# simonamtoft/downsampled-diffusion

Measured on AMD Instinct MI355X. Metric: images/sec (T=1000 sampling), 256x256 dDDPM-x3, higher is better.
Workload: dtype f32

## Files before the change

### downsampled-diffusion_amd/csrc/conv_wino.hip

```cpp
#include <atomic>
#include <cstdlib>
#include <type_traits>
#include <utility>

#include "conv_common.h"
#include "pack_elems.h"

namespace ddk {

__device__ __attribute__((aligned(128))) float g_wino_zero[32];

struct WinoParams {
    const float* src0;
    const float* src1;
    const float* wu;
    const float* bias;
    const float* resid;
    float* out;
    int c0, c1, cin;
    int B, H, W, TH, TW;
    int N, tiles;
    int splits, chunks, chunks_per_split;
    long long slab_stride;
    int post_mish;
    FastDivU dTW, dTH;
    float2* gn_part;
    int cpg, groups;
    const float* gn_gamma;
    const float* gn_beta;
    const float* gn_temb;
    const long long* gn_temb_rows;
    int gn_temb_stride;
    float gn_eps;
    float* cl_rec;
    unsigned* cl_cnt;
    unsigned* cl_fail;
    int cl_np;
    float* cl_slab;
    unsigned* cl_pair;
    const float* r1_x;
    const float* r1_w;
    const float* r1_b;
    int r1_cin, r1_ld;
};

constexpr int WBT = 32, WBN = 64;
constexpr int W_V = 4 * WBT * 32, W_U = 4 * WBN * 32;
constexpr int W_STAGE = W_V + W_U, W_NS = 3;
constexpr int W_LDS_FLOATS = W_NS * W_STAGE;
constexpr int W_TP = WBN + 4;
#ifndef DDK_WINO_LP
#define DDK_WINO_LP 4
#endif
constexpr int W_LP = DDK_WINO_LP;
static_assert(4 * 2 * WBT * W_TP <= W_LDS_FLOATS, "epilogue staging fits");

template <bool DGRAD>
__global__ __launch_bounds__(256) void pack_conv_weight_wino_kernel(const float* __restrict__ w, float* __restrict__ dst, int O, int I,
                                                                     int i_pad, long long total, int lo, int wi) {
    for (long long idx = blockIdx.x * 256LL + threadIdx.x; idx < total; idx += (long long)gridDim.x * 256)
        pack_wino_elem<DGRAD>(w, dst, idx, O, I, i_pad, lo, wi);
}

typedef int i32x4 __attribute__((ext_vector_type(4)));
typedef float f32x4 __attribute__((ext_vector_type(4)));

__device__ __forceinline__ i32x4 make_srd(const void* p, unsigned bytes) {
    const unsigned long long a = reinterpret_cast<unsigned long long>(p);
    i32x4 r;
    r.x = __builtin_amdgcn_readfirstlane((int)(unsigned)a);
    r.y = __builtin_amdgcn_readfirstlane((int)(unsigned)((a >> 32) & 0xFFFFu));
    r.z = __builtin_amdgcn_readfirstlane((int)bytes);
    r.w = 0x00020000;
    return r;
}
constexpr unsigned WINO_OOB = 0x80000000u;

__device__ __forceinline__ void buf_load16(f32x4& d, unsigned voff, const i32x4& srd, unsigned soff) {
    asm volatile("buffer_load_dwordx4 %0, %1, %2, %3 offen" : "=v"(d) : "v"(voff), "s"(srd), "s"(soff) : "memory");
}

__device__ __forceinline__ float4 f4add(float4 a, float4 b) { return make_float4(a.x + b.x, a.y + b.y, a.z + b.z, a.w + b.w); }
typedef float wino_f32x4 __attribute__((ext_vector_type(4)));
__device__ __forceinline__ void st_sc1_f4(float* p, float4 v) {
    const wino_f32x4 t = {v.x, v.y, v.z, v.w};
    asm volatile("global_store_dwordx4 %0, %1, off sc1\n\ts_nop 1" ::"v"(p), "v"(t) : "memory");
}
__device__ __forceinline__ void ld_sc1_f4x4(float4& a, float4& b, float4& c, float4& d, const float* pa, const float* pb, const float* pc,
                                            const float* pd) {
    wino_f32x4 x, y, z, w;
    asm volatile("global_load_dwordx4 %0, %4, off sc1\n\tglobal_load_dwordx4 %1, %5, off sc1\n\tglobal_load_dwordx4 %2, %6, off sc1\n\t"
                 "global_load_dwordx4 %3, %7, off sc1\n\ts_waitcnt vmcnt(0)"
                 : "=&v"(x), "=&v"(y), "=&v"(z), "=&v"(w)
                 : "v"(pa), "v"(pb), "v"(pc), "v"(pd)
                 : "memory");
    a = make_float4(x.x, x.y, x.z, x.w); b = make_float4(y.x, y.y, y.z, y.w);
    c = make_float4(z.x, z.y, z.z, z.w); d = make_float4(w.x, w.y, w.z, w.w);
}
__device__ __forceinline__ float4 f4sub(float4 a, float4 b) { return make_float4(a.x - b.x, a.y - b.y, a.z - b.z, a.w - b.w); }

__device__ unsigned long long g_wino_stamps[8 * 1024];

__device__ unsigned g_wino_cl_timeouts;
constexpr unsigned long long CL_TIMEOUT_TICKS = 2000000ull;

template <int DBG, bool CL = false>
__global__ __launch_bounds__(512) void conv3x3_wino_kernel(const WinoParams p) {
    extern __shared__ __attribute__((aligned(16))) float smem[];
    unsigned long long r_entry = 0;
    if (DBG) r_entry = __builtin_amdgcn_s_memrealtime();
    const int tid = threadIdx.x, lane = tid & 63;
    const int wid = __builtin_amdgcn_readfirstlane(tid >> 6);
    int tile_m, tile_n, split;
    {
        const int nwg = gridDim.x * gridDim.y * gridDim.z;
        const int bid = blockIdx.x + gridDim.x * (blockIdx.y + gridDim.y * blockIdx.z);
// ... 366 lines not shown
                    }
                }
            }
            __syncthreads();
            const unsigned long long* r0 = reinterpret_cast<const unsigned long long*>(p.cl_rec) +
                                           ((long long)image * p.cl_np * gridDim.y + tile_n) * 16 + gl;
            const bool poisoned = *gave_up != 0;
            float rm[8], rq[8];
#pragma unroll
            for (int i = 0; i < 8; ++i) {
                rm[i] = 0.f; rq[i] = 0.f;
                if (i < p.cl_np) {
                    const unsigned long long bits = __hip_atomic_load(r0 + (long long)i * gridDim.y * 16, __ATOMIC_RELAXED, __HIP_MEMORY_SCOPE_AGENT);
                    rm[i] = __uint_as_float((unsigned)bits);
                    rq[i] = __uint_as_float((unsigned)(bits >> 32));
                }
            }
            if (tid == 0) {
                const unsigned old = __hip_atomic_fetch_add(cnt + 1, 1u, __ATOMIC_RELAXED, __HIP_MEMORY_SCOPE_AGENT);
                if (old == (unsigned)p.cl_np - 1u) {
                    __hip_atomic_store(cnt, 0u, __ATOMIC_RELAXED, __HIP_MEMORY_SCOPE_AGENT);
                    __hip_atomic_store(cnt + 1, 0u, __ATOMIC_RELAXED, __HIP_MEMORY_SCOPE_AGENT);
                }
            }
            float ms = 0.f;
#pragma unroll
            for (int i = 0; i < 8; ++i) if (i < p.cl_np) ms += rm[i];
            const float gmean = poisoned ? __builtin_nanf("") : ms / (float)p.cl_np;
            float gm2 = 0.f, gd2 = 0.f;
#pragma unroll
            for (int i = 0; i < 8; ++i) if (i < p.cl_np) { gm2 += rq[i]; gd2 += (rm[i] - gmean) * (rm[i] - gmean); }
            const float n_i = 128.0f * (float)p.cpg;
            const float rstd = 1.0f / sqrtf((gm2 + n_i * gd2) / ((float)p.cl_np * n_i) + p.gn_eps);
            auto fin = [&](float4 v) {
                return make_float4(mish_f((v.x - gmean) * rstd * ga.x + be.x) + ts.x, mish_f((v.y - gmean) * rstd * ga.y + be.y) + ts.y,
                                   mish_f((v.z - gmean) * rstd * ga.z + be.z) + ts.z, mish_f((v.w - gmean) * rstd * ga.w + be.w) + ts.w);
            };
#pragma unroll
            for (int it = 0; it < 2; ++it) {
                *reinterpret_cast<float4*>(p.out + oo[it]) = f4add(fin(keep[it][0]), rs[it][0]);
                *reinterpret_cast<float4*>(p.out + oo[it] + p.N) = f4add(fin(keep[it][1]), rs[it][1]);
            }
        }
    }
    if (DBG && tid == 0) {
        asm volatile("s_waitcnt vmcnt(0)" ::: "memory");
        const int wg = (blockIdx.x + gridDim.x * (blockIdx.y + gridDim.y * blockIdx.z)) & 1023;
        g_wino_stamps[wg * 8 + 6] = __builtin_amdgcn_s_memrealtime();
        g_wino_stamps[wg * 8 + 7] = 1;
    }
}

#include "conv_wino2_kernel.inc"
#include "conv_winoT_kernel.inc"

enum { WINO_V_OLD = 0, WINO_V_D = 1, WINO_V_F = 2 };
static int wino_variant(int B, int H, int W, int N) {
#ifdef DDK_TUNING
    if (const char* e = getenv("DDK_WINO_VARIANT")) {
        const int v = atoi(e);
        if (v == WINO_V_OLD || v == WINO_V_D || (v == WINO_V_F && N % 128 == 0)) return v;
    }
#endif
    const long long mt = ceil_div((long long)B * (H / 2) * (W / 2), WBT);
    return (N % 128 == 0 && mt * (N / 128) >= 224) ? WINO_V_F : WINO_V_D;
}
static int wino_nt(int variant) { return variant == WINO_V_F ? 128 : WBN; }
bool conv_wino_ok(int kind, int H, int W, int cin, int N) {
    return kind == DDK_CONV3X3_S1 && H >= 2 && W >= 2 && H % 2 == 0 && W % 2 == 0 && cin > 0 && cin % 32 == 0 && N % 64 == 0;
}

int conv_wino_splits(int B, int H, int W, int cin, int N) {
    const long long tiles = (long long)B * (H / 2) * (W / 2);
    const long long wgs = ceil_div(tiles, WBT) * (N / wino_nt(wino_variant(B, H, W, N)));
    const int chunks = cin / 32;
    int s = 1;
    while (wgs * s < 256 && s * 2 <= chunks) s *= 2;
    const int cps = (int)ceil_div(chunks, s);
    return (int)ceil_div(chunks, cps);
}

static int wino_stats_shape_parts(int B, int H, int W, int cin, int N, int groups) {
    if (!conv_wino_ok(DDK_CONV3X3_S1, H, W, cin, N) || groups <= 0 || N % groups) return 0;
    const int cpg = N / groups, tpi = (H / 2) * (W / 2), nt_w = wino_nt(wino_variant(B, H, W, N));
    if (cpg % 4 || nt_w % cpg || nt_w / cpg > 8 || tpi % WBT || tpi / WBT > 32) return 0;
    return tpi / WBT;
}
int conv_wino_stats_parts(int B, int H, int W, int cin, int N, int groups) {
    if (conv_wino_splits(B, H, W, cin, N) != 1) return 0;
    return wino_stats_shape_parts(B, H, W, cin, N, groups);
}

bool convT_wino_ok(int H, int W, int cin, int N) {
    return H >= 2 && W >= 2 && H % 2 == 0 && W % 2 == 0 && cin > 0 && cin % 32 == 0 && N > 0 && N % WT_NT == 0;
}
int convT_wino_splits(int B, int H, int W, int cin, int N) {
    const long long wgs = ceil_div((long long)B * (H / 2) * (W / 2), WBT) * (N / WT_NT) * 4;
    const int chunks = cin / 32;
    int s = 1;
    while (wgs * s < 256 && s * 2 <= chunks) s *= 2;
    const int cps = (int)ceil_div(chunks, s);
    return (int)ceil_div(chunks, cps);
}
int convT_wino_forward(const ddk_conv_args& a, int splits, hipStream_t st) {
    WinoParams p{};
    p.src0 = a.src0; p.wu = a.weight_wino; p.bias = a.bias; p.out = a.out;
    p.c0 = a.c0; p.c1 = 0; p.cin = a.c0;
    p.B = a.B; p.H = a.H; p.W = a.W; p.TH = a.H / 2; p.TW = a.W / 2;
    p.N = a.N; p.tiles = a.B * p.TH * p.TW;
    p.chunks = p.cin / 32;
    p.chunks_per_split = (int)ceil_div(p.chunks, splits);
    p.splits = (int)ceil_div(p.chunks, p.chunks_per_split);
    p.slab_stride = (long long)a.B * (2 * a.H) * (2 * a.W) * a.N;
    p.dTW = make_fastdiv_u((unsigned)p.TW);
    p.dTH = make_fastdiv_u((unsigned)p.TH);
    if (p.splits > 1) p.out = static_cast<float*>(a.workspace);
    dim3 grid((unsigned)ceil_div(p.tiles, WBT), (unsigned)(a.N / WT_NT), (unsigned)(4 * p.splits));
#ifdef DDK_TUNING
    if (getenv("DDK_WINO_STAMPS")) {
        hipLaunchKernelGGL(convT_wino_kernel<1>, grid, dim3(1024), WT_LDS_FL * sizeof(float), st, p);
        return check_launch("convT_wino_kernel<dbg>");
    }
#endif
    hipLaunchKernelGGL(convT_wino_kernel<0>, grid, dim3(1024), WT_LDS_FL * sizeof(float), st, p);
    return check_launch("convT_wino_kernel");
}

int conv_wino_init_device() {
    DDK_HIP(hipFuncSetAttribute(reinterpret_cast<const void*>(&convT_wino_kernel<0>), hipFuncAttributeMaxDynamicSharedMemorySize,
                                (int)(WT_LDS_FL * sizeof(float))));
#ifdef DDK_TUNING
    DDK_HIP(hipFuncSetAttribute(reinterpret_cast<const void*>(&convT_wino_kernel<1>), hipFuncAttributeMaxDynamicSharedMemorySize,
                                (int)(WT_LDS_FL * sizeof(float))));
#endif
    DDK_HIP(hipFuncSetAttribute(reinterpret_cast<const void*>(&conv3x3_wino_kernel<0>), hipFuncAttributeMaxDynamicSharedMemorySize,
                                (int)(W_LDS_FLOATS * sizeof(float))));
    DDK_HIP(hipFuncSetAttribute(reinterpret_cast<const void*>(&conv3x3_wino_kernel<0, true>), hipFuncAttributeMaxDynamicSharedMemorySize,
                                (int)(W_LDS_FLOATS * sizeof(float))));
    DDK_HIP(hipFuncSetAttribute(reinterpret_cast<const void*>(&conv3x3_wino2_kernel<2, 0, false>), hipFuncAttributeMaxDynamicSharedMemorySize,
                                (int)(W2<2>::LDS_FL * sizeof(float))));
    DDK_HIP(hipFuncSetAttribute(reinterpret_cast<const void*>(&conv3x3_wino2_kernel<2, 0, true>), hipFuncAttributeMaxDynamicSharedMemorySize,
                                (int)(W2<2>::LDS_FL * sizeof(float))));
    DDK_HIP(hipFuncSetAttribute(reinterpret_cast<const void*>(&conv3x3_wino2_kernel<4, 0, false>), hipFuncAttributeMaxDynamicSharedMemorySize,
                                (int)(W2<4>::LDS_FL * sizeof(float))));
    DDK_HIP(hipFuncSetAttribute(reinterpret_cast<const void*>(&conv3x3_wino2_kernel<4, 0, true>), hipFuncAttributeMaxDynamicSharedMemorySize,
                                (int)(W2<4>::LDS_FL * sizeof(float))));
#ifdef DDK_TUNING
#define W2_DBG_ATTR(P_, D_) DDK_HIP(hipFuncSetAttribute(reinterpret_cast<const void*>(&conv3x3_wino2_kernel<P_, D_, false>), \
                                                hipFuncAttributeMaxDynamicSharedMemorySize, (int)(W2<P_>::LDS_FL * sizeof(float))))
    W2_DBG_ATTR(2, 1); W2_DBG_ATTR(2, 7); W2_DBG_ATTR(2, 9); W2_DBG_ATTR(2, 15); W2_DBG_ATTR(2, 17);
    W2_DBG_ATTR(4, 1); W2_DBG_ATTR(4, 7); W2_DBG_ATTR(4, 9); W2_DBG_ATTR(4, 15); W2_DBG_ATTR(4, 17);
#undef W2_DBG_ATTR
    DDK_HIP(hipFuncSetAttribute(reinterpret_cast<const void*>(&conv3x3_wino_kernel<1>), hipFuncAttributeMaxDynamicSharedMemorySize, (int)(W_LDS_FLOATS * sizeof(float))));
    DDK_HIP(hipFuncSetAttribute(reinterpret_cast<const void*>(&conv3x3_wino_kernel<2>), hipFuncAttributeMaxDynamicSharedMemorySize, (int)(W_LDS_FLOATS * sizeof(float))));
    DDK_HIP(hipFuncSetAttribute(reinterpret_cast<const void*>(&conv3x3_wino_kernel<3>), hipFuncAttributeMaxDynamicSharedMemorySize, (int)(W_LDS_FLOATS * sizeof(float))));
    DDK_HIP(hipFuncSetAttribute(reinterpret_cast<const void*>(&conv3x3_wino_kernel<4>), hipFuncAttributeMaxDynamicSharedMemorySize, (int)(W_LDS_FLOATS * sizeof(float))));
#endif
    return DDK_OK;
}

int conv_wino_cluster_np(int B, int H, int W, int cin, int N, int groups) {
    const int np = conv_wino_stats_parts(B, H, W, cin, N, groups);
    if (np <= 0 || np > 8) return 0;
    const int nt_w = wino_nt(wino_variant(B, H, W, N));
    if (N / groups > 32 || nt_w % (N / groups)) return 0;
    if (nt_w / (N / groups) > 8) return 0;
    const long long mt = (long long)B * np, nt = N / nt_w;
    if ((mt * nt) % 8) return 0;
    const long long run = mt * nt / 8;
    const long long per_round = run < 32 ? run : 32;
    if (run % (np * nt) || per_round % (np * nt)) return 0;
    return np;
}
int conv_wino_cluster_split_np(int B, int H, int W, int cin, int N, int groups, int* splits_out) {
    if (!conv_wino_ok(DDK_CONV3X3_S1, H, W, cin, N)) return 0;
    const int splits = conv_wino_splits(B, H, W, cin, N);
    if (splits_out) *splits_out = splits;
    if (splits <= 1 || splits > 4) return 0;
    const int np = wino_stats_shape_parts(B, H, W, cin, N, groups);
    if (np <= 0 || np > 8) return 0;
    const int variant = wino_variant(B, H, W, N);
    if (variant != WINO_V_D) return 0;
    const int nt_w = wino_nt(variant);
    if (N / groups > 32 || nt_w % (N / groups) || nt_w / (N / groups) > 8) return 0;
    const long long mt = (long long)B * np, nt = N / nt_w;
    if (mt * nt * splits > 256) return 0;
    return np;
}
size_t conv_wino_cluster_pair_words(int B, int H, int W, int N) {
    return (size_t)ceil_div((long long)B * (H / 2) * (W / 2), WBT) * (size_t)(N / WBN) * 16;
}
// ... 67 lines not shown
    p.post_mish = a.post_mish;
    p.dTW = make_fastdiv_u((unsigned)p.TW);
    p.dTH = make_fastdiv_u((unsigned)p.TH);
    if (p.splits > 1 && !fuse) p.out = static_cast<float*>(a.workspace);
    const int variant = wino_variant(a.B, a.H, a.W, a.N);
    if (variant != WINO_V_OLD) {
        dim3 grid2((unsigned)ceil_div(p.tiles, WBT), (unsigned)(a.N / wino_nt(variant)), (unsigned)p.splits);
        const bool f = variant == WINO_V_F;
        const size_t lds = (size_t)(f ? W2<2>::LDS_FL : W2<4>::LDS_FL) * sizeof(float);
#ifdef DDK_TUNING
        if (getenv("DDK_WINO_STAMPS")) {
            const int v = getenv("DDK_WINO_DEBUG") ? atoi(getenv("DDK_WINO_DEBUG")) : 1;
#define W2_DBG_LAUNCH(D_)                                                                                              \
    if (v == D_) {                                                                                                     \
        if (f) hipLaunchKernelGGL((conv3x3_wino2_kernel<2, D_, false>), grid2, dim3(768), lds, st, p);                 \
        else hipLaunchKernelGGL((conv3x3_wino2_kernel<4, D_, false>), grid2, dim3(768), lds, st, p);                   \
        return check_launch("conv3x3_wino2_kernel<dbg>");                                                              \
    }
            W2_DBG_LAUNCH(7) W2_DBG_LAUNCH(9) W2_DBG_LAUNCH(15) W2_DBG_LAUNCH(17)
#undef W2_DBG_LAUNCH
            if (f) hipLaunchKernelGGL((conv3x3_wino2_kernel<2, 1, false>), grid2, dim3(768), lds, st, p);
            else hipLaunchKernelGGL((conv3x3_wino2_kernel<4, 1, false>), grid2, dim3(768), lds, st, p);
            return check_launch("conv3x3_wino2_kernel<dbg>");
        }
#endif
        if (fuse) {
            if (f) hipLaunchKernelGGL((conv3x3_wino2_kernel<2, 0, true>), grid2, dim3(768), lds, st, p);
            else hipLaunchKernelGGL((conv3x3_wino2_kernel<4, 0, true>), grid2, dim3(768), lds, st, p);
            return check_launch("conv3x3_wino2_kernel<cluster>");
        }
        if (f) hipLaunchKernelGGL((conv3x3_wino2_kernel<2, 0, false>), grid2, dim3(768), lds, st, p);
        else hipLaunchKernelGGL((conv3x3_wino2_kernel<4, 0, false>), grid2, dim3(768), lds, st, p);
        return check_launch("conv3x3_wino2_kernel");
    }
    dim3 grid((unsigned)ceil_div(p.tiles, WBT), (unsigned)(a.N / WBN), (unsigned)p.splits);
#ifdef DDK_TUNING
    if (getenv("DDK_WINO_STAMPS")) {
        const int v = getenv("DDK_WINO_DEBUG") ? atoi(getenv("DDK_WINO_DEBUG")) : 1;
        if (v == 2) hipLaunchKernelGGL(conv3x3_wino_kernel<2>, grid, dim3(512), W_LDS_FLOATS * sizeof(float), st, p);
        else if (v == 3) hipLaunchKernelGGL(conv3x3_wino_kernel<3>, grid, dim3(512), W_LDS_FLOATS * sizeof(float), st, p);
        else if (v == 4) hipLaunchKernelGGL(conv3x3_wino_kernel<4>, grid, dim3(512), W_LDS_FLOATS * sizeof(float), st, p);
        else hipLaunchKernelGGL(conv3x3_wino_kernel<1>, grid, dim3(512), W_LDS_FLOATS * sizeof(float), st, p);
        return check_launch("conv3x3_wino_kernel<dbg>");
    }
#endif
    if (fuse) {
        hipLaunchKernelGGL((conv3x3_wino_kernel<0, true>), grid, dim3(512), W_LDS_FLOATS * sizeof(float), st, p);
        return check_launch("conv3x3_wino_kernel<cluster>");
    }
    hipLaunchKernelGGL(conv3x3_wino_kernel<0>, grid, dim3(512), W_LDS_FLOATS * sizeof(float), st, p);
    return check_launch("conv3x3_wino_kernel");
}

__global__ __launch_bounds__(256) void occupy_kernel(unsigned long long ticks, unsigned* sink) {
    extern __shared__ float occupy_lds[];
    occupy_lds[threadIdx.x] = (float)threadIdx.x;
    __syncthreads();
    const unsigned long long t_begin = __builtin_amdgcn_s_memrealtime();
    while (__builtin_amdgcn_s_memrealtime() - t_begin < ticks) __builtin_amdgcn_s_sleep(32);
    if (occupy_lds[(threadIdx.x + 1) & 255] < 0.f && sink) *sink = 1;
}

unsigned conv_wino_cluster_timeouts() {
    unsigned v = 0;
    if (hipMemcpyFromSymbol(&v, HIP_SYMBOL(g_wino_cl_timeouts), sizeof(v)) != hipSuccess) return ~0u;
    return v;
}

}

extern "C" int ddk_pack_conv_weight_wino(const float* w_oihw, float* dst, int O, int I, int i_pad, ddk_stream_t s) {
    using namespace ddk;
    DDK_REQUIRE(w_oihw && dst && O > 0 && I > 0 && i_pad >= I && i_pad % 32 == 0, "pack_conv_weight_wino: arguments (i_pad % 32 == 0)");
    const long long total = (long long)O * i_pad;
    DDK_REQUIRE(total < (1LL << 31), "pack_conv_weight_wino: 2^31 (n, c) pairs or more");
    const long long blocks = ceil_div(total, 256);
    hipLaunchKernelGGL(pack_conv_weight_wino_kernel<false>, dim3((unsigned)(blocks < 4096 ? blocks : 4096)), dim3(256), 0, as_stream(s), w_oihw,
                       dst, O, I, i_pad, total, 0, I);
    return check_launch("pack_conv_weight_wino_kernel");
}

extern "C" int ddk_pack_convT_weight_wino(const float* w_iohw, float* dst, int I, int O, int i_pad, ddk_stream_t s) {
    using namespace ddk;
    DDK_REQUIRE(w_iohw && dst && O > 0 && I > 0 && i_pad >= I && i_pad % 32 == 0, "pack_convT_weight_wino: arguments (i_pad % 32 == 0)");
    const long long total = (long long)O * i_pad;
    const long long blocks = ceil_div(total, 256);
    hipLaunchKernelGGL(pack_convT_weight_wino_kernel, dim3((unsigned)(blocks < 4096 ? blocks : 4096)), dim3(256), 0, as_stream(s), w_iohw, dst,
                       I, O, i_pad, total);
    return check_launch("pack_convT_weight_wino_kernel");
}
extern "C" int ddk_convT_wino_splits(int B, int H, int W, int cin, int N) {
    if (!ddk::convT_wino_ok(H, W, cin, N)) return 0;
    return ddk::convT_wino_splits(B, H, W, cin, N);
}

extern "C" int ddk_pack_conv_weight_wino_dgrad(const float* w_oihw, float* dst, int O, int I, int c_lo, int c_hi, int o_pad, ddk_stream_t s) {
    using namespace ddk;
    DDK_REQUIRE(w_oihw && dst && O > 0 && I > 0 && c_lo >= 0 && c_hi > c_lo && c_hi <= I && o_pad >= O && o_pad % 32 == 0,
                "pack_conv_weight_wino_dgrad: arguments (0 <= c_lo < c_hi <= I, o_pad % 32 == 0)");
    const long long total = (long long)(c_hi - c_lo) * o_pad;
    DDK_REQUIRE(total < (1LL << 31), "pack_conv_weight_wino_dgrad: 2^31 (n, c) pairs or more");
    const long long blocks = ceil_div(total, 256);
    hipLaunchKernelGGL(pack_conv_weight_wino_kernel<true>, dim3((unsigned)(blocks < 4096 ? blocks : 4096)), dim3(256), 0, as_stream(s), w_oihw,
                       dst, c_hi - c_lo, O, o_pad, total, c_lo, I);
    return check_launch("pack_conv_weight_wino_kernel<dgrad>");
}

#ifdef DDK_TUNING
extern "C" int ddk_debug_read_wino_timeline(unsigned long long* host_out) {
    if (hipDeviceSynchronize() != hipSuccess) return -2;
    return hipMemcpyFromSymbol(host_out, HIP_SYMBOL(ddk::g_wino_timeline), sizeof(unsigned long long) * 12 * 8 * 2) == hipSuccess ? 0 : -2;
}
extern "C" int ddk_debug_read_wino_stamps(unsigned long long* host_out) {
    if (hipDeviceSynchronize() != hipSuccess) return -2;
    if (hipMemcpyFromSymbol(host_out, HIP_SYMBOL(ddk::g_wino_stamps), sizeof(unsigned long long) * 8 * 1024) != hipSuccess) return -2;
    static unsigned long long zeros[8 * 1024];
    return hipMemcpyToSymbol(HIP_SYMBOL(ddk::g_wino_stamps), zeros, sizeof(zeros)) == hipSuccess ? 0 : -2;
}
#endif

extern "C" int ddk_conv_gn_partials(int B, int H, int W, int cin, int N, int groups) {
    return ddk::conv_wino_stats_parts(B, H, W, cin, N, groups);
}

extern "C" int ddk_conv_wino_splits(int B, int H, int W, int cin, int N) {
    if (!ddk::conv_wino_ok(DDK_CONV3X3_S1, H, W, cin, N)) return 0;
    return ddk::conv_wino_splits(B, H, W, cin, N);
}

extern "C" int ddk_conv3x3_gn_mish_cluster_ok(int B, int H, int W, int cin, int N, int groups) {
    if (!ddk::conv_wino_cluster_device_ok()) return 0;
    const int np = ddk::conv_wino_cluster_np(B, H, W, cin, N, groups);
// ... 70 lines not shown
```

### downsampled-diffusion_amd/csrc/ddk_internal.h

```cpp
#pragma once
#include <hip/hip_runtime.h>

#include <cstdarg>
#include <cstdint>
#include <cstdio>

#include "ddk.h"

#ifdef DDK_HOST_SANITIZE
#include "host_sanitize.h"
#endif

namespace ddk {

void set_error(const char* fmt, ...);

inline int fail_arg(const char* what) {
    set_error("bad argument: %s", what);
    return DDK_ERR_ARG;
}

inline int check_launch(const char* what) {
    hipError_t e = hipGetLastError();
    if (e != hipSuccess) {
// ... 66 lines not shown
    const int lane = threadIdx.x & 63, wid = threadIdx.x >> 6, nw = blockDim.x >> 6;
    __syncthreads();
    if (lane == 0) red[wid] = v;
    __syncthreads();
    float t = (lane < nw) ? red[lane] : 0.0f;
    t = wave_sum(t);
    return t;
}

__device__ __forceinline__ float block_max(float v, float* red) {
    v = wave_max(v);
    const int lane = threadIdx.x & 63, wid = threadIdx.x >> 6, nw = blockDim.x >> 6;
    __syncthreads();
    if (lane == 0) red[wid] = v;
    __syncthreads();
    float t = (lane < nw) ? red[lane] : -INFINITY;
    t = wave_max(t);
    return t;
}

int ensure_device_init();
int conv_init_device();
int wgrad_init_device();

size_t conv_workspace_bytes(int kind, int B, int H, int W, int cin, int N);
struct ConvLnFold {
    const float* c1;
    const float* c2;
    float eps;
};
struct WinoGnFuse {
    const float* gamma;
    const float* beta;
    const float* temb;
    const long long* temb_rows;
    int temb_stride;
    float eps;
    int groups;
    float* records;
    unsigned* counters;
    unsigned* fail;
    unsigned* pairs = nullptr;
    const float* res_x = nullptr;
    const float* res_w = nullptr;
    const float* res_b = nullptr;
    int res_cin = 0, res_ld = 0;
};
bool conv_ln_fold_ok(int B, int H, int W, int cin, int N);
int conv_forward(const ddk_conv_args& a, hipStream_t st, const ConvLnFold* ln = nullptr, const WinoGnFuse* fuse = nullptr);
int conv_splits(int kind, int B, int H, int W, int cin, int N);
bool conv_wino_ok(int kind, int H, int W, int cin, int N);
int conv_wino_splits(int B, int H, int W, int cin, int N);
int conv_wino_forward(const ddk_conv_args& a, int splits, hipStream_t st, const WinoGnFuse* fuse = nullptr);
int conv_wino_cluster_np(int B, int H, int W, int cin, int N, int groups);
int conv_wino_cluster_split_np(int B, int H, int W, int cin, int N, int groups, int* splits_out);
size_t conv_wino_cluster_pair_words(int B, int H, int W, int N);
bool conv_wino_variant_new(int B, int H, int W, int N);
bool conv_wino_cluster_device_ok();
size_t conv_wino_cluster_ws_floats(int B, int H, int W, int N);
unsigned conv_wino_cluster_timeouts();
bool convT_wino_ok(int H, int W, int cin, int N);
int convT_wino_splits(int B, int H, int W, int cin, int N);
int convT_wino_forward(const ddk_conv_args& a, int splits, hipStream_t st);
int conv_wino_init_device();
int conv_wino_stats_parts(int B, int H, int W, int cin, int N, int groups);
bool conv_first_ok(int cin, int N, int H, int W, int groups);
int conv_first(const float* x, const float* wp, const float* bias, float* out, float* gn_partials, int B, int H, int W, int cin, int N,
               int groups, int64_t* counter, int64_t* t_cur, hipStream_t st);
int conv_first_init_device();
bool conv_first_gn_ok(int cin, int N, int H, int W, int groups);
size_t conv_first_gn_ws_floats(int B, int H, int W);
int conv_first_gn(const float* x, const float* wp, const float* bias, const float* gamma, const float* beta, const float* temb,
                  int temb_stride, const long long* temb_rows, float eps, float* out, int B, int H, int W, int cin, int N, int groups,
                  float* records, unsigned* counters, unsigned* fail, int64_t* counter, int64_t* t_cur, hipStream_t st);
bool conv1x1_sm_ok(long long M, int c0, int c1, int N);
int conv1x1_sm(const float* src0, int c0, const float* src1, int c1, const float* w, const float* bias, const float* resid, float* out,
               long long M, int N, const ConvLnFold* ln, hipStream_t st);
int conv1x1_sm_init_device();
bool conv1x1_stream_ok(long long M, int cin, int N);
int conv1x1_stream(const float* x, int cin, const float* w, const float* bias, const float* dmish_src, const float* resid, float* out,
                   float* mish_out, long long M, int N, int pre_mish, int post_mish, hipStream_t st);
bool conv1x1_ws_ok(long long M, int K, int N);
int conv1x1_ws(const float* x, const float* w, const float* bias, const float* resid, float* out, long long M, int N, const ConvLnFold* ln,
               hipStream_t st, int images = 0);
int conv1x1_ws_init_device();
struct AddendSlabs {
    int n = 1;
    long long stride = 0;
    const float* bias = nullptr;
};
bool conv_gn_local_ok(int H, int W, int cin, int c0, int N, int groups);
int conv_gn_local(const float* src0, int c0, const float* src1, int c1, const float* w, const float* bias, const float* gamma,
                  const float* beta, const float* temb, int temb_stride, const long long* temb_rows, const float* addend, float* out,
                  int B, int H, int W, int N, int groups, float eps, hipStream_t st, const AddendSlabs& as = AddendSlabs(),
                  const AddendSlabs& src_slabs = AddendSlabs());
int conv_gn_local_init_device();
bool conv_gn_wlocal_ok(int H, int W, int cin, int c0, int N, int groups);
int conv_gn_wlocal(const float* src0, int c0, const float* src1, int c1, const float* w, const float* bias, const float* gamma,
                   const float* beta, const float* temb, int temb_stride, const long long* temb_rows, const float* addend, float* out,
                   int B, int H, int W, int N, int groups, float eps, hipStream_t st, const AddendSlabs& as = AddendSlabs(),
                   const AddendSlabs& src_slabs = AddendSlabs());
double conv_flops(int kind, int B, int H, int W, int cin, int N);
size_t groupnorm_workspace_bytes(int B, int HW, int C, int groups);
int gn_train_nsplit(int HW, int cpg);
int gn_stats_partials(const float* x, float* part, int B, int HW, int C, int groups, int ns, hipStream_t st);
int groupnorm_mish(const float* x, const float* gamma, const float* beta, const float* temb, int temb_stride,
// ... 53 lines not shown
```

### downsampled-diffusion_amd/csrc/unet_plan.hip

```cpp
#include <mutex>
#include <string>
#include <vector>

#include "ddk_internal.h"
#include "level_chain.h"

namespace ddk {

constexpr int HEADS = 4;
constexpr int HIDDEN = HEADS * 32;
constexpr int GROUPS = 8;
constexpr float GN_EPS = 1e-5f, LN_EPS = 1e-5f;

static inline int pad32(int c) { return (c + 31) / 32 * 32; }

enum PackKind { PK_COPY = 0, PK_CONV = 1, PK_CONVT = 2, PK_LINEAR_T = 3, PK_WINO = 4, PK_LOCAL = 5, PK_WLOCAL = 6, PK_FIRST = 7, PK_CONVT_WINO = 8,
                PK_ROWS = 9 , PK_LOCAL1 = 10 ,
                PK_CONVT_LOCAL = 11  };

struct Slot {
    std::string name;
    long long numel;
    int kind;
    size_t off;
    int O, I, KH, KW, i_pad, ld, col0;
    int split = 0, split_pad = 0;
    int attn = -1;
};

struct ConvW {
    size_t w = 0, b = 0;
    bool has_bias = false;
    int cin = 0, cin_pad = 0, cout = 0;
    size_t wu = 0;
    bool has_wu = false;
    size_t wl = 0;
    bool has_wl = false;
    size_t wwl = 0;
    bool has_wwl = false;
    size_t wf = 0;
    bool has_wf = false;
    size_t wl1 = 0;
    bool has_wl1 = false;
    size_t wtl = 0;
    bool has_wtl = false;
};
struct NormW { size_t g = 0, b = 0; int c_real = 0; };
struct ResW {
    int ci = 0, ci_pad = 0, co = 0, temb_off = 0, ci_real = 0, co_real = 0;
    ConvW c1, c2, res;
    NormW n1, n2;
    bool has_res = false;
};
struct AttnW {
    int c = 0, c_real = 0;
    NormW ln;
    ConvW qkv, out;
    size_t qkv_lnw = 0, ln_c1 = 0, ln_c2 = 0;
    size_t qkv_op = 0;
};

}

using namespace ddk;

struct SamplerGraph {
    const void *packed, *x, *noise, *ws, *c_recip, *c_recipm1, *c1, *c2, *sigma;
    int B, H, W, t_start, device;
    unsigned long long pack_epoch;
    hipGraph_t graph = nullptr;
    hipGraphExec_t exec = nullptr;
    hipGraph_t graph_multi = nullptr;
    hipGraphExec_t exec_multi = nullptr;
    hipEvent_t done = nullptr;
    unsigned long long last_use = 0;
};
constexpr int SAMPLER_MULTI = 16;

struct ddk_unet {
    std::mutex mu;
    std::vector<SamplerGraph> graphs;
    unsigned long long use_clock = 0;
    unsigned long long pack_epoch = 0;
    struct { const void* ws = nullptr; int t_start = -1, B = 0, H = 0, W = 0; unsigned long long pack_epoch = 0; } table;
    ddk_unet_config cfg;
    int cluster_gn = 1;
    int cluster_limit = 1 << 30;
    int cluster_np_max = 8;
    bool cluster_split = true;
    bool attn_kvctx = true;
    bool fold_down_reduce = false;
    bool first_gn = true;
    int level_chain = 9;
    int level_chain_max_batch = 32;
    int attn_fold_min_hw = 256;
    bool attn_fold = true;
    bool generic = false;
    std::vector<int> dimp;
    std::vector<Slot> slots;
    size_t packed_floats = 0;
    int L = 0;
    std::vector<int> dims;
    int time_dim = 0, temb_total = 0;
    size_t freqs = 0, w1t = 0, b1 = 0, w2t = 0, b2 = 0, temb_wt = 0, temb_bias = 0;
    std::vector<ResW> down_res, up_res;
    std::vector<AttnW> down_attn, up_attn;
    std::vector<ConvW> down_conv, up_conv;
    ResW mid1, mid2;
    AttnW mid_attn;
    ConvW final_conv;
    NormW final_norm;
    size_t final_w = 0, final_b = 0;

    size_t alloc(size_t n) {
        const size_t o = packed_floats;
        packed_floats += (n + 3) / 4 * 4;
        return o;
    }
    size_t add_copy(const std::string& name, long long n) {
        const size_t o = alloc((size_t)n);
        slots.push_back(Slot{name, n, PK_COPY, o, 0, 0, 0, 0, 0, 0, 0});
        return o;
    }
    void add_copy_at(const std::string& name, long long n, size_t off) {
        slots.push_back(Slot{name, n, PK_COPY, off, 0, 0, 0, 0, 0, 0, 0});
    }
    ConvW add_conv(const std::string& prefix, int cout, int cin, int k, bool bias, bool gn_follows = false, int split = 0, bool local = false) {
        ConvW c;
        c.cin = cin; c.cin_pad = split > 0 ? pad32(split) + pad32(cin - split) : pad32(cin); c.cout = cout;
        const int cout_rows = pad32(cout);
        c.w = alloc((size_t)cout_rows * k * k * c.cin_pad);
        Slot sl{prefix + "weight", (long long)cout * cin * k * k, PK_CONV, c.w, cout, cin, k, k, c.cin_pad, 0, 0};
        if (split > 0 && c.cin_pad != cin) { sl.split = split; sl.split_pad = pad32(split); }
        slots.push_back(sl);
        c.has_bias = bias;
        if (bias) {
            c.b = alloc((size_t)cout_rows);
            slots.push_back(Slot{prefix + "bias", cout, PK_COPY, c.b, 0, 0, 0, 0, 0, 0, 0});
        }
        if (generic) return c;
        if (k == 1 && bias && cout % 32 == 0 && c.cin_pad == cin && cin % 32 == 0) {
            c.wl1 = alloc((size_t)cout * c.cin_pad);
            c.has_wl1 = true;
            slots.push_back(Slot{prefix + "weight", (long long)cout * cin, PK_LOCAL1, c.wl1, cout, cin, 1, 1, c.cin_pad, 0, 0});
        }
        if (k == 3 && cout % 64 == 0) {
            c.wu = alloc((size_t)16 * cout * c.cin_pad);
            c.has_wu = true;
            slots.push_back(Slot{prefix + "weight", (long long)cout * cin * k * k, PK_WINO, c.wu, cout, cin, k, k, c.cin_pad, 0, 0});
        }
        if (k == 3 && (gn_follows || local) && cout % 32 == 0) {
            c.wl = alloc((size_t)9 * cout * c.cin_pad);
            c.has_wl = true;
            slots.push_back(Slot{prefix + "weight", (long long)cout * cin * k * k, PK_LOCAL, c.wl, cout, cin, k, k, c.cin_pad, 0, 0});
            if (gn_follows && (c.cin_pad <= 320 || c.cin_pad == 512)) {
                c.wwl = alloc((size_t)16 * cout * c.cin_pad);
                c.has_wwl = true;
                slots.push_back(Slot{prefix + "weight", (long long)cout * cin * k * k, PK_WLOCAL, c.wwl, cout, cin, k, k, c.cin_pad, 0, 0});
            }
        }
        return c;
    }
    ConvW add_convT(const std::string& prefix, int ch, bool local = false) {
        ConvW c;
        c.cin = ch; c.cin_pad = pad32(ch); c.cout = ch;
        c.w = alloc((size_t)16 * pad32(ch) * pad32(ch));
        slots.push_back(Slot{prefix + "weight", (long long)16 * ch * ch, PK_CONVT, c.w, ch, ch, 4, 4, pad32(ch), 0, 0});
        c.has_bias = true;
        c.b = alloc((size_t)pad32(ch));
        slots.push_back(Slot{prefix + "bias", ch, PK_COPY, c.b, 0, 0, 0, 0, 0, 0, 0});
        if (local && ch % 32 == 0 && !generic) {
            c.wtl = alloc((size_t)16 * ch * ch);
            c.has_wtl = true;
            slots.push_back(Slot{prefix + "weight", (long long)16 * ch * ch, PK_CONVT_LOCAL, c.wtl, ch, ch, 4, 4, ch, 0, 0});
        }
        if (ch % 128 == 0) {
            c.wu = alloc((size_t)36 * ch * ch);
            c.has_wu = true;
            slots.push_back(Slot{prefix + "weight", (long long)16 * ch * ch, PK_CONVT_WINO, c.wu, ch, ch, 4, 4, ch, 0, 0});
        }
        return c;
    }
    NormW add_norm(const std::string& wname, const std::string& bname, int c) {
        NormW n;
        n.c_real = c;
        n.g = alloc((size_t)pad32(c));
        slots.push_back(Slot{wname, c, PK_COPY, n.g, 0, 0, 0, 0, 0, 0, 0});
        n.b = alloc((size_t)pad32(c));
        slots.push_back(Slot{bname, c, PK_COPY, n.b, 0, 0, 0, 0, 0, 0, 0});
        return n;
    }
    ResW add_res(const std::string& p, int ci, int co, int& temb_cursor, int split = 0) {
        ResW r;
        r.ci_real = ci; r.co_real = co;
        r.ci = ci; r.ci_pad = split > 0 ? pad32(split) + pad32(ci - split) : pad32(ci); r.co = pad32(co);
        if (!generic) r.co = co;
        r.temb_off = temb_cursor;
        temb_cursor += co;
        slots.push_back(Slot{p + "mlp.1.weight", (long long)co * time_dim, PK_LINEAR_T, temb_wt, co, time_dim, 0, 0, 0, temb_total, r.temb_off});
        add_copy_at(p + "mlp.1.bias", co, temb_bias + r.temb_off);
        r.c1 = add_conv(p + "block1.block.0.", co, ci, 3, true, true, split);
        r.n1 = add_norm(p + "block1.block.1.weight", p + "block1.block.1.bias", co);
// ... 7 lines not shown
    std::vector<AttnW> attn_all;
    AttnW add_attn(const std::string& p, int c) {
        AttnW a;
        a.c = generic ? pad32(c) : c;
        a.c_real = c;
        const size_t s0 = slots.size();
        a.qkv = add_conv(p + "fn.fn.to_qkv.", 3 * HIDDEN, c, 1, false);
        const size_t s1 = slots.size();
        a.out = add_conv(p + "fn.fn.to_out.", c, HIDDEN, 1, true);
        const size_t s2 = slots.size();
        a.ln = add_norm(p + "fn.norm.g", p + "fn.norm.b", c);
        for (size_t i = s0; i < s1; ++i) slots[i].attn = n_attn;
        for (size_t i = s2; i < slots.size(); ++i) slots[i].attn = n_attn;
        a.qkv_lnw = alloc((size_t)3 * HIDDEN * pad32(c));
        a.ln_c1 = alloc((size_t)3 * HIDDEN);
        a.ln_c2 = alloc((size_t)3 * HIDDEN);
        a.qkv_op = alloc((size_t)3 * HIDDEN * pad32(c));
        attn_all.push_back(a);
        ++n_attn;
        return a;
    }
};

static int total_temb(const ddk_unet& u) {
    int tot = 0;
    for (int l = 0; l < u.L; ++l) tot += 2 * u.dims[l + 1];
    tot += 2 * u.dims[u.L];
    for (int i = 0; i < u.L - 1; ++i) tot += 2 * u.dims[u.L - 1 - i];
    return tot;
}

extern "C" ddk_unet* ddk_unet_create(const ddk_unet_config* cfg) {
    if (!cfg || cfg->n_levels < 1 || cfg->n_levels > 8 || cfg->in_ch < 1 || cfg->chan < 8 || cfg->chan % 8 ||
        cfg->chan > 512) {
        set_error("unet_create: need 1 <= n_levels <= 8, in_ch >= 1, unet_chan a multiple of 8 in [8, 512]");
        return nullptr;
    }
    for (int i = 0; i < cfg->n_levels; ++i)
        if (cfg->mults[i] < 1) { set_error("unet_create: unet_dims entries must be >= 1"); return nullptr; }
    if (cfg->mults[0] != 1) {
        set_error("unet_create: unet_dims[0] must be 1 (the reference's final Block(dim, dim) meets dim * unet_dims[0] channels "
                  "otherwise and raises, unet.py:69-72)");
        return nullptr;
    }
    {
        int ndev = 0;
        if (hipGetDeviceCount(&ndev) == hipSuccess && ndev > 0 && ensure_device_init() != DDK_OK) return nullptr;
        (void)hipGetLastError();
    }
    ddk_unet* u = new ddk_unet();
    u->cfg = *cfg;
    u->L = cfg->n_levels;
    u->generic = cfg->chan % 32 != 0;
    for (int i = 0; i < cfg->n_levels; ++i)
        if (cfg->chan * cfg->mults[i] > 512) { set_error("unet_create: level widths above 512 channels are not supported"); delete u; return nullptr; }
    u->dims.push_back(cfg->in_ch);
    for (int i = 0; i < u->L; ++i) u->dims.push_back(cfg->chan * cfg->mults[i]);
    for (int d : u->dims) u->dimp.push_back(u->generic ? pad32(d) : d);
    u->time_dim = cfg->chan;
    u->temb_total = total_temb(*u);
    const int td = u->time_dim;

    u->freqs = u->add_copy("@sinusoidal_freqs", td / 2);
    u->w1t = u->alloc((size_t)td * 4 * td);
    u->slots.push_back(Slot{"time_mlp.1.weight", (long long)4 * td * td, PK_LINEAR_T, u->w1t, 4 * td, td, 0, 0, 0, 4 * td, 0});
    u->b1 = u->add_copy("time_mlp.1.bias", 4 * td);
    u->w2t = u->alloc((size_t)4 * td * td);
    u->slots.push_back(Slot{"time_mlp.3.weight", (long long)4 * td * td, PK_LINEAR_T, u->w2t, td, 4 * td, 0, 0, 0, td, 0});
    u->b2 = u->add_copy("time_mlp.3.bias", td);
    u->temb_wt = u->alloc((size_t)td * u->temb_total);
    u->temb_bias = u->alloc((size_t)u->temb_total);

    int cur = 0;
    for (int l = 0; l < u->L; ++l) {
        const std::string p = "downs." + std::to_string(l) + ".";
        const int ci = u->dims[l], co = u->dims[l + 1];
        u->down_res.push_back(u->add_res(p + "0.", ci, co, cur));
        if (l == 0 && ci <= 8 && co <= 256 && !u->generic) {
            ConvW& c1 = u->down_res[0].c1;
            const int K2 = (9 * ci + 1) / 2;
            c1.wf = u->alloc((size_t)(co / 32) * K2 * 64);
            c1.has_wf = true;
            u->slots.push_back(Slot{p + "0.block1.block.0.weight", (long long)co * ci * 9, PK_FIRST, c1.wf, co, ci, 3, 3, 0, 0, 0});
        }
        u->down_res.push_back(u->add_res(p + "1.", co, co, cur));
        u->down_attn.push_back(u->add_attn(p + "2.", co));
        if (l < u->L - 1) u->down_conv.push_back(u->add_conv(p + "3.conv.", co, co, 3, true, false, 0, l == u->L - 2));
    }
    const int mid = u->dims[u->L];
    u->mid1 = u->add_res("mid_block1.", mid, mid, cur);
    u->mid_attn = u->add_attn("mid_attn.", mid);
    u->mid2 = u->add_res("mid_block2.", mid, mid, cur);
    for (int i = 0; i < u->L - 1; ++i) {
        const std::string p = "ups." + std::to_string(i) + ".";
        const int din = u->dims[u->L - 1 - i], dout = u->dims[u->L - i];
        u->up_res.push_back(u->add_res(p + "0.", 2 * dout, din, cur, dout));
        u->up_res.push_back(u->add_res(p + "1.", din, din, cur));
        u->up_attn.push_back(u->add_attn(p + "2.", din));
        u->up_conv.push_back(u->add_convT(p + "3.conv.", din, i == 0));
    }
    u->final_conv = u->add_conv("final_conv.0.block.0.", cfg->chan, cfg->chan, 3, true, true);
    u->final_norm = u->add_norm("final_conv.0.block.1.weight", "final_conv.0.block.1.bias", cfg->chan);
    if (u->generic) {
        u->final_w = u->alloc((size_t)cfg->in_ch * pad32(cfg->chan));
        u->slots.push_back(Slot{"final_conv.1.weight", (long long)cfg->in_ch * cfg->chan, PK_ROWS, u->final_w, cfg->in_ch, cfg->chan, 0, 0, 0,
                                pad32(cfg->chan), 0});
// ... 29 lines not shown
}

extern "C" int ddk_sampler_invalidate(ddk_unet* u) {
    DDK_REQUIRE(u, "sampler_invalidate: null plan");
    std::lock_guard<std::mutex> lock(u->mu);
    if (!u->graphs.empty()) DDK_HIP(hipDeviceSynchronize());
    drop_graphs(u);
    return DDK_OK;
}
static void destroy_entry(SamplerGraph& g) {
    if (g.done) { (void)hipEventSynchronize(g.done); (void)hipEventDestroy(g.done); }
    if (g.exec) (void)hipGraphExecDestroy(g.exec);
    if (g.graph) (void)hipGraphDestroy(g.graph);
    if (g.exec_multi) (void)hipGraphExecDestroy(g.exec_multi);
    if (g.graph_multi) (void)hipGraphDestroy(g.graph_multi);
}

extern "C" int ddk_sampler_release_workspace(ddk_unet* u, const void* workspace) {
    DDK_REQUIRE(u && workspace, "sampler_release_workspace: arguments");
    std::lock_guard<std::mutex> lock(u->mu);
    for (size_t i = 0; i < u->graphs.size();) {
        if (u->graphs[i].ws == workspace) {
            destroy_entry(u->graphs[i]);
            u->graphs.erase(u->graphs.begin() + (long)i);
        } else {
            ++i;
        }
    }
    if (u->table.ws == workspace) u->table.ws = nullptr;
    return DDK_OK;
}

extern "C" int ddk_unet_set_option(ddk_unet* u, int option, int value) {
    DDK_REQUIRE(u, "unet_set_option: null plan");
    if (option == DDK_OPT_CLUSTER_GROUPNORM) {
        std::lock_guard<std::mutex> lock(u->mu);
        if (!u->graphs.empty()) DDK_HIP(hipDeviceSynchronize());
        drop_graphs(u);
        u->cluster_gn = value < 0 ? 0 : value > 2 ? 2 : value;
        return DDK_OK;
    }
    if (option == DDK_OPT_ATTENTION_FOLD) {
        std::lock_guard<std::mutex> lock(u->mu);
        if (!u->graphs.empty()) DDK_HIP(hipDeviceSynchronize());
        drop_graphs(u);
        u->attn_fold = value != 0;
        return DDK_OK;
    }
    if (option == DDK_OPT_ATTENTION_KV_CONTEXT) {
        std::lock_guard<std::mutex> lock(u->mu);
        if (!u->graphs.empty()) DDK_HIP(hipDeviceSynchronize());
        drop_graphs(u);
        u->attn_kvctx = value != 0;
        return DDK_OK;
    }
    if (option == DDK_OPT_FIRST_GROUPNORM) {
        std::lock_guard<std::mutex> lock(u->mu);
        if (!u->graphs.empty()) DDK_HIP(hipDeviceSynchronize());
        drop_graphs(u);
        u->first_gn = value != 0;
        return DDK_OK;
    }
    if (option == DDK_OPT_LEVEL_CHAIN) {
        std::lock_guard<std::mutex> lock(u->mu);
        if (!u->graphs.empty()) DDK_HIP(hipDeviceSynchronize());
        drop_graphs(u);
        u->level_chain = value == 1 ? 9 : value == 2 ? 1 : value == 3 ? 15 : value == 4 ? 6 : value == 8 ? 2 : value == 16 ? 4 : value != 0 ? 9 : 0;
        return DDK_OK;
    }
    if (option == DDK_OPT_FOLD_DOWNSAMPLE_REDUCE) {
        std::lock_guard<std::mutex> lock(u->mu);
        if (!u->graphs.empty()) DDK_HIP(hipDeviceSynchronize());
        drop_graphs(u);
        u->fold_down_reduce = value != 0;
        return DDK_OK;
    }
    if (option == 10) {
        std::lock_guard<std::mutex> lock(u->mu);
        if (!u->graphs.empty()) DDK_HIP(hipDeviceSynchronize());
        drop_graphs(u);
        u->level_chain_max_batch = value;
        return DDK_OK;
    }
    if (option == 9) {
        std::lock_guard<std::mutex> lock(u->mu);
        if (!u->graphs.empty()) DDK_HIP(hipDeviceSynchronize());
        drop_graphs(u);
        u->attn_fold_min_hw = value;
        return DDK_OK;
    }
    if (option == 2) {
        std::lock_guard<std::mutex> lock(u->mu);
        u->cluster_limit = value;
        return DDK_OK;
    }
    if (option == 4) {
        std::lock_guard<std::mutex> lock(u->mu);
        if (!u->graphs.empty()) DDK_HIP(hipDeviceSynchronize());
        drop_graphs(u);
        u->cluster_np_max = value;
        return DDK_OK;
    }
    if (option == 11) {
        std::lock_guard<std::mutex> lock(u->mu);
        if (!u->graphs.empty()) DDK_HIP(hipDeviceSynchronize());
        drop_graphs(u);
// ... 22 lines not shown
        wg[(long long)n * cp + c] = wv * gv;
        s1 += wv * gv;
        s2 += wv * bv;
    }
    s1 = wave_sum(s1);
    s2 = wave_sum(s2);
    if (threadIdx.x == 0) { c1[n] = s1; c2[n] = s2; }
}

static int fold_attn(const AttnW& a, float* P, hipStream_t st) {
    hipLaunchKernelGGL(ln_fold_kernel, dim3(3 * HIDDEN), dim3(64), 0, st, P + a.qkv.w, P + a.ln.g, P + a.ln.b, P + a.qkv_lnw, P + a.ln_c1,
                       P + a.ln_c2, a.c, pad32(a.c));
    DDK_TRY(check_launch("ln_fold_kernel"));
    return qkv_operand_pack(P + a.qkv_lnw, P + a.qkv_op, HEADS, pad32(a.c), st);
}

static void weights_changed(const ddk_unet* u) {
    ddk_unet* m = const_cast<ddk_unet*>(u);
    std::lock_guard<std::mutex> lock(m->mu);
    ++m->pack_epoch;
}

extern "C" int ddk_unet_finalize_pack(const ddk_unet* u, void* packed, ddk_stream_t s) {
    DDK_REQUIRE(u && packed, "unet_finalize_pack: arguments");
    weights_changed(u);
    for (const AttnW& a : u->attn_all) DDK_TRY(fold_attn(a, static_cast<float*>(packed), as_stream(s)));
    return DDK_OK;
}

extern "C" int ddk_unet_pack_slot(const ddk_unet* u, int slot, const float* canonical, void* packed, ddk_stream_t s) {
    DDK_REQUIRE(u && canonical && packed && slot >= 0 && slot < (int)u->slots.size(), "unet_pack_slot: arguments");
    const Slot& sl = u->slots[slot];
    float* dst = static_cast<float*>(packed) + sl.off;
    weights_changed(u);
    int rc;
    switch (sl.kind) {
        case PK_COPY:
            DDK_HIP(hipMemcpyAsync(dst, canonical, (size_t)sl.numel * sizeof(float), hipMemcpyDeviceToDevice, as_stream(s)));
            rc = DDK_OK;
            break;
        case PK_CONV:
            rc = sl.split > 0 ? ddk_pack_conv_weight_split(canonical, dst, sl.O, sl.I, sl.KH, sl.KW, sl.i_pad, sl.split, sl.split_pad, s)
                              : ddk_pack_conv_weight(canonical, dst, sl.O, sl.I, sl.KH, sl.KW, sl.i_pad, s);
            break;
        case PK_CONVT: rc = sl.i_pad == sl.I ? ddk_pack_convT_weight(canonical, dst, sl.I, sl.O, s)
                                             : ddk_pack_convT_weight_padded(canonical, dst, sl.I, sl.O, sl.i_pad, s); break;
        case PK_ROWS:
            DDK_HIP(hipMemcpy2DAsync(dst, (size_t)sl.ld * sizeof(float), canonical, (size_t)sl.I * sizeof(float), (size_t)sl.I * sizeof(float),
                                     (size_t)sl.O, hipMemcpyDeviceToDevice, as_stream(s)));
            rc = DDK_OK;
            break;
        case PK_LINEAR_T: rc = ddk_pack_linear_T(canonical, dst, sl.O, sl.I, sl.ld, sl.col0, s); break;
        case PK_WINO: rc = ddk_pack_conv_weight_wino(canonical, dst, sl.O, sl.I, sl.i_pad, s); break;
        case PK_LOCAL: rc = ddk_pack_conv_weight_local(canonical, dst, sl.O, sl.I, sl.i_pad, s); break;
        case PK_LOCAL1: rc = ddk_pack_conv1x1_weight_local(canonical, dst, sl.O, sl.I, sl.i_pad, s); break;
        case PK_CONVT_LOCAL: rc = ddk_pack_convT_weight_local(canonical, dst, sl.I, sl.O, s); break;
        case PK_WLOCAL: rc = ddk_pack_conv_weight_wino_local(canonical, dst, sl.O, sl.I, sl.i_pad, s); break;
        case PK_FIRST: rc = ddk_pack_conv_weight_first(canonical, dst, sl.O, sl.I, s); break;
        case PK_CONVT_WINO: rc = ddk_pack_convT_weight_wino(canonical, dst, sl.I, sl.O, sl.i_pad, s); break;
        default: return fail_arg("unet_pack_slot: slot kind");
    }
    DDK_TRY(rc);
    if (sl.attn >= 0) DDK_TRY(fold_attn(u->attn_all[sl.attn], static_cast<float*>(packed), as_stream(s)));
    return DDK_OK;
}

namespace ddk {

struct Layout {
    size_t act = 0;
    size_t qkv = 0, o = 0, ctx = 0, splitk = 0, gn_ws = 0, cl = 0, chain = 0;
    std::vector<size_t> skip;
    size_t xpad = 0, temb = 0, tact = 0;
    size_t off_A = 0, off_B = 0, off_C = 0, off_raw = 0, off_a1 = 0, off_res = 0, off_xn = 0, off_qkv = 0, off_o = 0, off_ctx = 0,
           off_splitk = 0, off_gn = 0, off_xpad = 0, off_temb = 0, off_tact = 0, off_cl = 0, off_chain = 0;
    std::vector<size_t> off_skip;
    size_t total = 0;
};

static size_t al4(size_t n) { return (n + 3) / 4 * 4; }

static void upd(size_t& m, size_t v) { if (v > m) m = v; }

static bool convT_wino_use(int B, int H, int W, int cin, int N) {
    return convT_wino_ok(H, W, cin, N) && convT_wino_splits(B, H, W, cin, N) <= 2;
}
static bool use_wino(const ConvW& cw, int H, int W, int cin, int N) {
    return cw.has_wu && conv_wino_ok(DDK_CONV3X3_S1, H, W, cin, N);
}
static int conv3_splits(const ConvW& cw, int B, int H, int W, int cin, int N) {
    return use_wino(cw, H, W, cin, N) ? conv_wino_splits(B, H, W, cin, N) : conv_splits(DDK_CONV3X3_S1, B, H, W, cin, N);
}
static size_t conv3_ws_floats(const ConvW& cw, int B, int H, int W, int cin, int N) {
    if (!use_wino(cw, H, W, cin, N)) return conv_workspace_bytes(DDK_CONV3X3_S1, B, H, W, cin, N) / 4;
    const int s = conv_wino_splits(B, H, W, cin, N);
    return s > 1 ? (size_t)s * B * H * W * N : 0;
}

constexpr size_t CL_PAIR_WORDS = 128 * 16;
static size_t cl_counter_floats(int B) { return (size_t)B * 8 * 16 + 16 + (size_t)B * 64 + CL_PAIR_WORDS; }
static size_t cl_fail_offset(int B) { return (size_t)B * 8 * 16; }
static size_t cl_chain_offset(int B) { return (size_t)B * 8 * 16 + 16; }
static size_t cl_pair_offset(int B) { return (size_t)B * 8 * 16 + 16 + (size_t)B * 64; }
constexpr int CHAIN_BUFS = 18;
constexpr int CHAIN8_BUFS = 5;

// ... 84 lines not shown
    ly.act = al4(ly.act); ly.qkv = al4(ly.qkv); ly.o = al4(ly.o); ly.ctx = al4(ly.ctx);
    ly.splitk = al4(ly.splitk); ly.gn_ws = al4(ly.gn_ws); ly.cl = al4(ly.cl);
    if (level_chain_shape_ok(u, H0, W0)) ly.chain = (size_t)CHAIN_BUFS * B * 16 * 256;
    if (level8_chain_shape_ok(u, H0, W0)) upd(ly.chain, (size_t)CHAIN8_BUFS * B * 64 * 256);

    size_t off = 0;
    auto take = [&](size_t n) { const size_t o = off; off += n; return o; };
    ly.off_A = take(ly.act); ly.off_B = take(ly.act); ly.off_C = take(ly.act);
    ly.off_raw = take(ly.act); ly.off_a1 = take(ly.act); ly.off_res = take(ly.act); ly.off_xn = take(ly.act);
    ly.off_qkv = take(ly.qkv); ly.off_o = take(ly.o); ly.off_ctx = take(ly.ctx);
    ly.off_splitk = take(ly.splitk); ly.off_gn = take(ly.gn_ws); ly.off_cl = take(ly.cl); ly.off_chain = take(ly.chain);
    ly.off_xpad = take(ly.xpad); ly.off_temb = take(ly.temb); ly.off_tact = take(ly.tact);
    ly.off_skip.resize(u.L);
    for (int l = 0; l < u.L; ++l) ly.off_skip[l] = take(ly.skip[l]);
    ly.total = off;
    return ly;
}

struct Ctx {
    const ddk_unet& u;
    const float* P;
    float* W;
    const Layout& ly;
    int B;
    hipStream_t st;
    const float* temb;
    const long long* temb_rows;
    bool allow_cluster = false;
    int n_cluster = 0;
    const float* x_first = nullptr;
    const float* x_padded = nullptr;
};

static int run_conv(Ctx& c, int kind, const ConvW& cw, const float* src0, int c0, const float* src1, int c1, const float* resid,
                    float* out, int H, int W, int N, const float* weight_override = nullptr, const ConvLnFold* ln = nullptr) {
    ddk_conv_args a{};
    a.kind = kind;
    a.src0 = src0; a.src1 = src1; a.c0 = c0; a.c1 = c1;
    a.weight = weight_override ? weight_override : c.P + cw.w;
    a.bias = cw.has_bias ? c.P + cw.b : nullptr;
    a.resid = resid;
    a.out = out;
    a.B = c.B; a.H = H; a.W = W; a.N = N;
    a.pre_mish = 0;
    a.post_mish = 0;
    a.defer_reduce = 0;
    a.workspace = c.W + c.ly.off_splitk;
    a.workspace_bytes = c.ly.splitk * sizeof(float);
    if (kind == DDK_CONV3X3_S1 && !weight_override && use_wino(cw, H, W, c0 + c1, N)) a.weight_wino = c.P + cw.wu;
    if (kind == DDK_CONVT4X4_S2 && !weight_override && cw.has_wu && !src1 && convT_wino_use(c.B, H, W, c0, N)) a.weight_wino = c.P + cw.wu;
    return conv_forward(a, c.st, ln);
}

static bool conv_gn_is_local(const ConvW& cw, int B, int H, int W, int c0, int c1, int N) {
    return (cw.has_wl && (H * W == 16 || (H * W == 4 && B % 4 == 0)) && conv_gn_local_ok(H, W, c0 + c1, c0, N, GROUPS)) ||
           (cw.has_wwl && H * W == 64 && conv_gn_wlocal_ok(H, W, c0 + c1, c0, N, GROUPS));
}

static int run_conv_gn(Ctx& c, const ConvW& cw, const float* src0, int c0, const float* src1, int c1, float* raw, const NormW& n,
                       const float* temb, const float* addend, float* out, int H, int W, int N, const AddendSlabs& as = AddendSlabs(),
                       const AddendSlabs& ss = AddendSlabs()) {
    if (ss.n > 1 && !conv_gn_is_local(cw, c.B, H, W, c0, c1, N)) return fail_arg("run_conv_gn: slab source on a path that cannot sum it");
    if (c.u.generic) {
        if (as.n > 1 || ss.n > 1) return fail_arg("run_conv_gn: slab addend / source on the generic path");
        DDK_TRY(run_conv(c, DDK_CONV3X3_S1, cw, src0, c0, src1, c1, nullptr, raw, H, W, N));
        return groupnorm_mish_generic(raw, c.P + n.g, c.P + n.b, temb, c.u.temb_total, addend, out, c.B, H * W, N, n.c_real, GROUPS, GN_EPS,
                                      c.st, c.temb_rows);
    }
    if (cw.has_wl && (H * W == 16 || (H * W == 4 && c.B % 4 == 0)) && conv_gn_local_ok(H, W, c0 + c1, c0, N, GROUPS))
        return conv_gn_local(src0, c0, src1, c1, c.P + cw.wl, cw.has_bias ? c.P + cw.b : nullptr, c.P + n.g, c.P + n.b, temb,
                             c.u.temb_total, c.temb_rows, addend, out, c.B, H, W, N, GROUPS, GN_EPS, c.st, as, ss);
    if (cw.has_wwl && H * W == 64 && conv_gn_wlocal_ok(H, W, c0 + c1, c0, N, GROUPS))
        return conv_gn_wlocal(src0, c0, src1, c1, c.P + cw.wwl, cw.has_bias ? c.P + cw.b : nullptr, c.P + n.g, c.P + n.b, temb,
                              c.u.temb_total, c.temb_rows, addend, out, c.B, H, W, N, GROUPS, GN_EPS, c.st, as, ss);
    if (as.n > 1) return fail_arg("run_conv_gn: slab addend on a path that cannot sum it");
    if (cw.has_wf && c.x_first && src0 == c.x_padded && !src1 && conv_first_ok(c.u.cfg.in_ch, N, H, W, GROUPS)) {
        DDK_TRY(conv_first(c.x_first, c.P + cw.wf, cw.has_bias ? c.P + cw.b : nullptr, raw, nullptr, c.B, H, W, c.u.cfg.in_ch, N, GROUPS,
                           nullptr, nullptr, c.st));
        return groupnorm_mish(raw, c.P + n.g, c.P + n.b, temb, c.u.temb_total, addend, out, c.B, H * W, N, GROUPS, GN_EPS,
                              c.W + c.ly.off_gn, c.ly.gn_ws * sizeof(float), c.st, c.temb_rows);
    }
    const int cl_np = c.allow_cluster && cw.has_wu && conv_wino_cluster_device_ok() ? conv_wino_cluster_np(c.B, H, W, c0 + c1, N, GROUPS) : 0;
    if (cl_np > 0 && cl_np <= c.u.cluster_np_max && c.n_cluster++ < c.u.cluster_limit) {
        ddk_conv_args a{};
        a.kind = DDK_CONV3X3_S1;
        a.src0 = src0; a.src1 = src1; a.c0 = c0; a.c1 = c1;
        a.weight = c.P + cw.w;
        a.weight_wino = c.P + cw.wu;
        a.bias = cw.has_bias ? c.P + cw.b : nullptr;
        a.resid = addend;
        a.out = out;
        a.B = c.B; a.H = H; a.W = W; a.N = N;
        float* cl = c.W + c.ly.off_cl;
        const WinoGnFuse f{c.P + n.g, c.P + n.b, temb, c.temb_rows, c.u.temb_total, GN_EPS, GROUPS, cl + cl_counter_floats(c.B),
                           reinterpret_cast<unsigned*>(cl), reinterpret_cast<unsigned*>(cl + cl_fail_offset(c.B))};
        return conv_forward(a, c.st, nullptr, &f);
    }
    int cls_splits = 1;
    const int cls_np = c.allow_cluster && c.u.cluster_split && cw.has_wu && conv_wino_cluster_device_ok()
                           ? conv_wino_cluster_split_np(c.B, H, W, c0 + c1, N, GROUPS, &cls_splits) : 0;
    if (cls_np > 0 && cls_np <= c.u.cluster_np_max && (size_t)cls_splits * c.B * H * W * N <= c.ly.splitk &&
        conv_wino_cluster_pair_words(c.B, H, W, N) <= CL_PAIR_WORDS && c.n_cluster++ < c.u.cluster_limit) {
        ddk_conv_args a{};
        a.kind = DDK_CONV3X3_S1;
        a.src0 = src0; a.src1 = src1; a.c0 = c0; a.c1 = c1;
        a.weight = c.P + cw.w;
        a.weight_wino = c.P + cw.wu;
        a.bias = cw.has_bias ? c.P + cw.b : nullptr;
        a.resid = addend;
        a.out = out;
        a.B = c.B; a.H = H; a.W = W; a.N = N;
        a.workspace = c.W + c.ly.off_splitk;
        a.workspace_bytes = c.ly.splitk * sizeof(float);
        float* cl = c.W + c.ly.off_cl;
        WinoGnFuse f{c.P + n.g, c.P + n.b, temb, c.temb_rows, c.u.temb_total, GN_EPS, GROUPS, cl + cl_counter_floats(c.B),
                     reinterpret_cast<unsigned*>(cl), reinterpret_cast<unsigned*>(cl + cl_fail_offset(c.B))};
        f.pairs = reinterpret_cast<unsigned*>(cl + cl_pair_offset(c.B));
        return conv_forward(a, c.st, nullptr, &f);
    }
    const int np = cw.has_wu ? conv_wino_stats_parts(c.B, H, W, c0 + c1, N, GROUPS) : 0;
    if (np > 0) {
        ddk_conv_args a{};
        a.kind = DDK_CONV3X3_S1;
        a.src0 = src0; a.src1 = src1; a.c0 = c0; a.c1 = c1;
        a.weight = c.P + cw.w;
        a.weight_wino = c.P + cw.wu;
        a.bias = cw.has_bias ? c.P + cw.b : nullptr;
        a.out = raw;
        a.B = c.B; a.H = H; a.W = W; a.N = N;
        a.gn_partials = c.W + c.ly.off_gn;
        a.gn_groups = GROUPS;
        DDK_TRY(conv_forward(a, c.st));
        return groupnorm_mish_parts(raw, c.W + c.ly.off_gn, np, c.P + n.g, c.P + n.b, temb, c.u.temb_total, addend, out, c.B, H * W, N,
// ... 304 lines not shown
    c.allow_cluster = allow_cluster;
    float* bufA = ws + ly.off_A;
    float* bufB = ws + ly.off_B;
    float* bufC = ws + ly.off_C;
    float* raw = ws + ly.off_raw;
    float* a1 = ws + ly.off_a1;
    float* gnp = ws + ly.off_gn;

    int H = H0, W = W0;
    const float* cur = xpad;
    int cur_c = pad32(u.cfg.in_ch);
    AddendSlabs cur_ss;
    const bool first_fused = fast0 && c.allow_cluster && u.first_gn && conv_wino_cluster_device_ok() &&
                             conv_first_gn_ok(u.down_res[0].ci, u.down_res[0].co, H0, W0, GROUPS) && u.cluster_limit > 0;
    int64_t* dec_counter = (first_fused && step) ? step->state : nullptr;
    const bool chained = level_chain_use(c, H0, W0);
    const bool chain_edges = chained && (u.level_chain & 8) && u.L >= 2 && u.down_conv[u.L - 2].has_wl && u.down_conv[u.L - 2].has_bias &&
                             u.up_conv[0].has_wtl && u.up_conv[0].cin == 256 && u.down_conv[u.L - 2].cin == 256;
    const bool chained8 = level8_chain_use(c, H0, W0, 2);
    const bool chained8u = level8_chain_use(c, H0, W0, 4);
    for (int l = 0; l < u.L; ++l) {
        float* skip = ws + ly.off_skip[l];
        const int co = u.dimp[l + 1];
        if (chained && l == u.L - 1) {
            DDK_TRY(run_level_chain(c, 0, cur, skip, bufB, chain_edges ? ws + ly.off_skip[l - 1] : nullptr, chain_edges ? bufA : nullptr));
            cur_c = co;
            break;
        }
        const bool level_chained = chained8 && l == u.L - 2 && cur_ss.n == 1;
        if (level_chained) {
            DDK_TRY(run_level_chain(c, 1, cur, skip, nullptr));
        } else if (l == 0 && fast0) {
            const ResW& r = u.down_res[0];
            if (first_fused) {
                float* cl = ws + ly.off_cl;
                DDK_TRY(conv_first_gn(x, P + r.c1.wf, r.c1.has_bias ? P + r.c1.b : nullptr, P + r.n1.g, P + r.n1.b, c.temb + r.temb_off,
                                      u.temb_total, c.temb_rows, GN_EPS, a1, B, H, W, r.ci, r.co, GROUPS, cl + cl_counter_floats(B),
                                      reinterpret_cast<unsigned*>(cl), reinterpret_cast<unsigned*>(cl + cl_fail_offset(B)),
                                      step ? step->state : nullptr, step ? t : nullptr, st));
            } else {
                DDK_TRY(conv_first(x, P + r.c1.wf, r.c1.has_bias ? P + r.c1.b : nullptr, raw, gnp, B, H, W, r.ci, r.co, GROUPS,
                                   step ? step->state : nullptr, step ? t : nullptr, st));
                DDK_TRY(groupnorm_mish_parts(raw, gnp, H * W / 128, P + r.n1.g, P + r.n1.b, c.temb + r.temb_off, u.temb_total, nullptr, a1, B,
                                             H * W, r.co, GROUPS, GN_EPS, st, c.temb_rows));
            }
            ddk_conv_args a{};
            a.kind = DDK_CONV3X3_S1;
            a.src0 = a1; a.c0 = r.co;
            a.weight = P + r.c2.w;
            a.weight_wino = P + r.c2.wu;
            a.bias = r.c2.has_bias ? P + r.c2.b : nullptr;
            a.B = B; a.H = H; a.W = W; a.N = r.co;
            const int cl_np = c.allow_cluster && conv_wino_cluster_device_ok() && r.ci <= 8 ? conv_wino_cluster_np(B, H, W, r.co, r.co, GROUPS) : 0;
            if (cl_np > 0 && cl_np <= u.cluster_np_max && conv_wino_variant_new(B, H, W, r.co) && c.n_cluster++ < u.cluster_limit) {
                a.out = bufB;
                float* cl = ws + ly.off_cl;
                WinoGnFuse f{P + r.n2.g, P + r.n2.b, nullptr, nullptr, u.temb_total, GN_EPS, GROUPS, cl + cl_counter_floats(B),
                             reinterpret_cast<unsigned*>(cl), reinterpret_cast<unsigned*>(cl + cl_fail_offset(B))};
                f.res_x = x; f.res_w = P + r.res.w; f.res_b = r.res.has_bias ? P + r.res.b : nullptr; f.res_cin = r.ci; f.res_ld = r.res.cin_pad;
                DDK_TRY(conv_forward(a, st, nullptr, &f));
            } else {
                a.out = raw;
                a.gn_partials = gnp;
                a.gn_groups = GROUPS;
                DDK_TRY(conv_forward(a, st));
                DDK_TRY(groupnorm_mish_parts(raw, gnp, conv_wino_stats_parts(B, H, W, r.co, r.co, GROUPS), P + r.n2.g, P + r.n2.b, nullptr,
                                             u.temb_total, nullptr, bufB, B, H * W, r.co, GROUPS, GN_EPS, st, nullptr, x, P + r.res.w,
                                             r.res.has_bias ? P + r.res.b : nullptr, r.ci, r.res.cin_pad));
            }
        } else {
            DDK_TRY(run_res(c, u.down_res[2 * l], cur, cur_c, nullptr, 0, bufB, H, W, cur_ss));
            cur_ss = AddendSlabs();
        }
        if (!level_chained) {
            DDK_TRY(run_res(c, u.down_res[2 * l + 1], bufB, co, nullptr, 0, bufC, H, W));
            DDK_TRY(run_attn(c, u.down_attn[l], bufC, skip, H, W));
        }
        if (l < u.L - 1 && chain_edges && l + 1 == u.L - 1) {
            H /= 2; W /= 2;
            cur = skip;
        } else if (l < u.L - 1) {
            const int s2 = conv_splits(DDK_CONV3X3_S2, B, H, W, co, co);
            if (u.fold_down_reduce && s2 > 1 && !(chained && l + 1 == u.L - 1) && !(chained8 && l + 1 == u.L - 2) &&
                res_takes_slab_source(u, u.down_res[2 * l + 2], B, H / 2, W / 2, co)) {
                ddk_conv_args a{};
                a.kind = DDK_CONV3X3_S2;
                a.src0 = skip; a.c0 = co;
                a.weight = P + u.down_conv[l].w;
                a.out = bufA;
                a.B = B; a.H = H; a.W = W; a.N = co;
                a.defer_reduce = 1;
                a.workspace = ws + ly.off_splitk;
                a.workspace_bytes = ly.splitk * sizeof(float);
                DDK_TRY(conv_forward(a, st));
                cur_ss.n = s2;
                cur_ss.stride = (long long)B * (H / 2) * (W / 2) * co;
                cur_ss.bias = u.down_conv[l].has_bias ? P + u.down_conv[l].b : nullptr;
                H /= 2; W /= 2;
                cur = ws + ly.off_splitk;
            } else {
                DDK_TRY(run_conv(c, DDK_CONV3X3_S2, u.down_conv[l], skip, co, nullptr, 0, nullptr, bufA, H, W, co));
                H /= 2; W /= 2;
                cur = bufA;
            }
        } else {
            cur = skip;
        }
        cur_c = co;
    }
    if (!chained) {
        DDK_TRY(run_res(c, u.mid1, cur, cur_c, nullptr, 0, bufB, H, W));
        DDK_TRY(run_attn(c, u.mid_attn, bufB, bufC, H, W));
        DDK_TRY(run_res(c, u.mid2, bufC, cur_c, nullptr, 0, bufA, H, W));
        cur = bufA;
    }
    for (int i = 0; i < u.L - 1; ++i) {
        const int lvl = u.L - 1 - i;
        const float* skip = ws + ly.off_skip[lvl];
        const int dout = u.dimp[lvl + 1], din = u.dimp[lvl];
        if (chained8u && i == 1) {
            DDK_TRY(run_level_chain(c, 2, cur, const_cast<float*>(skip), bufB));
        } else if (!(chained && i == 0)) {
            DDK_TRY(run_res(c, u.up_res[2 * i], cur, cur_c, skip, dout, bufB, H, W));
            DDK_TRY(run_res(c, u.up_res[2 * i + 1], bufB, din, nullptr, 0, bufC, H, W));
            DDK_TRY(run_attn(c, u.up_attn[i], bufC, bufB, H, W));
        }
        if (!(chain_edges && i == 0))
            DDK_TRY(run_conv(c, DDK_CONVT4X4_S2, u.up_conv[i], bufB, din, nullptr, 0, nullptr, bufA, H, W, din));
        H *= 2; W *= 2;
        cur = bufA;
        cur_c = din;
    }
    const int chan = u.generic ? pad32(u.cfg.chan) : u.cfg.chan, n_out = u.cfg.in_ch;
    const int npf = u.final_conv.has_wu ? conv_wino_stats_parts(B, H, W, cur_c, chan, GROUPS) : 0;
    if (npf > 0 && final_tail_ok(H * W, chan, GROUPS, n_out, npf) && (!step || step->per == (long long)H * W * n_out)) {
        ddk_conv_args a{};
        a.kind = DDK_CONV3X3_S1;
        a.src0 = cur; a.c0 = cur_c;
        a.weight = P + u.final_conv.w;
        a.weight_wino = P + u.final_conv.wu;
        a.bias = u.final_conv.has_bias ? P + u.final_conv.b : nullptr;
        a.out = raw;
        a.B = B; a.H = H; a.W = W; a.N = chan;
        a.gn_partials = gnp;
        a.gn_groups = GROUPS;
        DDK_TRY(conv_forward(a, st));
        if (step)
            return final_tail(raw, gnp, npf, P + u.final_norm.g, P + u.final_norm.b, GN_EPS, P + u.final_w, P + u.final_b, n_out, nullptr,
                              step->x, step->noise, step->noise_step_stride, step->t_first, t, step->c_recip, step->c_recipm1, step->c1,
                              step->c2, step->sigma, step->state, 0, 0, B, H * W, chan, GROUPS, st, dec_counter);
        return final_tail(raw, gnp, npf, P + u.final_norm.g, P + u.final_norm.b, GN_EPS, P + u.final_w, P + u.final_b, n_out, out, nullptr,
                          nullptr, 0, 0, nullptr, nullptr, nullptr, nullptr, nullptr, nullptr, nullptr, 0, 0, B, H * W, chan, GROUPS, st);
    }
    DDK_TRY(run_conv_gn(c, u.final_conv, cur, cur_c, nullptr, 0, raw, u.final_norm, nullptr, nullptr, a1, H, W, chan));
    float* eps_hat = step ? step->eps_hat : out;
    DDK_TRY(conv1x1_small_n(a1, P + u.final_w, P + u.final_b, eps_hat, (long long)B * H * W, chan, n_out, st));
    if (!step) return DDK_OK;
    return p_sample_update(step->x, eps_hat, step->noise, step->noise_step_stride, step->t_first, t, step->c_recip, step->c_recipm1,
                           step->c1, step->c2, step->sigma, B, step->per, 0, 0, st, step->state, dec_counter);
}

static int check_shape(const ddk_unet* u, int B, int H, int W) {
    DDK_REQUIRE(u, "unet: null plan");
    DDK_REQUIRE(B > 0 && H > 0 && W > 0, "unet: B/H/W must be positive");
    const int f = 1 << (u->L - 1);
    if (H % f || W % f) {
        set_error("unet: spatial size %dx%d must be divisible by %d (%d stride-2 stages, unet.py:43-50)", H, W, f, u->L - 1);
        return DDK_ERR_ARG;
    }
    return DDK_OK;
}

__global__ void set_chain_state_kernel(int64_t* state, int64_t t_start, uint64_t seed, uint32_t stream_id) {
    state[0] = t_start;
    state[1] = (int64_t)seed;
    state[2] = (int64_t)stream_id;
}

}

extern "C" size_t ddk_unet_workspace_bytes(const ddk_unet* u, int B, int H, int W) {
    if (check_shape(u, B, H, W) != DDK_OK) return 0;
    return make_layout(*u, B, H, W).total * sizeof(float);
}

extern "C" int ddk_unet_forward(const ddk_unet* u, const void* packed, const float* x, const int64_t* t, float* out, int B, int H,
                                int W, void* workspace, size_t workspace_bytes, ddk_stream_t s) {
    DDK_TRY(check_shape(u, B, H, W));
    DDK_REQUIRE(packed && x && t && out && workspace, "unet_forward: null pointer");
    DDK_REQUIRE(aligned16(packed) && aligned16(workspace) && aligned16(x) && aligned16(out), "unet_forward: alignment");
    const Layout ly = make_layout(*u, B, H, W);
    if (workspace_bytes < ly.total * sizeof(float)) {
        set_error("unet_forward: workspace too small (%zu < %zu)", workspace_bytes, ly.total * sizeof(float));
        return DDK_ERR_WORKSPACE;
    }
    float* ws = static_cast<float*>(workspace);
    DDK_TRY(ensure_device_init());
    DDK_HIP(hipMemsetAsync(ws + ly.off_cl, 0, cl_counter_floats(B) * sizeof(float), as_stream(s)));
    return forward_core(*u, static_cast<const float*>(packed), x, const_cast<int64_t*>(t), out, B, H, W, ws, ly, as_stream(s),
// ... 1 lines not shown
}

extern "C" int ddk_unet_cluster_check(const ddk_unet* u, void* workspace, int B, int H, int W, ddk_stream_t s) {
    DDK_TRY(check_shape(u, B, H, W));
    DDK_REQUIRE(workspace, "unet_cluster_check: null workspace");
    const Layout ly = make_layout(*u, B, H, W);
    unsigned* word = reinterpret_cast<unsigned*>(static_cast<float*>(workspace) + ly.off_cl + cl_fail_offset(B));
    unsigned v = 0;
    DDK_HIP(hipMemcpyAsync(&v, word, sizeof(v), hipMemcpyDeviceToHost, as_stream(s)));
    DDK_HIP(hipStreamSynchronize(as_stream(s)));
    if (v == 0) return DDK_OK;
    DDK_HIP(hipMemsetAsync(word, 0, sizeof(v), as_stream(s)));
    set_error("in-launch GroupNorm: %u workgroup(s) gave up waiting for their cluster (the GPU is shared, masked or partitioned); "
              "results on this workspace are invalid -- rerun with DDK_OPT_CLUSTER_GROUPNORM = 0", v);
    return DDK_ERR_CLUSTER;
}

extern "C" double ddk_unet_flops(const ddk_unet* u, int B, int H0, int W0) {
    if (check_shape(u, B, H0, W0) != DDK_OK) return 0;
    double f = 0;
    auto res = [&](const ResW& r, int H, int W) {
        f += conv_flops(DDK_CONV3X3_S1, B, H, W, r.ci_real, r.co_real) + conv_flops(DDK_CONV3X3_S1, B, H, W, r.co_real, r.co_real);
        if (r.has_res) f += conv_flops(DDK_CONV1X1, B, H, W, r.ci_real, r.co_real);
        f += 2.0 * B * u->time_dim * r.co_real;
    };
    auto attn = [&](const AttnW& a, int H, int W) {
        f += conv_flops(DDK_CONV1X1, B, H, W, a.c_real, 3 * HIDDEN) + conv_flops(DDK_CONV1X1, B, H, W, HIDDEN, a.c_real);
        f += 2.0 * 2.0 * B * HEADS * 32.0 * 32.0 * H * W;
    };
    int H = H0, W = W0;
    f += 2.0 * B * (u->time_dim * 4.0 * u->time_dim) * 2;
    for (int l = 0; l < u->L; ++l) {
        res(u->down_res[2 * l], H, W); res(u->down_res[2 * l + 1], H, W); attn(u->down_attn[l], H, W);
        if (l < u->L - 1) { f += conv_flops(DDK_CONV3X3_S2, B, H, W, u->dims[l + 1], u->dims[l + 1]); H /= 2; W /= 2; }
    }
    res(u->mid1, H, W); attn(u->mid_attn, H, W); res(u->mid2, H, W);
    for (int i = 0; i < u->L - 1; ++i) {
        res(u->up_res[2 * i], H, W); res(u->up_res[2 * i + 1], H, W); attn(u->up_attn[i], H, W);
        f += conv_flops(DDK_CONVT4X4_S2, B, H, W, u->up_conv[i].cin, u->up_conv[i].cout);
        H *= 2; W *= 2;
    }
    f += conv_flops(DDK_CONV3X3_S1, B, H, W, u->cfg.chan, u->cfg.chan) + conv_flops(DDK_CONV1X1, B, H, W, u->cfg.chan, u->cfg.in_ch);
    return f;
}

extern "C" double ddk_unet_flops_executed(const ddk_unet* u, int B, int H0, int W0) {
    if (check_shape(u, B, H0, W0) != DDK_OK) return 0;
    double f = 0;
    auto conv3 = [&](const ConvW& cw, int H, int W, int c0, int c1, int N, bool gn) {
        const int cin = c0 + c1;
        if (gn && cw.has_wl && (H * W == 16 || (H * W == 4 && B % 4 == 0)) && conv_gn_local_ok(H, W, cin, c0, N, GROUPS))
            return 2.0 * B * H * W * 9.0 * cin * N;
        if (gn && cw.has_wwl && H * W == 64 && conv_gn_wlocal_ok(H, W, cin, c0, N, GROUPS)) return 2.0 * B * (H * W / 4) * 16.0 * cin * N;
        if (use_wino(cw, H, W, cin, N)) return 2.0 * (double)(ceil_div((long long)B * (H / 2) * (W / 2), 32) * 32) * 16.0 * cin * N;
        return 2.0 * B * H * W * 9.0 * cin * N;
    };
    auto res = [&](const ResW& r, int H, int W, int c0, int c1, bool fast) {
        if (fast) {
            f += 2.0 * B * H * W * (2.0 * ((9 * r.ci + 1) / 2)) * r.co;
            f += 2.0 * B * H * W * (double)r.ci * r.co;
        } else {
            f += conv3(r.c1, H, W, c0, c1, r.co, true);
            if (r.has_res) f += conv_flops(DDK_CONV1X1, B, H, W, c0 + c1, r.co);
        }
        f += conv3(r.c2, H, W, r.co, 0, r.co, true);
    };
    auto attn = [&](const AttnW& a, int H, int W) {
        if (attn_fold_eligible(*u, a, B, H, W)) {
            f += conv_flops(DDK_CONV1X1, B, H, W, a.c, 2 * HIDDEN) + 2.0 * B * HEADS * 32.0 * 32.0 * H * W;
            f += 2.0 * B * (4.0 * HIDDEN * 32.0 * a.c + (double)a.c * HIDDEN * a.c) + conv_flops(DDK_CONV1X1, B, H, W, a.c, a.c);
            return;
        }
        f += conv_flops(DDK_CONV1X1, B, H, W, a.c, 3 * HIDDEN) + conv_flops(DDK_CONV1X1, B, H, W, HIDDEN, a.c);
        f += 2.0 * 2.0 * B * HEADS * 32.0 * 32.0 * H * W;
    };
    int H = H0, W = W0, cur_c = pad32(u->cfg.in_ch);
    for (int l = 0; l < u->L; ++l) {
        const int co = u->dims[l + 1];
        res(u->down_res[2 * l], H, W, cur_c, 0, l == 0 && first_fast(*u, B, H, W));
        res(u->down_res[2 * l + 1], H, W, co, 0, false);
        attn(u->down_attn[l], H, W);
        if (l < u->L - 1) { f += conv_flops(DDK_CONV3X3_S2, B, H, W, co, co); H /= 2; W /= 2; }
        cur_c = co;
    }
    res(u->mid1, H, W, cur_c, 0, false); attn(u->mid_attn, H, W); res(u->mid2, H, W, cur_c, 0, false);
    for (int i = 0; i < u->L - 1; ++i) {
        const int lvl = u->L - 1 - i, dout = u->dims[lvl + 1], din = u->dims[lvl];
        res(u->up_res[2 * i], H, W, cur_c, dout, false);
        res(u->up_res[2 * i + 1], H, W, din, 0, false);
        attn(u->up_attn[i], H, W);
        if (u->up_conv[i].has_wu && convT_wino_use(B, H, W, din, din))
            f += 2.0 * (double)(ceil_div((long long)B * (H / 2) * (W / 2), 32) * 32) * 36.0 * din * din;
        else
            f += conv_flops(DDK_CONVT4X4_S2, B, H, W, din, din);
        H *= 2; W *= 2;
        cur_c = din;
    }
    f += conv3(u->final_conv, H, W, cur_c, 0, u->cfg.chan, true) + 2.0 * B * H * W * (double)u->cfg.chan * u->cfg.in_ch;
    return f;
}

namespace ddk {
struct SamplerLayout {
    size_t unet_floats, off_eps, off_t, off_table, off_tact_all, off_tall, total;
};
static SamplerLayout sampler_layout(const ddk_unet& u, int B, int H, int W, int t_start) {
    SamplerLayout s;
    const size_t rows = (size_t)t_start + 1;
    s.unet_floats = make_layout(u, B, H, W).total;
    s.off_eps = s.unet_floats;
    s.off_t = s.off_eps + al4((size_t)B * H * W * u.cfg.in_ch);
    s.off_table = s.off_t + al4(2 * (size_t)(B + 3));
    s.off_tact_all = s.off_table + al4(rows * u.temb_total);
    s.off_tall = s.off_tact_all + al4(rows * u.time_dim);
    s.total = s.off_tall + al4(2 * rows);
    return s;
}

__global__ void iota64_kernel(int64_t* out, int n) {
    const int i = blockIdx.x * blockDim.x + threadIdx.x;
    if (i < n) out[i] = i;
}
}

extern "C" size_t ddk_sampler_workspace_bytes(const ddk_unet* u, int B, int H, int W, int t_start) {
    if (check_shape(u, B, H, W) != DDK_OK || t_start < 0) return 0;
    return sampler_layout(*u, B, H, W, t_start).total * sizeof(float);
}

extern "C" int ddk_sampler_run(const ddk_sampler_args* a, ddk_stream_t s) {
    DDK_REQUIRE(a && a->unet && a->packed && a->x && a->workspace, "sampler: null pointer");
    DDK_REQUIRE(a->c_recip && a->c_recipm1 && a->c1 && a->c2 && a->sigma, "sampler: null schedule table");
    ddk_unet& u = *const_cast<ddk_unet*>(a->unet);
    DDK_TRY(check_shape(&u, a->B, a->H, a->W));
    DDK_REQUIRE(a->t_start >= a->t_end && a->t_end >= 0, "sampler: need t_start >= t_end >= 0");
    DDK_REQUIRE(aligned16(a->packed) && aligned16(a->workspace) && aligned16(a->x) && aligned16(a->noise), "sampler: alignment");
    const int B = a->B, H = a->H, W = a->W, C = u.cfg.in_ch;
    const long long per = (long long)H * W * C;
    DDK_REQUIRE(per % 4 == 0, "sampler: H*W*in_ch must be a multiple of 4");
    const SamplerLayout sl = sampler_layout(u, B, H, W, a->t_start);
    if (a->workspace_bytes < sl.total * sizeof(float)) {
        set_error("sampler: workspace too small (%zu < %zu)", a->workspace_bytes, sl.total * sizeof(float));
        return DDK_ERR_WORKSPACE;
    }
    DDK_TRY(ensure_device_init());
    const Layout ly = make_layout(u, B, H, W);
    hipStream_t st = as_stream(s);
    float* ws = static_cast<float*>(a->workspace);
    float* eps_hat = ws + sl.off_eps;
    int64_t* t_cur = reinterpret_cast<int64_t*>(ws + sl.off_t);
    int64_t* state = t_cur + B;
// ... 100 lines not shown
```

### downsampled-diffusion_amd/ddk/lib.py

```python
import ctypes as C
import os

import torch

_HERE = os.path.dirname(os.path.abspath(__file__))
LIB_PATH = os.environ.get("DDK_LIB", os.path.join(os.path.dirname(_HERE), "csrc", "libddk.so"))


class DDKError(RuntimeError):
    pass


ABI_VERSION = 400
ERR_CLUSTER = -4


class ConvArgs(C.Structure):
    _fields_ = [
        ("kind", C.c_int), ("src0", C.c_void_p), ("src1", C.c_void_p), ("c0", C.c_int), ("c1", C.c_int),
        ("weight", C.c_void_p), ("bias", C.c_void_p), ("resid", C.c_void_p), ("out", C.c_void_p),
        ("B", C.c_int), ("H", C.c_int), ("W", C.c_int), ("N", C.c_int), ("pre_mish", C.c_int), ("post_mish", C.c_int), ("defer_reduce", C.c_int),
        ("workspace", C.c_void_p), ("workspace_bytes", C.c_size_t), ("weight_wino", C.c_void_p),
        ("gn_partials", C.c_void_p), ("gn_groups", C.c_int), ("mish_out", C.c_void_p), ("dmish_src", C.c_void_p),
    ]


class UnetConfig(C.Structure):
    _fields_ = [("in_ch", C.c_int), ("chan", C.c_int), ("n_levels", C.c_int), ("mults", C.c_int * 8)]


class SamplerArgs(C.Structure):
    _fields_ = [
        ("unet", C.c_void_p), ("packed", C.c_void_p), ("x", C.c_void_p), ("noise", C.c_void_p),
        ("c_recip", C.c_void_p), ("c_recipm1", C.c_void_p), ("c1", C.c_void_p), ("c2", C.c_void_p),
        ("sigma", C.c_void_p), ("B", C.c_int), ("H", C.c_int), ("W", C.c_int), ("t_start", C.c_int),
        ("t_end", C.c_int), ("seed", C.c_uint64), ("stream_id", C.c_uint32), ("use_graph", C.c_int),
        ("workspace", C.c_void_p), ("workspace_bytes", C.c_size_t),
    ]


class WgradReduceJob(C.Structure):
    _fields_ = [("slab", C.c_void_p), ("grad", C.c_void_p), ("bias_slab", C.c_void_p), ("grad_b", C.c_void_p), ("slab_stride", C.c_longlong),
                ("block0", C.c_longlong), ("splits", C.c_int), ("N", C.c_int), ("ntaps", C.c_int), ("cx", C.c_int), ("c_real", C.c_int),
                ("cw", C.c_int), ("c_off", C.c_int), ("reserved", C.c_int)]


class RowsSumJob(C.Structure):
    _fields_ = [("rows", C.c_void_p), ("out", C.c_void_p * 4), ("batch_stride", C.c_longlong), ("row_stride", C.c_longlong),
                ("block0", C.c_longlong), ("nbatch", C.c_int), ("nrows", C.c_int), ("n", C.c_int), ("reserved", C.c_int)]


class PackJob(C.Structure):
    _fields_ = [("src", C.c_void_p), ("dst", C.c_void_p), ("total", C.c_longlong), ("block0", C.c_longlong), ("kind", C.c_int),
                ("p", C.c_int * 7)]


_P, _I, _LL, _F, _SZ = C.c_void_p, C.c_int, C.c_longlong, C.c_float, C.c_size_t

SIGNATURES = {
    "ddk_version": (_I, []),
    "ddk_last_error": (C.c_char_p, []),
    "ddk_device_ok": (_I, []),
    "ddk_nchw_to_nhwc": (_I, [_P, _P, _I, _I, _I, _I, _I, _P]),
    "ddk_nhwc_to_nchw": (_I, [_P, _P, _I, _I, _I, _I, _I, _P]),
    "ddk_pad_channels": (_I, [_P, _P, _LL, _I, _I, _P]),
    "ddk_pack_conv_weight": (_I, [_P, _P, _I, _I, _I, _I, _I, _P]),
    "ddk_pack_convT_weight": (_I, [_P, _P, _I, _I, _P]),
    "ddk_pack_conv_weight_split": (_I, [_P, _P, _I, _I, _I, _I, _I, _I, _I, _P]),
    "ddk_pack_convT_weight_padded": (_I, [_P, _P, _I, _I, _I, _P]),
    "ddk_pack_linear_T": (_I, [_P, _P, _I, _I, _I, _I, _P]),
    "ddk_pack_conv_weight_wino": (_I, [_P, _P, _I, _I, _I, _P]),
    "ddk_pack_conv_weight_wino_dgrad": (_I, [_P, _P, _I, _I, _I, _I, _I, _P]),
    "ddk_conv_wino_splits": (_I, [_I, _I, _I, _I, _I]),
    "ddk_pack_convT_weight_wino": (_I, [_P, _P, _I, _I, _I, _P]),
    "ddk_convT_wino_splits": (_I, [_I, _I, _I, _I, _I]),
    "ddk_conv_gn_partials": (_I, [_I, _I, _I, _I, _I, _I]),
    "ddk_groupnorm_mish_partials": (_I, [_P, _P, _I, _P, _P, _P, _I, _P, _P, _I, _I, _I, _I, _F, _P]),
    "ddk_pack_conv_weight_first": (_I, [_P, _P, _I, _I, _P]),
    "ddk_conv_first_ok": (_I, [_I, _I, _I, _I, _I]),
    "ddk_conv_first": (_I, [_P, _P, _P, _P, _P, _I, _I, _I, _I, _I, _I, _P]),
    "ddk_conv1x1_ws_ok": (_I, [C.c_longlong, _I, _I]),
    "ddk_conv1x1_ws": (_I, [_P, _P, _P, _P, _P, C.c_longlong, _I, _P, _P, _F, _P]),
    "ddk_conv1x1_ws_images": (_I, [_P, _P, _P, _P, _P, C.c_longlong, _I, _P, _P, _F, _I, _P]),
    "ddk_linattn_context_kv": (_I, [_P, _P, _I, _I, _I, _P, _SZ, _P]),
    "ddk_attention_fold": (_I, [_P, _P, _P, _P, _P, _P, _P, _P, _P, _I, _I, _I, _P]),
    "ddk_groupnorm_mish_partials_res1x1": (_I, [_P, _P, _I, _P, _P, _P, _I, _P, _P, _P, _I, _P, _I, _I, _I, _I, _F, _P]),
    "ddk_final_tail": (_I, [_P, _P, _I, _P, _P, _F, _P, _P, _I, _P, _P, _P, _P, _P, _P, _P, _P, _P, C.c_uint64, C.c_uint32, _I, _I, _I, _I, _P]),
    "ddk_pack_conv_weight_local": (_I, [_P, _P, _I, _I, _I, _P]),
    "ddk_pack_conv1x1_weight_local": (_I, [_P, _P, _I, _I, _I, _P]),
    "ddk_pack_convT_weight_local": (_I, [_P, _P, _I, _I, _P]),
    "ddk_pack_conv_weight_wino_local": (_I, [_P, _P, _I, _I, _I, _P]),
    "ddk_conv3x3_gn_mish_wino_ok": (_I, [_I, _I, _I, _I, _I, _I]),
    "ddk_conv3x3_gn_mish_wino": (_I, [_P, _I, _P, _I, _P, _P, _P, _P, _P, _I, _P, _P, _I, _I, _I, _I, _I, _F, _P]),
    "ddk_conv3x3_gn_mish_slabs": (_I, [_P, _I, _LL, _P, _I, _P, _P, _P, _P, _P, _I, _P, _I, _LL, _P, _P, _I, _I, _I, _I, _I, _F, _P]),
    "ddk_attention_kv_context_workspace_bytes": (_SZ, [_I, _I]),
    "ddk_attention_kv_context_ok": (_I, [_I, _I, _I, _I]),
    "ddk_attention_kv_context": (_I, [_P, _P, _P, _P, _F, _P, _I, _I, _P, _SZ, _P]),
    "ddk_pack_qkv_operand": (_I, [_P, _P, _I, _I, _P]),
    "ddk_linattn_small_from_x": (_I, [_P, _P, _P, _P, _F, _P, _P, _I, _I, _I, _I, _P]),
    "ddk_conv3x3_gn_mish_ok": (_I, [_I, _I, _I, _I, _I, _I]),
    "ddk_conv3x3_gn_mish": (_I, [_P, _I, _P, _I, _P, _P, _P, _P, _P, _I, _P, _P, _I, _I, _I, _I, _I, _F, _P]),
    "ddk_conv_workspace_bytes": (_SZ, [_I, _I, _I, _I, _I, _I]),
    "ddk_conv_splits": (_I, [_I, _I, _I, _I, _I, _I]),
    "ddk_conv_forward": (_I, [C.POINTER(ConvArgs), _P]),
    "ddk_debug_read_stamps": (_I, [_P]),
    "ddk_groupnorm_mish": (_I, [_P, _P, _P, _P, _I, _P, _P, _I, _I, _I, _I, _F, _P, _SZ, _P]),
    "ddk_groupnorm_workspace_bytes": (_SZ, [_I, _I, _I, _I]),
    "ddk_groupnorm_mish_slabs": (_I, [_P, _I, _LL, _P, _P, _P, _P, _I, _P, _P, _I, _I, _I, _I, _F, _P]),
    "ddk_chan_layernorm": (_I, [_P, _P, _P, _P, _LL, _I, _F, _P]),
    "ddk_mish": (_I, [_P, _P, _LL, _P]),
    "ddk_tanh": (_I, [_P, _P, _LL, _P]),
    "ddk_avgpool2": (_I, [_P, _P, _I, _I, _I, _I, _P]),
    "ddk_upsample_nearest2": (_I, [_P, _P, _I, _I, _I, _I, _P]),
    "ddk_add": (_I, [_P, _P, _P, _LL, _P]),
    "ddk_linattn_context_workspace_bytes": (_SZ, [_I, _I, _I]),
    "ddk_linattn_context": (_I, [_P, _P, _I, _I, _I, _P, _SZ, _P]),
    "ddk_linattn_apply": (_I, [_P, _P, _P, _I, _I, _I, _P]),
    "ddk_linattn_fused_small": (_I, [_P, _P, _P, _I, _I, _I, _P]),
    "ddk_time_mlp": (_I, [_P, _P, _P, _P, _P, _P, _P, _P, _I, _I, _P]),
    "ddk_time_proj": (_I, [_P, _P, _P, _P, _I, _I, _I, _P]),
    "ddk_conv1x1_small_n": (_I, [_P, _P, _P, _P, _LL, _I, _I, _P]),
    "ddk_q_sample": (_I, [_P, _P, _P, _P, _P, _P, _I, _LL, _P]),
    "ddk_p_sample_update": (_I, [_P, _P, _P, _P, _P, _P, _P, _P, _P, _I, _LL, C.c_uint64, C.c_uint32, _P]),
    "ddk_randn": (_I, [_P, _LL, C.c_uint64, C.c_uint32, C.c_uint32, _P]),
    "ddk_fix_samples": (_I, [_P, _P, _I, _I, _I, _I, _P]),
    "ddk_sq_err_sum": (_I, [_P, _P, _P, _I, _LL, _P]),
    "ddk_vlb_terms_workspace_bytes": (_SZ, [_I, _LL]),
    "ddk_vlb_terms": (_I, [_P, _P, _P, _P, _P, _P, _P, _P, _P, _P, _P, _P, _I, _LL, _P, _SZ, _P]),
    "ddk_unet_create": (_P, [C.POINTER(UnetConfig)]),
    "ddk_unet_destroy": (None, [_P]),
    "ddk_unet_num_slots": (_I, [_P]),
    "ddk_unet_slot_name": (C.c_char_p, [_P, _I]),
    "ddk_unet_slot_numel": (_LL, [_P, _I]),
    "ddk_unet_packed_bytes": (_SZ, [_P]),
    "ddk_unet_pack_slot": (_I, [_P, _I, _P, _P, _P]),
    "ddk_unet_finalize_pack": (_I, [_P, _P, _P]),
    "ddk_unet_workspace_bytes": (_SZ, [_P, _I, _I, _I]),
    "ddk_unet_forward": (_I, [_P, _P, _P, _P, _P, _I, _I, _I, _P, _SZ, _P]),
    "ddk_conv3x3_gn_mish_cluster_ok": (_I, [_I, _I, _I, _I, _I, _I]),
    "ddk_conv3x3_gn_mish_cluster_workspace_bytes": (_SZ, [_I, _I, _I, _I]),
    "ddk_conv3x3_gn_mish_cluster_split_workspace_bytes": (_SZ, [_I, _I, _I, _I, _I, _I]),
    "ddk_conv3x3_gn_mish_cluster": (_I, [_P, _I, _P, _I, _P, _P, _P, _P, _P, _I, _P, _P, _I, _I, _I, _I, _I, _F, _P, _SZ, _P]),
    "ddk_unet_set_option": (_I, [_P, _I, _I]),
    "ddk_debug_cluster_timeouts": (C.c_uint, []),
    "ddk_conv3x3_gn_mish_cluster_check": (_I, [_P, _I, _P]),
    "ddk_unet_cluster_check": (_I, [_P, _P, _I, _I, _I, _P]),
    "ddk_debug_occupy": (_I, [_I, _I, _I, _P]),
    "ddk_debug_clock_probe": (_I, [_P, _I, _P]),
    "ddk_unet_flops": (C.c_double, [_P, _I, _I, _I]),
    "ddk_unet_flops_executed": (C.c_double, [_P, _I, _I, _I]),
    "ddk_sampler_workspace_bytes": (_SZ, [_P, _I, _I, _I, _I]),
    "ddk_sampler_run": (_I, [C.POINTER(SamplerArgs), _P]),
    "ddk_sampler_invalidate": (_I, [_P]),
    "ddk_sampler_release_workspace": (_I, [_P, _P]),
    "ddk_pack_conv_weight_dgrad": (_I, [_P, _P, _I, _I, _I, _I, _I, _I, _P]),
    "ddk_zero_stuff2": (_I, [_P, _P, _I, _I, _I, _I, _I, _I, _P]),
    "ddk_conv_wgrad_workspace_bytes": (_SZ, [_I, _I, _I, _I, _I, _I]),
    "ddk_conv_wgrad": (_I, [_I, _P, _P, _P, _I, _I, _I, _I, _I, _I, _I, _I, _P, _SZ, _P]),
    "ddk_conv_wgrad_bias": (_I, [_I, _P, _P, _P, _P, _I, _I, _I, _I, _I, _I, _I, _I, _P, _SZ, _P]),
    "ddk_bias_grad": (_I, [_P, _P, _LL, _I, _I, _P, _SZ, _P]),
    "ddk_groupnorm_train_workspace_bytes": (_SZ, [_I, _I, _I, _I]),
    "ddk_dropout_epoch": (_I, [C.c_uint64, _I, _P]),
    "ddk_groupnorm_mish_train_fwd": (_I, [_P, _P, _P, _P, _I, _P, _F, C.c_uint64, C.c_uint32, _P, _I, _I, _I, _I, _F, _P, _SZ, _P]),
    "ddk_groupnorm_mish_bwd": (_I, [_P, _P, _P, _F, C.c_uint64, C.c_uint32, _P, _P, _P, _I, _I, _I, _I, _F, _P, _SZ, _P]),
    "ddk_groupnorm_mish_train_fwd_slabs": (_I, [_P, _I, _LL, _P, _P, _P, _P, _P, _I, _P, _F, C.c_uint64, C.c_uint32, _P, _I, _I, _I, _I,
                                                _F, _P]),
    "ddk_groupnorm_mish_bwd_slabs": (_I, [_P, _P, _P, _F, C.c_uint64, C.c_uint32, _P, _I, _LL, _P, _P, _I, _I, _I, _I, _F, _P]),
    "ddk_rows_sum": (_I, [_P, _I, _LL, _P, _I, _I, _P]),
    "ddk_rows_sum_batched": (_I, [_P, _I, _LL, _I, _LL, _P, _I, _I, _P]),
    "ddk_rows_sum_targets": (_I, [_P, _I, _LL, _I, _LL, _P, _P, _P, _P, _I, _I, _P]),
    "ddk_multi_add": (_I, [_P, _P, _I, _LL, _P]),
    "ddk_conv_wgrad_defer": (_I, [_I, _P, _P, _P, _P, _I, _I, _I, _I, _I, _I, _I, _I, _P, _SZ, _P, _P]),
    "ddk_wgrad_reduce_jobs": (_I, [_P, _I, _P]),
    "ddk_rows_sum_jobs": (_I, [_P, _I, _P]),
    "ddk_pack_jobs_layout": (_LL, [_P, _I]),
    "ddk_pack_jobs": (_I, [_P, _I, _LL, _P]),
    "ddk_chan_layernorm_bwd": (_I, [_P, _P, _P, _P, _P, _I, C.POINTER(C.c_int), _LL, _I, _F, _P]),
    "ddk_chan_layernorm_bwd_add": (_I, [_P, _P, _P, _P, _P, _P, _I, C.POINTER(C.c_int), _LL, _I, _F, _P]),
    "ddk_groupnorm_mish_generic_train_fwd": (_I, [_P, _P, _P, _P, _I, _P, _F, C.c_uint64, C.c_uint32, _P, _I, _I, _I, _I, _I, _F, _P]),
    "ddk_groupnorm_mish_generic_bwd": (_I, [_P, _P, _P, _F, C.c_uint64, C.c_uint32, _P, _P, _P, _I, _I, _I, _I, _I, _F, _P]),
    "ddk_chan_layernorm_generic": (_I, [_P, _P, _P, _P, _LL, _I, _I, _F, _P]),
    "ddk_chan_layernorm_generic_bwd": (_I, [_P, _P, _P, _P, _P, _P, _I, C.POINTER(C.c_int), _LL, _I, _I, _F, _P]),
    "ddk_linattn_train_workspace_bytes": (_SZ, [_I, _I, _I]),
    "ddk_linattn_stats": (_I, [_P, _P, _I, _I, _I, _P, _SZ, _P]),
    "ddk_linattn_bwd": (_I, [_P, _P, _P, _P, _P, _P, _I, _I, _I, _P, _SZ, _P]),
    "ddk_linattn_bwd_recompute": (_I, [_P, _P, _P, _P, _P, _P, _I, _I, _I, _P, _SZ, _P]),
    "ddk_mish_bwd": (_I, [_P, _P, _P, _LL, _P]),
    "ddk_tanh_bwd": (_I, [_P, _P, _P, _LL, _P]),
    "ddk_avgpool2_bwd": (_I, [_P, _P, _I, _I, _I, _I, _P]),
    "ddk_upsample_nearest2_bwd": (_I, [_P, _P, _I, _I, _I, _I, _P]),
    "ddk_sq_err_grad": (_I, [_P, _P, _P, _P, _I, _LL, _P]),
    "ddk_ae_objective": (_I, [_P, _P, _P, _I, _I, _P, _P]),
    "ddk_ae_objective_bwd": (_I, [_P, _P, _I, _I, _P, _P, _P]),
    "ddk_scale_per_sample": (_I, [_P, _P, _P, _I, _LL, _P]),
    "ddk_conv1x1_small_n_bwd": (_I, [_P, _P, _P, _P, _P, _I, C.POINTER(C.c_int), _LL, _I, _I, _P]),
# ... 54 lines not shown
```

### downsampled-diffusion_amd/ddk/ops.py

```python
import ctypes as C

import torch

from . import lib as L

CONV3X3_S1, CONV3X3_S2, CONV1X1, CONVT4X4_S2 = 0, 1, 2, 3
GN_GROUPS, GN_EPS, LN_EPS = 8, 1e-5, 1e-5


def pad32(c):
    return (c + 31) // 32 * 32


class _PackEntry:
    __slots__ = ("wref", "out", "job", "fresh", "pooled")


_pack_cache = {}
_weights_epoch = [0]
_pack_table = {}
pack_stats = {"single": 0, "batched_launches": 0, "batched_jobs": 0}
_graph_tables = []
_graph_keep = [_graph_tables]

# ... 106 lines not shown
        raise L.DDKError(f"expected float32, got {t.dtype}")
    return t


def nchw_to_nhwc(x, c_pad=None):
    b, c, h, w = x.shape
    c_pad = c if c_pad is None else c_pad
    out = torch.empty((b, h, w, c_pad), device=x.device, dtype=torch.float32)
    L.check(L.load().ddk_nchw_to_nhwc(L.ptr(_f32(x)), L.ptr(out), b, c, h, w, c_pad, L.stream()), "nchw_to_nhwc")
    return out


def nhwc_to_nchw(x, c=None):
    b, h, w, cs = x.shape
    c = cs if c is None else c
    out = torch.empty((b, c, h, w), device=x.device, dtype=torch.float32)
    L.check(L.load().ddk_nhwc_to_nchw(L.ptr(_f32(x)), L.ptr(out), b, c, h, w, cs, L.stream()), "nhwc_to_nchw")
    return out


def pad_channels(x, c_pad):
    c = x.shape[-1]
    out = torch.empty((*x.shape[:-1], c_pad), device=x.device, dtype=torch.float32)
    L.check(L.load().ddk_pad_channels(L.ptr(_f32(x)), L.ptr(out), x.numel() // c, c, c_pad, L.stream()), "pad_channels")
    return out


def pack_conv_weight(w):
    o, i, kh, kw = w.shape
    out = torch.empty((o, kh * kw, pad32(i)), device=w.device, dtype=torch.float32)
    L.check(L.load().ddk_pack_conv_weight(L.ptr(_f32(w.contiguous())), L.ptr(out), o, i, kh, kw, pad32(i), L.stream()),
            "pack_conv_weight")
    return out


def pack_convT_weight(w):
    i, o, kh, kw = w.shape
    if (kh, kw) != (4, 4):
        raise L.DDKError("pack_convT_weight: kernel must be 4x4")
    out = torch.empty((4, o, 4, i), device=w.device, dtype=torch.float32)
    L.check(L.load().ddk_pack_convT_weight(L.ptr(_f32(w.contiguous())), L.ptr(out), i, o, L.stream()), "pack_convT_weight")
    return out


def pack_conv_weight_wino(w):
    o, i, kh, kw = w.shape
    if (kh, kw) != (3, 3):
        raise L.DDKError("pack_conv_weight_wino: kernel must be 3x3")
    out = torch.empty((pad32(i) // 32, 16, o, 32), device=w.device, dtype=torch.float32)
    L.check(L.load().ddk_pack_conv_weight_wino(L.ptr(_f32(w.contiguous())), L.ptr(out), o, i, pad32(i), L.stream()), "pack_conv_weight_wino")
    return out


def pack_convT_weight_wino(w):
    i, o, kh, kw = w.shape
    if (kh, kw) != (4, 4):
        raise L.DDKError("pack_convT_weight_wino: kernel must be 4x4")
    out = torch.empty((4, pad32(i) // 32, 9, o, 32), device=w.device, dtype=torch.float32)
    L.check(L.load().ddk_pack_convT_weight_wino(L.ptr(_f32(w.contiguous())), L.ptr(out), i, o, pad32(i), L.stream()), "pack_convT_weight_wino")
    return out


def pack_conv_weight_local(w):
    o, i, kh, kw = w.shape
    if (kh, kw) != (3, 3) or o % 32:
        raise L.DDKError("pack_conv_weight_local: kernel must be 3x3 and O % 32 == 0")
    out = torch.empty((o // 32, 9, pad32(i) // 32, 1024), device=w.device, dtype=torch.float32)
    L.check(L.load().ddk_pack_conv_weight_local(L.ptr(_f32(w.contiguous())), L.ptr(out), o, i, pad32(i), L.stream()), "pack_conv_weight_local")
    return out


def pack_conv_weight_wino_local(w):
    o, i, kh, kw = w.shape
    if (kh, kw) != (3, 3) or o % 32:
        raise L.DDKError("pack_conv_weight_wino_local: kernel must be 3x3 and O % 32 == 0")
    out = torch.empty((o // 32, pad32(i) // 32, 16, 1024), device=w.device, dtype=torch.float32)
    L.check(L.load().ddk_pack_conv_weight_wino_local(L.ptr(_f32(w.contiguous())), L.ptr(out), o, i, pad32(i), L.stream()),
            "pack_conv_weight_wino_local")
    return out


def wino_weight(weight, x_shape, c_lo=None, c_hi=None, dgrad=False):
    b, h, w_, cin_x = x_shape
    o, i = weight.shape[0], weight.shape[1]
    if tuple(weight.shape[2:]) != (3, 3):
        return None
    if dgrad:
        lo, hi = (0 if c_lo is None else c_lo), (i if c_hi is None else c_hi)
        n_out, cin = hi - lo, o
    else:
        lo, hi, n_out, cin = 0, i, o, pad32(i)
    if L.load().ddk_conv_wino_splits(b, h, w_, pad32(cin), n_out) <= 0:
        return None
    if dgrad:
        def pack(t):
            out = torch.empty((pad32(o) // 32, 16, hi - lo, 32), device=t.device, dtype=torch.float32)
            L.check(L.load().ddk_pack_conv_weight_wino_dgrad(L.ptr(_f32(t.contiguous())), L.ptr(out), o, i, lo, hi, pad32(o), L.stream()),
                    "pack_conv_weight_wino_dgrad")
            return out
        return cached_pack(("wino_dgrad", lo, hi), weight, pack)
    return cached_pack("wino", weight, pack_conv_weight_wino)


def conv(kind, x, w_packed, bias=None, n_out=None, x2=None, resid=None, pre_mish=False, post_mish=False, w_wino=None, mish_out=None,
         dmish_src=None, leave_slabs=False):
    b, h, w_, c0 = x.shape
# ... 138 lines not shown
    ws = _ws(x.device, nbytes, "kvctx")
    L.check(lib.ddk_attention_kv_context(L.ptr(_f32(x)), L.ptr(wkv), L.ptr(c1), L.ptr(c2), eps, L.ptr(ctx), b, h * w_, L.ptr(ws), nbytes,
                                         L.stream()), "attention_kv_context")
    return ctx


def groupnorm_mish_from_partials_res1x1(x, part, tiles_per_image, gamma, beta, res_x, res_w, res_b, temb=None, groups=GN_GROUPS,
                                        eps=GN_EPS):
    b, h, w_, n = x.shape
    cin = res_x.shape[-1]
    out = torch.empty_like(x)
    stride = temb.stride(0) if temb is not None else 0
    L.check(L.load().ddk_groupnorm_mish_partials_res1x1(
        L.ptr(_f32(x)), L.ptr(part), tiles_per_image, L.ptr(gamma), L.ptr(beta), temb.data_ptr() if temb is not None else None, stride,
        L.ptr(_f32(res_x)), L.ptr(res_w.reshape(n, cin).contiguous()), L.ptr(res_b), cin, L.ptr(out), b, h * w_, n, groups, eps,
        L.stream()), "groupnorm_mish_partials_res1x1")
    return out


def final_tail(raw, part, tiles_per_image, gamma, beta, w, bias, x=None, t=None, tables=None, noise=None, seed=0, stream_id=0,
               want_eps=True, groups=GN_GROUPS, eps=GN_EPS):
    b, h, w_, c = raw.shape
    n_out = w.shape[0]
    eps_out = torch.empty((b, h, w_, n_out), device=raw.device, dtype=torch.float32) if want_eps else None
    tb = tables or {}
    L.check(L.load().ddk_final_tail(L.ptr(_f32(raw)), L.ptr(part), tiles_per_image, L.ptr(gamma), L.ptr(beta), eps,
                                    L.ptr(w.reshape(n_out, c).contiguous()), L.ptr(bias), n_out, L.ptr(eps_out), L.ptr(x), L.ptr(noise),
                                    L.ptr(t), L.ptr(tb.get("c_recip")), L.ptr(tb.get("c_recipm1")), L.ptr(tb.get("c1")),
                                    L.ptr(tb.get("c2")), L.ptr(tb.get("sigma")), seed, stream_id, b, h * w_, c, groups, L.stream()),
            "final_tail")
    return eps_out


def conv3x3_gn_mish_cluster(x, w_wino, bias, gamma, beta, x2=None, temb=None, addend=None, groups=GN_GROUPS, eps=GN_EPS, check=True):
    b, h, w_, c0 = x.shape
    c1 = 0 if x2 is None else x2.shape[-1]
    n = w_wino.shape[2]
    lib = L.load()
    if lib.ddk_conv3x3_gn_mish_cluster_ok(b, h, w_, c0 + c1, n, groups) <= 0:
        raise L.DDKError(f"conv3x3_gn_mish_cluster: shape {tuple(x.shape)} (+{c1}) -> {n} not eligible")
    nbytes = max(lib.ddk_conv3x3_gn_mish_cluster_workspace_bytes(b, h, w_, n),
                 lib.ddk_conv3x3_gn_mish_cluster_split_workspace_bytes(b, h, w_, c0 + c1, n, groups))
    ws = _ws(x.device, nbytes, "cluster")
    out = torch.empty((b, h, w_, n), device=x.device, dtype=torch.float32)
    stride = temb.stride(0) if temb is not None else 0
    L.check(lib.ddk_conv3x3_gn_mish_cluster(L.ptr(_f32(x)), c0, L.ptr(x2), c1, L.ptr(w_wino), L.ptr(bias), L.ptr(gamma), L.ptr(beta),
                                            temb.data_ptr() if temb is not None else None, stride, L.ptr(addend), L.ptr(out), b, h, w_, n,
                                            groups, eps, L.ptr(ws), nbytes, L.stream()), "conv3x3_gn_mish_cluster")
    if check:
        L.check(lib.ddk_conv3x3_gn_mish_cluster_check(L.ptr(ws), b, L.stream()), "conv3x3_gn_mish_cluster")
    return out


def cluster_check(device, b):
    ws = _scratch.get((str(device), "cluster", torch.cuda.current_stream().cuda_stream))
    if ws is None:
        raise L.DDKError(f"cluster_check: no cluster workspace on {device} for the current stream")
    L.check(L.load().ddk_conv3x3_gn_mish_cluster_check(L.ptr(ws), b, L.stream()), "conv3x3_gn_mish_cluster")


class ClockProbe:

    def __init__(self, device, workgroups=64):
        self.n = workgroups
        self.a = torch.zeros((workgroups, 4), device=device, dtype=torch.int64)
        self.b = torch.zeros((workgroups, 4), device=device, dtype=torch.int64)
        self._first = True

    def probe(self):
        buf = self.a if self._first else self.b
        self._first = False
        L.check(L.load().ddk_debug_clock_probe(buf.data_ptr(), self.n, L.stream()), "debug_clock_probe")

    def ghz(self):
        a, b = self.a.cpu().numpy(), self.b.cpu().numpy()
        rates = []
        for i in range(min(len(a), len(b))):
            if int(a[i, 3]) == 1 and int(b[i, 3]) == 1 and int(a[i, 0]) == int(b[i, 0]):
                dc, dt = int(b[i, 1]) - int(a[i, 1]), int(b[i, 2]) - int(a[i, 2])
                if dt > 0 and dc > 0:
                    rates.append(dc / dt * 0.1)
        rates.sort()
        return rates[len(rates) // 2] if rates else None


def cluster_timeouts():
    return int(L.load().ddk_debug_cluster_timeouts())


def conv3x3_groupnorm_mish(x, w_packed, bias, gamma, beta, x2=None, temb=None, addend=None, groups=GN_GROUPS, eps=GN_EPS, w_wino=None):
    b, h, w_, c0 = x.shape
    c1 = 0 if x2 is None else x2.shape[-1]
    n = w_packed.shape[0]
    lib = L.load()
    wino = w_wino is not None and lib.ddk_conv_wino_splits(b, h, w_, c0 + c1, n) > 0
    if wino and lib.ddk_conv_gn_partials(b, h, w_, c0 + c1, n, groups) > 0:
        raw, part, np_ = conv_with_gn_partials(x, w_packed, bias, w_wino, x2=x2, groups=groups)
        return groupnorm_mish_from_partials(raw, part, np_, gamma, beta, temb=temb, addend=addend, groups=groups, eps=eps)
    splits = lib.ddk_conv_wino_splits(b, h, w_, c0 + c1, n) if wino else lib.ddk_conv_splits(CONV3X3_S1, b, h, w_, c0 + c1, n)
    if splits == 1 or lib.ddk_groupnorm_workspace_bytes(b, h * w_, n, groups) != 0:
        return groupnorm_mish(conv(CONV3X3_S1, x, w_packed, bias, x2=x2, w_wino=w_wino), gamma, beta, temb=temb, addend=addend,
                              groups=groups, eps=eps)
    ws_bytes = splits * b * h * w_ * n * 4 if wino else lib.ddk_conv_workspace_bytes(CONV3X3_S1, b, h, w_, c0 + c1, n)
    ws = torch.empty(ws_bytes // 4, device=x.device, dtype=torch.float32)
    out = torch.empty((b, h, w_, n), device=x.device, dtype=torch.float32)
    a = L.ConvArgs(CONV3X3_S1, L.ptr(_f32(x)), L.ptr(x2), c0, c1, L.ptr(w_packed), None, None, L.ptr(out), b, h, w_, n, 0, 0, 1,
# ... 713 lines not shown
```

### include/ddk.h

```cpp
#ifndef DDK_H
#define DDK_H

#include <stddef.h>
#include <stdint.h>

#ifdef __cplusplus
extern "C" {
#endif

typedef void* ddk_stream_t;

#define DDK_OK 0
#define DDK_ERR_ARG (-1)
#define DDK_ERR_HIP (-2)
#define DDK_ERR_WORKSPACE (-3)
#define DDK_ERR_CLUSTER (-4)

int ddk_version(void);
const char* ddk_last_error(void);
int ddk_device_ok(void);

int ddk_nchw_to_nhwc(const float* src, float* dst, int B, int C, int H, int W, int c_pad, ddk_stream_t s);
int ddk_nhwc_to_nchw(const float* src, float* dst, int B, int C, int H, int W, int c_stride, ddk_stream_t s);
int ddk_pad_channels(const float* src, float* dst, long long M, int C, int c_pad, ddk_stream_t s);
int ddk_pack_conv_weight(const float* w_oihw, float* dst, int O, int I, int KH, int KW, int i_pad, ddk_stream_t s);
int ddk_pack_conv_weight_split(const float* w_oihw, float* dst, int O, int I, int KH, int KW, int i_pad, int split, int split_pad,
                               ddk_stream_t s);
int ddk_pack_convT_weight(const float* w_iohw, float* dst, int I, int O, ddk_stream_t s);
int ddk_pack_convT_weight_padded(const float* w_iohw, float* dst, int I, int O, int c_pad, ddk_stream_t s);
int ddk_pack_linear_T(const float* w_oi, float* dst, int O, int I, int ld, int col0, ddk_stream_t s);

enum ddk_conv_kind {
    DDK_CONV3X3_S1 = 0,
    DDK_CONV3X3_S2 = 1,
    DDK_CONV1X1 = 2,
    DDK_CONVT4X4_S2 = 3,
    DDK_CONV4X4_S2 = 4
};

typedef struct ddk_conv_args {
    int kind;
    const float* src0;
    const float* src1;
    int c0, c1;
    const float* weight;
    const float* bias;
    const float* resid;
    float* out;
    int B, H, W;
    int N;
    int pre_mish;
    int post_mish;
    int defer_reduce;
    void* workspace;
    size_t workspace_bytes;
    const float* weight_wino;
    float* gn_partials;
    int gn_groups;
    float* mish_out;
    const float* dmish_src;
} ddk_conv_args;

int ddk_pack_conv_weight_wino(const float* w_oihw, float* dst, int O, int I, int i_pad, ddk_stream_t s);
int ddk_conv_gn_partials(int B, int H, int W, int cin, int N, int groups);
int ddk_conv_wino_splits(int B, int H, int W, int cin, int N);
size_t ddk_conv_workspace_bytes(int kind, int B, int H, int W, int cin, int N);
int ddk_conv_splits(int kind, int B, int H, int W, int cin, int N);
int ddk_conv_forward(const ddk_conv_args* a, ddk_stream_t s);
int ddk_debug_read_stamps(unsigned long long* host_out);

int ddk_groupnorm_mish(const float* x, const float* gamma, const float* beta, const float* temb,
                       int temb_stride, const float* addend, float* out, int B, int HW, int C, int groups,
                       float eps, void* workspace, size_t workspace_bytes, ddk_stream_t s);
size_t ddk_groupnorm_workspace_bytes(int B, int HW, int C, int groups);
int ddk_groupnorm_mish_slabs(const float* slabs, int nslab, long long slab_stride, const float* conv_bias,
                             const float* gamma, const float* beta, const float* temb, int temb_stride,
                             const float* addend, float* out, int B, int HW, int C, int groups, float eps,
                             ddk_stream_t s);
int ddk_pack_conv_weight_local(const float* w_oihw, float* dst, int O, int I, int i_pad, ddk_stream_t s);
int ddk_pack_conv1x1_weight_local(const float* w_oi, float* dst, int O, int I, int i_pad, ddk_stream_t s);
int ddk_pack_convT_weight_local(const float* w_iohw, float* dst, int I, int O, ddk_stream_t s);
int ddk_conv3x3_gn_mish_ok(int H, int W, int cin, int c0, int N, int groups);
int ddk_conv3x3_gn_mish(const float* src0, int c0, const float* src1, int c1, const float* weight, const float* bias,
                        const float* gamma, const float* beta, const float* temb, int temb_stride, const float* addend,
                        float* out, int B, int H, int W, int N, int groups, float eps, ddk_stream_t s);
int ddk_groupnorm_mish_partials(const float* x, const float* partials, int tiles_per_image, const float* gamma, const float* beta,
                                const float* temb, int temb_stride, const float* addend, float* out, int B, int HW, int C,
                                int groups, float eps, ddk_stream_t s);
int ddk_pack_conv_weight_first(const float* w_oihw, float* dst, int O, int I, ddk_stream_t s);
int ddk_conv_first_ok(int cin, int N, int H, int W, int groups);
int ddk_conv_first(const float* x, const float* w_first, const float* bias, float* out, float* gn_partials, int B, int H, int W,
                   int cin, int N, int groups, ddk_stream_t s);
int ddk_conv1x1_ws_ok(long long M, int K, int N);
int ddk_conv1x1_ws(const float* x, const float* w, const float* bias, const float* resid, float* out, long long M, int N,
                   const float* ln_c1, const float* ln_c2, float ln_eps, ddk_stream_t s);
int ddk_conv1x1_ws_images(const float* x, const float* w, const float* bias, const float* resid, float* out, long long M, int N,
                          const float* ln_c1, const float* ln_c2, float ln_eps, int images, ddk_stream_t s);
int ddk_groupnorm_mish_partials_res1x1(const float* x, const float* partials, int tiles_per_image, const float* gamma, const float* beta,
                                       const float* temb, int temb_stride, const float* res_x, const float* res_w, const float* res_b,
                                       int res_cin, float* out, int B, int HW, int C, int groups, float eps, ddk_stream_t s);
int ddk_pack_conv_weight_wino_local(const float* w_oihw, float* dst, int O, int I, int i_pad, ddk_stream_t s);
int ddk_conv3x3_gn_mish_wino_ok(int H, int W, int cin, int c0, int N, int groups);
int ddk_conv3x3_gn_mish_wino(const float* src0, int c0, const float* src1, int c1, const float* weight, const float* bias,
                             const float* gamma, const float* beta, const float* temb, int temb_stride, const float* addend,
                             float* out, int B, int H, int W, int N, int groups, float eps, ddk_stream_t s);
int ddk_conv3x3_gn_mish_slabs(const float* src, int src_slabs, long long src_stride, const float* src_bias, int c0, const float* weight,
                              const float* bias, const float* gamma, const float* beta, const float* temb, int temb_stride,
                              const float* addend, int addend_slabs, long long addend_stride, const float* addend_bias, float* out, int B,
                              int H, int W, int N, int groups, float eps, ddk_stream_t s);
int ddk_conv3x3_gn_mish_cluster_ok(int B, int H, int W, int cin, int N, int groups);
int ddk_conv3x3_gn_mish_cluster_check(void* workspace, int B, ddk_stream_t s);
size_t ddk_conv3x3_gn_mish_cluster_workspace_bytes(int B, int H, int W, int N);
size_t ddk_conv3x3_gn_mish_cluster_split_workspace_bytes(int B, int H, int W, int cin, int N, int groups);
int ddk_conv3x3_gn_mish_cluster(const float* src0, int c0, const float* src1, int c1, const float* weight_wino, const float* bias,
                                const float* gamma, const float* beta, const float* temb, int temb_stride, const float* addend,
                                float* out, int B, int H, int W, int N, int groups, float eps, void* workspace, size_t workspace_bytes,
// ... 24 lines not shown
int ddk_time_mlp(const int64_t* t, const float* freqs, const float* w1t, const float* b1, const float* w2t,
                 const float* b2, float* act, float* raw, int B, int dim, ddk_stream_t s);
int ddk_time_proj(const float* act, const float* wt, const float* bias, float* out, int B, int dim, int n_out,
                  ddk_stream_t s);

int ddk_conv1x1_small_n(const float* x, const float* w, const float* bias, float* out, long long M, int C,
                        int n_out, ddk_stream_t s);

int ddk_q_sample(const float* x, const float* eps, const int64_t* t, const float* sqrt_acp,
                 const float* sqrt_1m_acp, float* out, int B, long long per, ddk_stream_t s);
int ddk_p_sample_update(float* x, const float* eps_hat, const float* noise, const int64_t* t,
                        const float* c_recip, const float* c_recipm1, const float* c1, const float* c2,
                        const float* sigma, int B, long long per, uint64_t seed, uint32_t stream_id,
                        ddk_stream_t s);
int ddk_final_tail(const float* raw, const float* partials, int tiles_per_image, const float* gamma, const float* beta, float eps,
                   const float* w, const float* bias, int n_out, float* eps_out, float* x, const float* noise, const int64_t* t,
                   const float* c_recip, const float* c_recipm1, const float* c1, const float* c2, const float* sigma, uint64_t seed,
                   uint32_t stream_id, int B, int HW, int C, int groups, ddk_stream_t s);
int ddk_randn(float* out, long long n, uint64_t seed, uint32_t step, uint32_t stream_id, ddk_stream_t s);
int ddk_fix_samples(const float* x_nchw, float* out_nhwc, int B, int C, int H, int W, ddk_stream_t s);
size_t ddk_vlb_terms_workspace_bytes(int B, long long per);
int ddk_vlb_terms(const float* x, const float* x_t, const float* eps_hat, const float* eps, const int64_t* t,
                  const float* c_recip, const float* c_recipm1, const float* c1, const float* c2,
                  const float* post_logvar, float* vlb, float* sqerr, int B, long long per, void* workspace,
                  size_t workspace_bytes, ddk_stream_t s);
int ddk_sq_err_sum(const float* a, const float* b, float* per_sample, int B, long long per, ddk_stream_t s);

typedef struct ddk_unet_config {
    int in_ch;
    int chan;
    int n_levels;
    int mults[8];
} ddk_unet_config;

typedef struct ddk_unet ddk_unet;

ddk_unet* ddk_unet_create(const ddk_unet_config* cfg);
void ddk_unet_destroy(ddk_unet* u);
int ddk_unet_num_slots(const ddk_unet* u);
const char* ddk_unet_slot_name(const ddk_unet* u, int slot);
long long ddk_unet_slot_numel(const ddk_unet* u, int slot);
size_t ddk_unet_packed_bytes(const ddk_unet* u);
int ddk_unet_pack_slot(const ddk_unet* u, int slot, const float* canonical, void* packed, ddk_stream_t s);
int ddk_unet_finalize_pack(const ddk_unet* u, void* packed, ddk_stream_t s);
size_t ddk_unet_workspace_bytes(const ddk_unet* u, int B, int H, int W);
int ddk_unet_forward(const ddk_unet* u, const void* packed, const float* x, const int64_t* t, float* out,
                     int B, int H, int W, void* workspace, size_t workspace_bytes, ddk_stream_t s);
#define DDK_OPT_CLUSTER_GROUPNORM 1
#define DDK_OPT_ATTENTION_FOLD 3
#define DDK_OPT_FOLD_DOWNSAMPLE_REDUCE 5
#define DDK_OPT_ATTENTION_KV_CONTEXT 6
#define DDK_OPT_LEVEL_CHAIN 7
#define DDK_OPT_FIRST_GROUPNORM 8
int ddk_unet_set_option(ddk_unet* u, int option, int value);
int ddk_unet_cluster_check(const ddk_unet* u, void* workspace, int B, int H, int W, ddk_stream_t s);
unsigned ddk_debug_cluster_timeouts(void);
int ddk_debug_clock_probe(unsigned long long* out, int workgroups, ddk_stream_t s);
int ddk_debug_occupy(int workgroups, int lds_bytes, int microseconds, ddk_stream_t s);
double ddk_unet_flops(const ddk_unet* u, int B, int H, int W);
double ddk_unet_flops_executed(const ddk_unet* u, int B, int H, int W);

typedef struct ddk_sampler_args {
    const ddk_unet* unet;
    const void* packed;
    float* x;
    const float* noise;
    const float* c_recip;
    const float* c_recipm1;
    const float* c1;
    const float* c2;
    const float* sigma;
    int B, H, W;
    int t_start;
    int t_end;
    uint64_t seed;
    uint32_t stream_id;
    int use_graph;
    void* workspace;
    size_t workspace_bytes;
} ddk_sampler_args;

size_t ddk_sampler_workspace_bytes(const ddk_unet* u, int B, int H, int W, int t_start);
int ddk_sampler_run(const ddk_sampler_args* a, ddk_stream_t s);
int ddk_sampler_invalidate(ddk_unet* u);
int ddk_sampler_release_workspace(ddk_unet* u, const void* workspace);



int ddk_pack_conv_weight_wino_dgrad(const float* w_oihw, float* dst, int O, int I, int c_lo, int c_hi, int o_pad, ddk_stream_t s);
int ddk_pack_convT_weight_wino(const float* w_iohw, float* dst, int I, int O, int i_pad, ddk_stream_t s);
int ddk_convT_wino_splits(int B, int H, int W, int cin, int N);
int ddk_pack_conv_weight_dgrad(const float* w_oihw, float* dst, int O, int I, int KH, int KW, int i_pad, int o_pad,
                               ddk_stream_t s);
int ddk_zero_stuff2(const float* in, float* out, int B, int H, int W, int Ho, int Wo, int C, ddk_stream_t s);
size_t ddk_conv_wgrad_workspace_bytes(int kind, int B, int H, int W, int cx, int N);
int ddk_conv_wgrad(int kind, const float* x, const float* dy, float* grad_w, int B, int H, int W, int cx, int c_real,
                   int cw, int c_off, int N, void* workspace, size_t workspace_bytes, ddk_stream_t s);
int ddk_conv_wgrad_bias(int kind, const float* x, const float* dy, float* grad_w, float* grad_b, int B, int H, int W, int cx, int c_real,
                        int cw, int c_off, int N, void* workspace, size_t workspace_bytes, ddk_stream_t s);
int ddk_bias_grad(const float* dy, float* grad_b, long long M, int N, int accumulate, void* workspace,
                  size_t workspace_bytes, ddk_stream_t s);
size_t ddk_groupnorm_train_workspace_bytes(int B, int HW, int C, int groups);
int ddk_dropout_epoch(unsigned long long set_to, int bump, ddk_stream_t s);
int ddk_groupnorm_mish_train_fwd(const float* x, const float* gamma, const float* beta, const float* temb,
                                 int temb_stride, const float* addend, float drop_p, uint64_t seed, uint32_t layer,
                                 float* out, int B, int HW, int C, int groups, float eps, void* workspace,
// ... 102 lines not shown
```

Before: 25.99.

## Add Winograd F(4x4,3x3) conv kernel with fused GroupNorm epilogues for UNet

Adds a Winograd F(4,3) convolution path (6x6 tiles) with its own weight packing, a warp-specialized loader/compute kernel, and plain, GroupNorm-partials and in-launch cluster GroupNorm epilogues. The UNet selects it for eligible 3x3 convs, including the final conv, under a new option. F(4,3) needs fewer multiplies per output than the existing F(2,3) path, which should cut compute in the large-resolution convs. The trade-off is weaker numerical accuracy from the larger transform constants, plus more LDS and register pressure per workgroup.

Result: faster. 26.54, median of 6 (+2.1%).

```diff
diff --git a/downsampled-diffusion_amd/csrc/conv_wino.hip b/downsampled-diffusion_amd/csrc/conv_wino.hip
--- a/downsampled-diffusion_amd/csrc/conv_wino.hip
+++ b/downsampled-diffusion_amd/csrc/conv_wino.hip
@@ -5,6 +5,7 @@
 
 #include "conv_common.h"
 #include "pack_elems.h"
+#include "wino4_matrices.h"
 
 namespace ddk {
 
@@ -62,6 +63,25 @@
         pack_wino_elem<DGRAD>(w, dst, idx, O, I, i_pad, lo, wi);
 }
 
+__global__ __launch_bounds__(256) void pack_conv_weight_wino4_kernel(const float* __restrict__ w, float* __restrict__ dst, int O, int I,
+                                                                      int i_pad, long long total) {
+    for (long long idx = blockIdx.x * 256LL + threadIdx.x; idx < total; idx += (long long)gridDim.x * 256) {
+        const int c = (int)((unsigned)idx % (unsigned)i_pad);
+        const int n = (int)((unsigned)idx / (unsigned)i_pad);
+        double g[3][3];
+        for (int a = 0; a < 3; ++a)
+            for (int b = 0; b < 3; ++b) g[a][b] = c < I ? (double)w[(((long long)n * I + c) * 3 + a) * 3 + b] : 0.0;
+        double t[6][3];
+        for (int i = 0; i < 6; ++i)
+            for (int b = 0; b < 3; ++b) t[i][b] = wino4::G[i][0] * g[0][b] + wino4::G[i][1] * g[1][b] + wino4::G[i][2] * g[2][b];
+        for (int i = 0; i < 6; ++i)
+            for (int j = 0; j < 6; ++j) {
+                const double u = t[i][0] * wino4::G[j][0] + t[i][1] * wino4::G[j][1] + t[i][2] * wino4::G[j][2];
+                dst[((((long long)(c >> 5)) * 36 + (6 * i + j)) * O + n) * 32 + (c & 31)] = (float)u;
+            }
+    }
+}
+
 typedef int i32x4 __attribute__((ext_vector_type(4)));
 typedef float f32x4 __attribute__((ext_vector_type(4)));
 
@@ -534,6 +554,7 @@
 }
 
 #include "conv_wino2_kernel.inc"
+#include "conv_wino4_kernel.inc"
 #include "conv_winoT_kernel.inc"
 
 enum { WINO_V_OLD = 0, WINO_V_D = 1, WINO_V_F = 2 };
@@ -619,6 +640,12 @@
                                 (int)(W_LDS_FLOATS * sizeof(float))));
     DDK_HIP(hipFuncSetAttribute(reinterpret_cast<const void*>(&conv3x3_wino_kernel<0, true>), hipFuncAttributeMaxDynamicSharedMemorySize,
                                 (int)(W_LDS_FLOATS * sizeof(float))));
+    DDK_HIP(hipFuncSetAttribute(reinterpret_cast<const void*>(&conv3x3_wino4_kernel<W4_PLAIN>), hipFuncAttributeMaxDynamicSharedMemorySize,
+                                (int)(w4::LDS_FL * sizeof(float))));
+    DDK_HIP(hipFuncSetAttribute(reinterpret_cast<const void*>(&conv3x3_wino4_kernel<W4_PARTS>), hipFuncAttributeMaxDynamicSharedMemorySize,
+                                (int)(w4::LDS_FL * sizeof(float))));
+    DDK_HIP(hipFuncSetAttribute(reinterpret_cast<const void*>(&conv3x3_wino4_kernel<W4_CLUSTER>), hipFuncAttributeMaxDynamicSharedMemorySize,
+                                (int)(w4::LDS_FL * sizeof(float))));
     DDK_HIP(hipFuncSetAttribute(reinterpret_cast<const void*>(&conv3x3_wino2_kernel<2, 0, false>), hipFuncAttributeMaxDynamicSharedMemorySize,
                                 (int)(W2<2>::LDS_FL * sizeof(float))));
     DDK_HIP(hipFuncSetAttribute(reinterpret_cast<const void*>(&conv3x3_wino2_kernel<2, 0, true>), hipFuncAttributeMaxDynamicSharedMemorySize,
@@ -792,6 +819,76 @@
     return check_launch("conv3x3_wino_kernel");
 }
 
+bool conv_wino4_ok(int B, int H, int W, int cin, int N) {
+    return B > 0 && H >= 4 && W >= 4 && H % 4 == 0 && W % 4 == 0 && cin > 0 && cin % 32 == 0 && N > 0 && N % w4::NT == 0 &&
+           (long long)B * H * W * (cin > N ? cin : N) * 4 < (1LL << 31);
+}
+int conv_wino4_stats_parts(int B, int H, int W, int cin, int N, int groups) {
+    if (!conv_wino4_ok(B, H, W, cin, N) || groups <= 0 || N % groups) return 0;
+    const int cpg = N / groups;
+    if (W != 32 || H % 16 || cpg % 4 || w4::NT % cpg) return 0;
+    return H * W / 128;
+}
+int conv_wino4_cluster_np(int B, int H, int W, int cin, int N, int groups) {
+    if (!conv_wino4_ok(B, H, W, cin, N) || groups <= 0 || N % groups) return 0;
+    const int cpg = N / groups, tpi = (H / 4) * (W / 4);
+    if (cpg % 4 || w4::NT % cpg || tpi % w4::TILES) return 0;
+    const int np = tpi / w4::TILES;
+    const long long wgs = (long long)B * np * (N / w4::NT);
+    if (np > 8 || N / w4::NT > 8 || wgs < 224 || wgs > 256) return 0;
+    return np;
+}
+int conv_wino4_forward(const ddk_conv_args& a, hipStream_t st, const WinoGnFuse* fuse) {
+    DDK_REQUIRE(a.kind == DDK_CONV3X3_S1 && a.src0 && a.weight_wino && a.out && conv_wino4_ok(a.B, a.H, a.W, a.c0 + a.c1, a.N),
+                "conv(wino4): arguments or shape (H, W multiples of 4; cin, N multiples of 32)");
+    DDK_REQUIRE(a.c0 % 32 == 0 && a.c1 % 32 == 0 && (a.c1 == 0) == (a.src1 == nullptr), "conv(wino4): sources of multiples of 32 channels");
+    DDK_REQUIRE(!a.pre_mish && !a.defer_reduce && !a.mish_out && !a.dmish_src, "conv(wino4): only bias / resid / post_mish epilogues");
+    DDK_REQUIRE(aligned16(a.src0) && aligned16(a.src1) && aligned16(a.weight_wino) && aligned16(a.bias) && aligned16(a.resid) &&
+                    aligned16(a.out), "conv(wino4): 16-byte alignment");
+    WinoParams p{};
+    if (fuse) {
+        const int np = conv_wino4_cluster_np(a.B, a.H, a.W, a.c0 + a.c1, a.N, fuse->groups);
+        DDK_REQUIRE(np > 0 && !a.post_mish && !a.gn_partials && !fuse->pairs, "conv(wino4): shape not eligible for the in-launch GroupNorm");
+        DDK_REQUIRE(fuse->gamma && fuse->beta && fuse->records && fuse->counters && aligned16(fuse->gamma) && aligned16(fuse->beta) &&
+                        aligned16(fuse->temb) && fuse->temb_stride % 4 == 0 && aligned16(fuse->records) && aligned16(fuse->counters),
+                    "conv(wino4): in-launch GroupNorm arguments");
+        p.gn_gamma = fuse->gamma; p.gn_beta = fuse->beta; p.gn_temb = fuse->temb; p.gn_temb_rows = fuse->temb_rows;
+        p.gn_temb_stride = fuse->temb_stride; p.gn_eps = fuse->eps;
+        p.cl_rec = fuse->records; p.cl_cnt = fuse->counters; p.cl_fail = fuse->fail; p.cl_np = np;
+        if (fuse->res_x) {
+            DDK_REQUIRE(fuse->res_w && fuse->res_cin > 0 && fuse->res_cin <= 8 && fuse->res_ld >= fuse->res_cin && !a.resid,
+                        "conv(wino4, cluster): the 1x1 addend takes <= 8 input channels and excludes a tensor addend");
+            p.r1_x = fuse->res_x; p.r1_w = fuse->res_w; p.r1_b = fuse->res_b; p.r1_cin = fuse->res_cin; p.r1_ld = fuse->res_ld;
+        }
+        p.groups = fuse->groups;
+        p.cpg = a.N / fuse->groups;
+    }
+    if (a.gn_partials) {
+        DDK_REQUIRE(conv_wino4_stats_parts(a.B, a.H, a.W, a.c0 + a.c1, a.N, a.gn_groups) > 0 && !a.resid && !a.post_mish,
+                    "conv(wino4): gn_partials needs conv_wino4_stats_parts() > 0 and no resid / post_mish");
+        DDK_REQUIRE((reinterpret_cast<uintptr_t>(a.gn_partials) & 7u) == 0, "conv(wino4): gn_partials alignment");
+        p.gn_part = reinterpret_cast<float2*>(a.gn_partials);
+        p.groups = a.gn_groups;
+        p.cpg = a.N / a.gn_groups;
+    }
+    p.src0 = a.src0; p.src1 = a.src1; p.wu = a.weight_wino; p.bias = a.bias; p.resid = a.resid; p.out = a.out;
+    p.c0 = a.c0; p.c1 = a.c1; p.cin = a.c0 + a.c1;
+    p.B = a.B; p.H = a.H; p.W = a.W; p.TH = a.H / 4; p.TW = a.W / 4;
+    p.N = a.N; p.tiles = a.B * p.TH * p.TW;
+    p.chunks = p.cin / 32;
+    p.chunks_per_split = p.chunks;
+    p.splits = 1;
+    p.post_mish = a.post_mish;
+    p.dTW = make_fastdiv_u((unsigned)p.TW);
+    p.dTH = make_fastdiv_u((unsigned)p.TH);
+    const dim3 grid((unsigned)ceil_div(p.tiles, w4::TILES), (unsigned)(a.N / w4::NT));
+    const size_t lds = (size_t)w4::LDS_FL * sizeof(float);
+    if (fuse) hipLaunchKernelGGL(conv3x3_wino4_kernel<W4_CLUSTER>, grid, dim3(1024), lds, st, p);
+    else if (p.gn_part) hipLaunchKernelGGL(conv3x3_wino4_kernel<W4_PARTS>, grid, dim3(1024), lds, st, p);
+    else hipLaunchKernelGGL(conv3x3_wino4_kernel<W4_PLAIN>, grid, dim3(1024), lds, st, p);
+    return check_launch("conv3x3_wino4_kernel");
+}
+
 __global__ __launch_bounds__(256) void occupy_kernel(unsigned long long ticks, unsigned* sink) {
     extern __shared__ float occupy_lds[];
     occupy_lds[threadIdx.x] = (float)threadIdx.x;
@@ -818,6 +915,57 @@
     hipLaunchKernelGGL(pack_conv_weight_wino_kernel<false>, dim3((unsigned)(blocks < 4096 ? blocks : 4096)), dim3(256), 0, as_stream(s), w_oihw,
                        dst, O, I, i_pad, total, 0, I);
     return check_launch("pack_conv_weight_wino_kernel");
+}
+
+extern "C" int ddk_pack_conv_weight_wino4(const float* w_oihw, float* dst, int O, int I, int i_pad, ddk_stream_t s) {
+    using namespace ddk;
+    DDK_REQUIRE(w_oihw && dst && O > 0 && I > 0 && i_pad >= I && i_pad % 32 == 0, "pack_conv_weight_wino4: arguments (i_pad % 32 == 0)");
+    const long long total = (long long)O * i_pad;
+    DDK_REQUIRE(total * 36 < (1LL << 31), "pack_conv_weight_wino4: 2^31 packed elements or more");
+    const long long blocks = ceil_div(total, 256);
+    hipLaunchKernelGGL(pack_conv_weight_wino4_kernel, dim3((unsigned)(blocks < 4096 ? blocks : 4096)), dim3(256), 0, as_stream(s), w_oihw, dst,
+                       O, I, i_pad, total);
+    return check_launch("pack_conv_weight_wino4_kernel");
+}
+extern "C" int ddk_conv_wino4_ok(int B, int H, int W, int cin, int N) { return ddk::conv_wino4_ok(B, H, W, cin, N) ? 1 : 0; }
+extern "C" int ddk_conv_wino4_gn_partials(int B, int H, int W, int cin, int N, int groups) {
+    return ddk::conv_wino4_stats_parts(B, H, W, cin, N, groups);
+}
+extern "C" int ddk_conv_wino4_forward(const ddk_conv_args* a, ddk_stream_t s) {
+    DDK_REQUIRE(a, "conv_wino4_forward: null arguments");
+    return ddk::conv_wino4_forward(*a, ddk::as_stream(s));
+}
+extern "C" int ddk_conv3x3_gn_mish_cluster_wino4(const float* src0, int c0, const float* src1, int c1, const float* weight_wino4, const float* bias,
+                                                 const float* gamma, const float* beta, const float* temb, int temb_stride, const float* addend,
+                                                 float* out, int B, int H, int W, int N, int groups, float eps, void* workspace,
+                                                 size_t workspace_bytes, ddk_stream_t s) {
+    using namespace ddk;
+    DDK_REQUIRE(src0 && weight_wino4 && gamma && beta && out && workspace, "conv3x3_gn_mish_cluster_wino4: null pointer");
+    DDK_REQUIRE(conv_wino_cluster_device_ok() && conv_wino4_cluster_np(B, H, W, c0 + c1, N, groups) > 0,
+                "conv3x3_gn_mish_cluster_wino4: shape or device not eligible");
+    DDK_REQUIRE(ddk_conv3x3_gn_mish_cluster_workspace_bytes(B, H, W, N) > 0 &&
+                    workspace_bytes >= ddk_conv3x3_gn_mish_cluster_workspace_bytes(B, H, W, N) && aligned16(workspace),
+                "conv3x3_gn_mish_cluster_wino4: workspace (ddk_conv3x3_gn_mish_cluster_workspace_bytes)");
+    float* ws = static_cast<float*>(workspace);
+    DDK_HIP(hipMemsetAsync(ws, 0, ((size_t)B * 8 * 16 + 16) * sizeof(float), as_stream(s)));
+    ddk_conv_args a{};
+    a.kind = DDK_CONV3X3_S1;
+    a.src0 = src0; a.src1 = src1; a.c0 = c0; a.c1 = c1;
+    a.weight_wino = weight_wino4;
+    a.bias = bias;
+    a.resid = addend;
+    a.out = out;
+    a.B = B; a.H = H; a.W = W; a.N = N;
+    const WinoGnFuse f{gamma, beta, temb, nullptr, temb_stride, eps, groups, ws + (size_t)B * 8 * 16 + 16, reinterpret_cast<unsigned*>(ws),
+                       reinterpret_cast<unsigned*>(ws + (size_t)B * 8 * 16)};
+    return conv_wino4_forward(a, as_stream(s), &f);
+}
+extern "C" int ddk_debug_wino4_matrices(double* at, double* g, double* bt) {
+    DDK_REQUIRE(at && g && bt, "debug_wino4_matrices: null pointer");
+    for (int i = 0; i < 24; ++i) at[i] = ddk::wino4::AT[i / 6][i % 6];
+    for (int i = 0; i < 18; ++i) g[i] = ddk::wino4::G[i / 3][i % 3];
+    for (int i = 0; i < 36; ++i) bt[i] = ddk::wino4::BT[i / 6][i % 6];
+    return DDK_OK;
 }
 
 extern "C" int ddk_pack_convT_weight_wino(const float* w_iohw, float* dst, int I, int O, int i_pad, ddk_stream_t s) {
diff --git a/downsampled-diffusion_amd/csrc/conv_wino4_kernel.inc b/downsampled-diffusion_amd/csrc/conv_wino4_kernel.inc
--- /dev/null
+++ b/downsampled-diffusion_amd/csrc/conv_wino4_kernel.inc
@@ -0,0 +1,410 @@
+
+namespace w4 {
+constexpr int TILES = 32, NT = 32;
+constexpr int IMG = TILES * 32;
+constexpr int V_FL = 6 * IMG, U_FL = 6 * IMG, STAGE = V_FL + U_FL;
+constexpr int TP = NT + 4;
+constexpr int T_FL = 2 * 16 * TILES * TP;
+constexpr int RING_FL = 3 * STAGE;
+constexpr int RED = (RING_FL > T_FL ? RING_FL : T_FL);
+constexpr int LDS_FL = RED + 2 * 64 + 4;
+static_assert(T_FL <= RED && LDS_FL * 4 <= 160 * 1024, "LDS budget");
+constexpr int PIECES = 24;
+constexpr int LPL = PIECES / 8;
+}
+typedef float f32x2 __attribute__((ext_vector_type(2)));
+__device__ __forceinline__ void buf_load8(f32x2& d, unsigned voff, const i32x4& srd, unsigned soff) {
+    asm volatile("buffer_load_dwordx2 %0, %1, %2, %3 offen" : "=v"(d) : "v"(voff), "s"(srd), "s"(soff) : "memory");
+}
+
+enum { W4_PLAIN = 0, W4_PARTS = 1, W4_CLUSTER = 2 };
+template <int EPI>
+__global__ __launch_bounds__(1024) void conv3x3_wino4_kernel(const WinoParams p) {
+    using namespace w4;
+    extern __shared__ __attribute__((aligned(16))) float smem[];
+    const int tid = threadIdx.x, lane = tid & 63;
+    const int wid = __builtin_amdgcn_readfirstlane(tid >> 6);
+    int tile_m, tile_n;
+    {
+        const int nwg = gridDim.x * gridDim.y;
+        const int bid = blockIdx.x + gridDim.x * blockIdx.y;
+        const int q = nwg >> 3, r = nwg & 7, xcd = bid & 7, idx = bid >> 3;
+        const int logical = (xcd < r ? xcd * (q + 1) : r * (q + 1) + (xcd - r) * q) + idx;
+        tile_n = logical % gridDim.y;
+        tile_m = logical / gridDim.y;
+    }
+    const int t0 = tile_m * TILES, n0 = tile_n * NT;
+    const int n_chunks = p.chunks;
+    const int n_stages = n_chunks * 6;
+    const unsigned lds_base = (unsigned)(size_t)(__attribute__((address_space(3))) float*)smem;
+
+    if (wid >= 8) {
+        const int lw = wid - 8;
+        const int lt = lw * 64 + lane;
+        const int t = lt >> 4, cp = lt & 15;
+        __builtin_amdgcn_s_setprio(3);
+        const int g = t0 + t;
+        const bool tile_ok = g < p.tiles;
+        const unsigned gg = tile_ok ? (unsigned)g : 0u;
+        const unsigned tmp = fdiv_u(gg, p.dTW);
+        const int tx = (int)(gg - tmp * (unsigned)p.TW);
+        const unsigned bq = fdiv_u(tmp, p.dTH);
+        const int ty = (int)(tmp - bq * (unsigned)p.TH), b = (int)bq;
+        const int py0 = 4 * ty - 1, px0 = 4 * tx - 1;
+        const int pix0 = (b * p.H + py0) * p.W + px0;
+        unsigned rmask = 0, cmask = 0;
+#pragma unroll
+        for (int k = 0; k < 6; ++k) {
+            if (tile_ok && (unsigned)(py0 + k) < (unsigned)p.H) rmask |= 1u << k;
+            if ((unsigned)(px0 + k) < (unsigned)p.W) cmask |= 1u << k;
+        }
+        const i32x4 srd0 = make_srd(p.src0, (unsigned)((long long)p.B * p.H * p.W * p.c0 * 4));
+        const i32x4 srd1 = make_srd(p.src1 ? p.src1 : p.src0, (unsigned)((long long)p.B * p.H * p.W * (p.src1 ? p.c1 : p.c0) * 4));
+        const int v_off = t * 32 + (((cp >> 1) ^ ((t >> 1) & 7)) << 2) + 2 * (cp & 1);
+        f32x2 d[36];
+        auto load_row = [&](int chunk, auto rowc) {
+            constexpr int row = decltype(rowc)::value;
+            const int cc = chunk << 5;
+            const bool first = cc < p.c0;
+            const int cs = first ? p.c0 : p.c1;
+            const unsigned soff = (unsigned)((first ? cc : cc - p.c0) * 4);
+            i32x4 srd;
+            srd.x = first ? srd0.x : srd1.x; srd.y = first ? srd0.y : srd1.y; srd.z = first ? srd0.z : srd1.z; srd.w = srd0.w;
+            const unsigned base = (unsigned)(((pix0 + row * p.W) * cs + cp * 2) * 4);
+            const bool rok = (rmask >> row) & 1u;
+#pragma unroll
+            for (int dx = 0; dx < 6; ++dx) {
+                const unsigned vo = (rok && ((cmask >> dx) & 1u)) ? base + (unsigned)(dx * cs * 4) : WINO_OOB;
+                buf_load8(d[row * 6 + dx], vo, srd, soff);
+            }
+        };
+        auto pin = [&]() {
+#pragma unroll
+            for (int i = 0; i < 36; ++i) asm volatile("" : "+v"(d[i]));
+        };
+        auto bt_columns = [&]() {
+#pragma unroll
+            for (int c = 0; c < 6; ++c)
+                wino4::bt6(d[c], d[6 + c], d[12 + c], d[18 + c], d[24 + c], d[30 + c], d[c], d[6 + c], d[12 + c], d[18 + c], d[24 + c],
+                           d[30 + c]);
+        };
+        auto write_v = [&](auto ic, int buf) {
+            constexpr int i = decltype(ic)::value;
+            f32x2 o0, o1, o2, o3, o4, o5;
+            wino4::bt6(d[i * 6 + 0], d[i * 6 + 1], d[i * 6 + 2], d[i * 6 + 3], d[i * 6 + 4], d[i * 6 + 5], o0, o1, o2, o3, o4, o5);
+            float* base = smem + buf * STAGE + v_off;
+            *reinterpret_cast<f32x2*>(base + 0 * IMG) = o0;
+            *reinterpret_cast<f32x2*>(base + 1 * IMG) = o1;
+            *reinterpret_cast<f32x2*>(base + 2 * IMG) = o2;
+            *reinterpret_cast<f32x2*>(base + 3 * IMG) = o3;
+            *reinterpret_cast<f32x2*>(base + 4 * IMG) = o4;
+            *reinterpret_cast<f32x2*>(base + 5 * IMG) = o5;
+        };
+        const int prow = lane >> 3, ppos = lane & 7;
+        const unsigned uv_even = (unsigned)((prow * 32 + ((ppos ^ (prow >> 1)) << 2)) * 4);
+        const unsigned uv_odd = (unsigned)((prow * 32 + ((ppos ^ (4 + (prow >> 1))) << 2)) * 4);
+        auto issue_u = [&](int T, int buf) {
+            const int chunk = T / 6, i = T - chunk * 6;
+            const float* base = p.wu + (((long long)chunk * 36 + 6 * i) * p.N + n0) * 32;
+            const unsigned dst = lds_base + (unsigned)((buf * STAGE + V_FL) * 4);
+#pragma unroll
+            for (int j = 0; j < LPL; ++j) {
+                const int g = lw * LPL + j;
+                const int image = g >> 2, rb = g & 3;
+                lds_dma16_s(base + ((long long)image * p.N + rb * 8) * 32, (rb & 1) ? uv_odd : uv_even, dst + (unsigned)(g * 1024));
+            }
+        };
+        auto produce = [&](auto ic, int tc, int T, int buf) -> bool {
+            constexpr int i = decltype(ic)::value;
+            if constexpr (i == 0) {
+                wait_vmcnt<0>();
+                pin();
+                bt_columns();
+            }
+            write_v(ic, buf);
+            bool loaded = false;
+            if (tc + 1 < n_chunks) { load_row(tc + 1, ic); loaded = true; }
+            issue_u(T, buf);
+            return loaded;
+        };
+        using I0 = std::integral_constant<int, 0>;
+        using I1 = std::integral_constant<int, 1>;
+        static_for<6>([&](auto rc) { load_row(0, rc); });
+        issue_u(0, 0);
+        wait_vmcnt<0>();
+        pin();
+        bt_columns();
+        write_v(I0{}, 0);
+        write_v(I1{}, 1);
+        if (1 < n_chunks) { load_row(1, I0{}); load_row(1, I1{}); }
+        issue_u(1, 1);
+        asm volatile("s_waitcnt lgkmcnt(0)" ::: "memory");
+        __builtin_amdgcn_s_barrier();
+        int b0 = 0;
+        for (int qi = 0; qi < n_chunks; ++qi) {
+            static_for<6>([&](auto sc) {
+                constexpr int s = decltype(sc)::value;
+                const int S = qi * 6 + s;
+                const int buf2 = b0 == 0 ? 2 : b0 - 1;
+                const bool more = S + 2 < n_stages;
+                pin();
+                bool loaded = false;
+                if (more) loaded = produce(std::integral_constant<int, (s + 2) % 6>{}, qi + (s + 2 >= 6 ? 1 : 0), S + 2, buf2);
+                if (more) { if (loaded) wait_vmcnt<LPL + 6>(); else wait_vmcnt<LPL>(); }
+                else wait_vmcnt<0>();
+                asm volatile("s_waitcnt lgkmcnt(0)" ::: "memory");
+                __builtin_amdgcn_s_barrier();
+                b0 = b0 == 2 ? 0 : b0 + 1;
+            });
+        }
+        return;
+    }
+
+    const int mh = wid & 1, nh = (wid >> 1) & 1, cg = wid >> 2;
+    f32x4 acc[6][3];
+#pragma unroll
+    for (int i = 0; i < 6; ++i)
+#pragma unroll
+        for (int jj = 0; jj < 3; ++jj) acc[i][jj] = f32x4{0.f, 0.f, 0.f, 0.f};
+    {
+        const int r16 = lane & 15, kq = lane >> 4;
+        const int arow = 16 * mh + r16, brow = 16 * nh + r16;
+        int aoff[2], boff[2];
+#pragma unroll
+        for (int h = 0; h < 2; ++h) {
+            aoff[h] = (3 * cg) * IMG + arow * 32 + (((4 * h + kq) ^ ((arow >> 1) & 7)) << 2);
+            boff[h] = V_FL + (3 * cg) * IMG + brow * 32 + (((4 * h + kq) ^ ((brow >> 1) & 7)) << 2);
+        }
+        __builtin_amdgcn_s_barrier();
+        int buf = 0;
+        for (int c = 0; c < n_chunks; ++c) {
+            static_for<6>([&](auto sc) {
+                constexpr int i = decltype(sc)::value;
+                const float* st = smem + buf * STAGE;
+                float4 a[2][2], bb[2][2];
+                auto frag = [&](int jj, int slot) {
+#pragma unroll
+                    for (int h = 0; h < 2; ++h) {
+                        a[slot][h] = *reinterpret_cast<const float4*>(st + aoff[h] + jj * IMG);
+                        bb[slot][h] = *reinterpret_cast<const float4*>(st + boff[h] + jj * IMG);
+                    }
+                };
+                frag(0, 0);
+                static_for<3>([&](auto jc) {
+                    constexpr int jj = decltype(jc)::value;
+                    if constexpr (jj < 2) frag(jj + 1, (jj + 1) & 1);
+                    f32x4& cacc = acc[i][jj];
+#pragma unroll
+                    for (int h = 0; h < 2; ++h) {
+                        const float4& av = a[jj & 1][h];
+                        const float4& bv = bb[jj & 1][h];
+                        cacc = __builtin_amdgcn_mfma_f32_16x16x4f32(av.x, bv.x, cacc, 0, 0, 0);
+                        cacc = __builtin_amdgcn_mfma_f32_16x16x4f32(av.y, bv.y, cacc, 0, 0, 0);
+                        cacc = __builtin_amdgcn_mfma_f32_16x16x4f32(av.z, bv.z, cacc, 0, 0, 0);
+                        cacc = __builtin_amdgcn_mfma_f32_16x16x4f32(av.w, bv.w, cacc, 0, 0, 0);
+                    }
+                });
+                __builtin_amdgcn_s_barrier();
+                buf = buf == 2 ? 0 : buf + 1;
+            });
+        }
+    }
+    {
+        float* Ts = smem + cg * (16 * TILES * TP);
+        const int col = 16 * nh + (lane & 15);
+#pragma unroll
+        for (int r = 0; r < 4; ++r) {
+            const int tile = 16 * mh + 4 * (lane >> 4) + r;
+            float T[4][3];
+#pragma unroll
+            for (int jj = 0; jj < 3; ++jj) {
+                const float m0 = acc[0][jj][r], m1 = acc[1][jj][r], m2 = acc[2][jj][r], m3 = acc[3][jj][r], m4 = acc[4][jj][r],
+                            m5 = acc[5][jj][r];
+                const float pp = m1 + m2, qq = m1 - m2;
+                T[0][jj] = ((m0 + pp) + m3) + m4;
+                T[1][jj] = (qq + 0.5f * m3) - 2.0f * m4;
+                T[2][jj] = (pp + 0.25f * m3) + 4.0f * m4;
+                T[3][jj] = ((qq + 0.125f * m3) - 8.0f * m4) + m5;
+            }
+#pragma unroll
+            for (int a = 0; a < 4; ++a) {
+                float P[4];
+                if (cg == 0) {
+                    const float s = T[a][1] + T[a][2], dd = T[a][1] - T[a][2];
+                    P[0] = T[a][0] + s; P[1] = dd; P[2] = s; P[3] = dd;
+                } else {
+                    const float u = T[a][0], v = T[a][1];
+                    P[0] = u + v; P[1] = 0.5f * u - 2.0f * v; P[2] = 0.25f * u + 4.0f * v; P[3] = (0.125f * u - 8.0f * v) + T[a][2];
+                }
+#pragma unroll
+                for (int b = 0; b < 4; ++b) Ts[((a * 4 + b) * TILES + tile) * TP + col] = P[b];
+            }
+        }
+    }
+    __syncthreads();
+
+    const int cq = tid & 7, t = (tid >> 3) & 31, h = tid >> 8;
+    const int g = t0 + t, gn = n0 + cq * 4;
+    const bool ok = g < p.tiles && gn < p.N;
+    int ty = 0, tx = 0, bi = 0;
+    if (ok) {
+        const unsigned tmp = fdiv_u((unsigned)g, p.dTW);
+        tx = g - (int)tmp * p.TW;
+        const unsigned bq = fdiv_u(tmp, p.dTH);
+        ty = (int)tmp - (int)bq * p.TH;
+        bi = (int)bq;
+    }
+    float4 bias4 = make_float4(0.f, 0.f, 0.f, 0.f);
+    if (p.bias && ok) bias4 = *reinterpret_cast<const float4*>(p.bias + gn);
+    float4 keep[8];
+    int oo[8];
+#pragma unroll
+    for (int it = 0; it < 8; ++it) {
+        const int px = 2 * it + h, a = px >> 2, bcol = px & 3;
+        const float* tp = smem + (px * TILES + t) * TP + cq * 4;
+        float4 y = f4add(*reinterpret_cast<const float4*>(tp), *reinterpret_cast<const float4*>(tp + 16 * TILES * TP));
+        y = f4add(y, bias4);
+        keep[it] = make_float4(0.f, 0.f, 0.f, 0.f);
+        oo[it] = 0;
+        if (!ok) continue;
+        const int o = (((bi * p.H + 4 * ty + a) * p.W) + 4 * tx + bcol) * p.N + gn;
+        oo[it] = o;
+        if constexpr (EPI != W4_CLUSTER) {
+            if (p.resid) y = f4add(y, *reinterpret_cast<const float4*>(p.resid + o));
+            if (p.post_mish) y = make_float4(mish_f(y.x), mish_f(y.y), mish_f(y.z), mish_f(y.w));
+            *reinterpret_cast<float4*>(p.out + o) = y;
+        }
+        keep[it] = y;
+    }
+    if constexpr (EPI != W4_PLAIN) {
+        const int qpg = p.cpg >> 2;
+        const int gl = cq / qpg;
+        float* red = smem + RED;
+        auto part_sum = [&](float v, float* rd) {
+            for (int o = 1; o < qpg; o <<= 1) v += __shfl_xor(v, o, 64);
+            v += __shfl_xor(v, 8, 64);
+            v += __shfl_xor(v, 16, 64);
+            v += __shfl_xor(v, 32, 64);
+            if (lane < 8 && (cq & (qpg - 1)) == 0) rd[wid * 8 + gl] = v;
+            asm volatile("s_waitcnt lgkmcnt(0)\n\ts_barrier" ::: "memory");
+            if constexpr (EPI == W4_PARTS) return rd[(wid & 3) * 8 + gl] + rd[((wid & 3) + 4) * 8 + gl];
+            float tot = 0.f;
+#pragma unroll
+            for (int w = 0; w < 8; ++w) tot += rd[w * 8 + gl];
+            return tot;
+        };
+        auto sum4 = [](float4 v) { return (v.x + v.y) + (v.z + v.w); };
+        const float n_part = (EPI == W4_PARTS ? 128.0f : 512.0f) * (float)p.cpg;
+        float s1 = 0.f;
+#pragma unroll
+        for (int it = 0; it < 8; ++it) s1 += sum4(keep[it]);
+        const float mean = part_sum(s1, red) * (1.0f / n_part);
+        auto sq4 = [&](float4 v) {
+            const float a = v.x - mean, b = v.y - mean, c = v.z - mean, e = v.w - mean;
+            return (a * a + b * b) + (c * c + e * e);
+        };
+        float s2 = 0.f;
+#pragma unroll
+        for (int it = 0; it < 8; ++it) s2 += sq4(keep[it]);
+        const float m2 = part_sum(s2, red + 64);
+        if constexpr (EPI == W4_PARTS) {
+            if (wid < 4 && lane < 8 && (cq & (qpg - 1)) == 0)
+                p.gn_part[((long long)tile_m * 4 + wid) * p.groups + n0 / p.cpg + gl] = make_float2(mean, m2);
+        } else {
+            const int image = tile_m / p.cl_np;
+            unsigned long long* rec = reinterpret_cast<unsigned long long*>(p.cl_rec) + ((long long)tile_m * gridDim.y + tile_n) * 16;
+            unsigned* cnt = p.cl_cnt + ((long long)image * gridDim.y + tile_n) * 16;
+            int* gave_up = reinterpret_cast<int*>(red + 128);
+            if (tid == 0) *gave_up = 0;
+            if (tid < 8 && (cq & (qpg - 1)) == 0) {
+                const unsigned long long bits = (unsigned long long)__float_as_uint(mean) | ((unsigned long long)__float_as_uint(m2) << 32);
+                __hip_atomic_store(rec + gl, bits, __ATOMIC_RELAXED, __HIP_MEMORY_SCOPE_AGENT);
+            }
+            float4 ga = make_float4(0.f, 0.f, 0.f, 0.f), be = ga, ts = ga;
+            if (wid == 0) {
+                asm volatile("s_waitcnt vmcnt(0)" ::: "memory");
+                if (lane == 0) __hip_atomic_fetch_add(cnt, 1u, __ATOMIC_RELAXED, __HIP_MEMORY_SCOPE_AGENT);
+            }
+            if (ok) {
+                ga = *reinterpret_cast<const float4*>(p.gn_gamma + gn);
+                be = *reinterpret_cast<const float4*>(p.gn_beta + gn);
+                if (p.gn_temb) {
+                    const long long tr = p.gn_temb_rows ? p.gn_temb_rows[bi] : bi;
+                    ts = *reinterpret_cast<const float4*>(p.gn_temb + tr * p.gn_temb_stride + gn);
+                }
+            }
+            if (tid == 0 && __hip_atomic_load(cnt, __ATOMIC_RELAXED, __HIP_MEMORY_SCOPE_AGENT) < (unsigned)p.cl_np) {
+                const unsigned long long t_begin = __builtin_amdgcn_s_memrealtime();
+                for (;;) {
+                    __builtin_amdgcn_s_sleep(4);
+                    if (__hip_atomic_load(cnt, __ATOMIC_RELAXED, __HIP_MEMORY_SCOPE_AGENT) >= (unsigned)p.cl_np) break;
+                    if (__builtin_amdgcn_s_memrealtime() - t_begin > CL_TIMEOUT_TICKS) {
+                        atomicAdd(&g_wino_cl_timeouts, 1u);
+                        if (p.cl_fail) __hip_atomic_fetch_add(p.cl_fail, 1u, __ATOMIC_RELAXED, __HIP_MEMORY_SCOPE_AGENT);
+                        *gave_up = 1;
+                        break;
+                    }
+                }
+            }
+            __syncthreads();
+            const unsigned long long* r0 = reinterpret_cast<const unsigned long long*>(p.cl_rec) +
+                                           ((long long)image * p.cl_np * gridDim.y + tile_n) * 16 + gl;
+            const bool poisoned = *gave_up != 0;
+            float rm[8], rq[8];
+#pragma unroll
+            for (int i = 0; i < 8; ++i) {
+                rm[i] = 0.f; rq[i] = 0.f;
+                if (i < p.cl_np) {
+                    const unsigned long long bits = __hip_atomic_load(r0 + (long long)i * gridDim.y * 16, __ATOMIC_RELAXED, __HIP_MEMORY_SCOPE_AGENT);
+                    rm[i] = __uint_as_float((unsigned)bits);
+                    rq[i] = __uint_as_float((unsigned)(bits >> 32));
+                }
+            }
+            if (tid == 0) {
+                const unsigned old = __hip_atomic_fetch_add(cnt + 1, 1u, __ATOMIC_RELAXED, __HIP_MEMORY_SCOPE_AGENT);
+                if (old == (unsigned)p.cl_np - 1u) {
+                    __hip_atomic_store(cnt, 0u, __ATOMIC_RELAXED, __HIP_MEMORY_SCOPE_AGENT);
+                    __hip_atomic_store(cnt + 1, 0u, __ATOMIC_RELAXED, __HIP_MEMORY_SCOPE_AGENT);
+                }
+            }
+            float ms = 0.f;
+#pragma unroll
+            for (int i = 0; i < 8; ++i) if (i < p.cl_np) ms += rm[i];
+            const float gmean = poisoned ? __builtin_nanf("") : ms / (float)p.cl_np;
+            float gm2 = 0.f, gd2 = 0.f;
+#pragma unroll
+            for (int i = 0; i < 8; ++i) if (i < p.cl_np) { gm2 += rq[i]; gd2 += (rm[i] - gmean) * (rm[i] - gmean); }
+            const float rstd = 1.0f / sqrtf((gm2 + n_part * gd2) / ((float)p.cl_np * n_part) + p.gn_eps);
+            if (ok) {
+                float4 bb = make_float4(0.f, 0.f, 0.f, 0.f);
+                float wv[4][8];
+                if (p.r1_x) {
+                    if (p.r1_b) bb = *reinterpret_cast<const float4*>(p.r1_b + gn);
+#pragma unroll
+                    for (int jj = 0; jj < 4; ++jj)
+#pragma unroll
+                        for (int k = 0; k < 8; ++k) wv[jj][k] = k < p.r1_cin ? p.r1_w[(long long)(gn + jj) * p.r1_ld + k] : 0.f;
+                }
+#pragma unroll
+                for (int it = 0; it < 8; ++it) {
+                    const float4 v = keep[it];
+                    float4 f = make_float4(mish_f((v.x - gmean) * rstd * ga.x + be.x) + ts.x, mish_f((v.y - gmean) * rstd * ga.y + be.y) + ts.y,
+                                           mish_f((v.z - gmean) * rstd * ga.z + be.z) + ts.z, mish_f((v.w - gmean) * rstd * ga.w + be.w) + ts.w);
+                    if (p.resid) f = f4add(f, *reinterpret_cast<const float4*>(p.resid + oo[it]));
+                    if (p.r1_x) {
+                        const int pix = oo[it] / p.N;
+                        float r[4] = {bb.x, bb.y, bb.z, bb.w};
+#pragma unroll
+                        for (int k = 0; k < 8; ++k) {
+                            const float xk = k < p.r1_cin ? p.r1_x[(long long)pix * p.r1_cin + k] : 0.f;
+#pragma unroll
+                            for (int jj = 0; jj < 4; ++jj) r[jj] += xk * wv[jj][k];
+                        }
+                        f = f4add(f, make_float4(r[0], r[1], r[2], r[3]));
+                    }
+                    *reinterpret_cast<float4*>(p.out + oo[it]) = f;
+                }
+            }
+        }
+    }
+}
diff --git a/downsampled-diffusion_amd/csrc/ddk_internal.h b/downsampled-diffusion_amd/csrc/ddk_internal.h
--- a/downsampled-diffusion_amd/csrc/ddk_internal.h
+++ b/downsampled-diffusion_amd/csrc/ddk_internal.h
@@ -142,6 +142,10 @@
 bool conv_wino_ok(int kind, int H, int W, int cin, int N);
 int conv_wino_splits(int B, int H, int W, int cin, int N);
 int conv_wino_forward(const ddk_conv_args& a, int splits, hipStream_t st, const WinoGnFuse* fuse = nullptr);
+bool conv_wino4_ok(int B, int H, int W, int cin, int N);
+int conv_wino4_stats_parts(int B, int H, int W, int cin, int N, int groups);
+int conv_wino4_cluster_np(int B, int H, int W, int cin, int N, int groups);
+int conv_wino4_forward(const ddk_conv_args& a, hipStream_t st, const WinoGnFuse* fuse = nullptr);
 int conv_wino_cluster_np(int B, int H, int W, int cin, int N, int groups);
 int conv_wino_cluster_split_np(int B, int H, int W, int cin, int N, int groups, int* splits_out);
 size_t conv_wino_cluster_pair_words(int B, int H, int W, int N);
diff --git a/downsampled-diffusion_amd/csrc/unet_plan.hip b/downsampled-diffusion_amd/csrc/unet_plan.hip
--- a/downsampled-diffusion_amd/csrc/unet_plan.hip
+++ b/downsampled-diffusion_amd/csrc/unet_plan.hip
@@ -16,7 +16,8 @@
 
 enum PackKind { PK_COPY = 0, PK_CONV = 1, PK_CONVT = 2, PK_LINEAR_T = 3, PK_WINO = 4, PK_LOCAL = 5, PK_WLOCAL = 6, PK_FIRST = 7, PK_CONVT_WINO = 8,
                 PK_ROWS = 9 , PK_LOCAL1 = 10 ,
-                PK_CONVT_LOCAL = 11  };
+                PK_CONVT_LOCAL = 11 ,
+                PK_WINO4 = 12  };
 
 struct Slot {
     std::string name;
@@ -34,6 +35,8 @@
     int cin = 0, cin_pad = 0, cout = 0;
     size_t wu = 0;
     bool has_wu = false;
+    size_t wu4 = 0;
+    bool has_wu4 = false;
     size_t wl = 0;
     bool has_wl = false;
     size_t wwl = 0;
@@ -90,12 +93,14 @@
     bool cluster_split = true;
     bool attn_kvctx = true;
     bool fold_down_reduce = false;
+    bool wino4 = true;
     bool first_gn = true;
     int level_chain = 9;
     int level_chain_max_batch = 32;
     int attn_fold_min_hw = 256;
     bool attn_fold = true;
     bool generic = false;
+    int wino4_width = 0;
     std::vector<int> dimp;
     std::vector<Slot> slots;
     size_t packed_floats = 0;
@@ -148,6 +153,11 @@
             c.wu = alloc((size_t)16 * cout * c.cin_pad);
             c.has_wu = true;
             slots.push_back(Slot{prefix + "weight", (long long)cout * cin * k * k, PK_WINO, c.wu, cout, cin, k, k, c.cin_pad, 0, 0});
+        }
+        if (k == 3 && cin == cout && cout == wino4_width && cout % 32 == 0 && split == 0) {
+            c.wu4 = alloc((size_t)36 * cout * c.cin_pad);
+            c.has_wu4 = true;
+            slots.push_back(Slot{prefix + "weight", (long long)cout * cin * k * k, PK_WINO4, c.wu4, cout, cin, k, k, c.cin_pad, 0, 0});
         }
         if (k == 3 && (gn_follows || local) && cout % 32 == 0) {
             c.wl = alloc((size_t)9 * cout * c.cin_pad);
@@ -261,6 +271,7 @@
     u->cfg = *cfg;
     u->L = cfg->n_levels;
     u->generic = cfg->chan % 32 != 0;
+    u->wino4_width = cfg->chan;
     for (int i = 0; i < cfg->n_levels; ++i)
         if (cfg->chan * cfg->mults[i] > 512) { set_error("unet_create: level widths above 512 channels are not supported"); delete u; return nullptr; }
     u->dims.push_back(cfg->in_ch);
@@ -396,6 +407,13 @@
         if (!u->graphs.empty()) DDK_HIP(hipDeviceSynchronize());
         drop_graphs(u);
         u->attn_kvctx = value != 0;
+        return DDK_OK;
+    }
+    if (option == DDK_OPT_WINO4) {
+        std::lock_guard<std::mutex> lock(u->mu);
+        if (!u->graphs.empty()) DDK_HIP(hipDeviceSynchronize());
+        drop_graphs(u);
+        u->wino4 = value != 0;
         return DDK_OK;
     }
     if (option == DDK_OPT_FIRST_GROUPNORM) {
@@ -524,6 +542,7 @@
             break;
         case PK_LINEAR_T: rc = ddk_pack_linear_T(canonical, dst, sl.O, sl.I, sl.ld, sl.col0, s); break;
         case PK_WINO: rc = ddk_pack_conv_weight_wino(canonical, dst, sl.O, sl.I, sl.i_pad, s); break;
+        case PK_WINO4: rc = ddk_pack_conv_weight_wino4(canonical, dst, sl.O, sl.I, sl.i_pad, s); break;
         case PK_LOCAL: rc = ddk_pack_conv_weight_local(canonical, dst, sl.O, sl.I, sl.i_pad, s); break;
         case PK_LOCAL1: rc = ddk_pack_conv1x1_weight_local(canonical, dst, sl.O, sl.I, sl.i_pad, s); break;
         case PK_CONVT_LOCAL: rc = ddk_pack_convT_weight_local(canonical, dst, sl.I, sl.O, s); break;
@@ -714,6 +733,13 @@
     return conv_forward(a, c.st, ln);
 }
 
+static int wino4_cluster_np(const ddk_unet& u, const ConvW& cw, int B, int H, int W, int cin, int N) {
+    return u.wino4 && cw.has_wu4 ? conv_wino4_cluster_np(B, H, W, cin, N, GROUPS) : 0;
+}
+static bool final_wino4(const ddk_unet& u, int B, int H, int W, int cin, int N) {
+    return u.wino4 && u.final_conv.has_wu4 && conv_wino4_stats_parts(B, H, W, cin, N, GROUPS) == conv_wino_stats_parts(B, H, W, cin, N, GROUPS);
+}
+
 static bool conv_gn_is_local(const ConvW& cw, int B, int H, int W, int c0, int c1, int N) {
     return (cw.has_wl && (H * W == 16 || (H * W == 4 && B % 4 == 0)) && conv_gn_local_ok(H, W, c0 + c1, c0, N, GROUPS)) ||
            (cw.has_wwl && H * W == 64 && conv_gn_wlocal_ok(H, W, c0 + c1, c0, N, GROUPS));
@@ -741,6 +767,21 @@
                            nullptr, nullptr, c.st));
         return groupnorm_mish(raw, c.P + n.g, c.P + n.b, temb, c.u.temb_total, addend, out, c.B, H * W, N, GROUPS, GN_EPS,
                               c.W + c.ly.off_gn, c.ly.gn_ws * sizeof(float), c.st, c.temb_rows);
+    }
+    const int cl4 = c.allow_cluster && conv_wino_cluster_device_ok() ? wino4_cluster_np(c.u, cw, c.B, H, W, c0 + c1, N) : 0;
+    if (cl4 > 0 && cl4 <= c.u.cluster_np_max && c.n_cluster++ < c.u.cluster_limit) {
+        ddk_conv_args a{};
+        a.kind = DDK_CONV3X3_S1;
+        a.src0 = src0; a.src1 = src1; a.c0 = c0; a.c1 = c1;
+        a.weight_wino = c.P + cw.wu4;
+        a.bias = cw.has_bias ? c.P + cw.b : nullptr;
+        a.resid = addend;
+        a.out = out;
+        a.B = c.B; a.H = H; a.W = W; a.N = N;
+        float* cl = c.W + c.ly.off_cl;
+        const WinoGnFuse f{c.P + n.g, c.P + n.b, temb, c.temb_rows, c.u.temb_total, GN_EPS, GROUPS, cl + cl_counter_floats(c.B),
+                           reinterpret_cast<unsigned*>(cl), reinterpret_cast<unsigned*>(cl + cl_fail_offset(c.B))};
+        return conv_wino4_forward(a, c.st, &f);
     }
     const int cl_np = c.allow_cluster && cw.has_wu && conv_wino_cluster_device_ok() ? conv_wino_cluster_np(c.B, H, W, c0 + c1, N, GROUPS) : 0;
     if (cl_np > 0 && cl_np <= c.u.cluster_np_max && c.n_cluster++ < c.u.cluster_limit) {
@@ -1151,7 +1192,16 @@
             a.bias = r.c2.has_bias ? P + r.c2.b : nullptr;
             a.B = B; a.H = H; a.W = W; a.N = r.co;
             const int cl_np = c.allow_cluster && conv_wino_cluster_device_ok() && r.ci <= 8 ? conv_wino_cluster_np(B, H, W, r.co, r.co, GROUPS) : 0;
-            if (cl_np > 0 && cl_np <= u.cluster_np_max && conv_wino_variant_new(B, H, W, r.co) && c.n_cluster++ < u.cluster_limit) {
+            const int cl4 = c.allow_cluster && conv_wino_cluster_device_ok() && r.ci <= 8 ? wino4_cluster_np(u, r.c2, B, H, W, r.co, r.co) : 0;
+            if (cl4 > 0 && cl4 <= u.cluster_np_max && c.n_cluster++ < u.cluster_limit) {
+                a.out = bufB;
+                a.weight_wino = P + r.c2.wu4;
+                float* cl = ws + ly.off_cl;
+                WinoGnFuse f{P + r.n2.g, P + r.n2.b, nullptr, nullptr, u.temb_total, GN_EPS, GROUPS, cl + cl_counter_floats(B),
+                             reinterpret_cast<unsigned*>(cl), reinterpret_cast<unsigned*>(cl + cl_fail_offset(B))};
+                f.res_x = x; f.res_w = P + r.res.w; f.res_b = r.res.has_bias ? P + r.res.b : nullptr; f.res_cin = r.ci; f.res_ld = r.res.cin_pad;
+                DDK_TRY(conv_wino4_forward(a, st, &f));
+            } else if (cl_np > 0 && cl_np <= u.cluster_np_max && conv_wino_variant_new(B, H, W, r.co) && c.n_cluster++ < u.cluster_limit) {
                 a.out = bufB;
                 float* cl = ws + ly.off_cl;
                 WinoGnFuse f{P + r.n2.g, P + r.n2.b, nullptr, nullptr, u.temb_total, GN_EPS, GROUPS, cl + cl_counter_floats(B),
@@ -1243,7 +1293,12 @@
         a.B = B; a.H = H; a.W = W; a.N = chan;
         a.gn_partials = gnp;
         a.gn_groups = GROUPS;
-        DDK_TRY(conv_forward(a, st));
+        if (final_wino4(u, B, H, W, cur_c, chan)) {
+            a.weight_wino = P + u.final_conv.wu4;
+            DDK_TRY(conv_wino4_forward(a, st));
+        } else {
+            DDK_TRY(conv_forward(a, st));
+        }
         if (step)
             return final_tail(raw, gnp, npf, P + u.final_norm.g, P + u.final_norm.b, GN_EPS, P + u.final_w, P + u.final_b, n_out, nullptr,
                               step->x, step->noise, step->noise_step_stride, step->t_first, t, step->c_recip, step->c_recipm1, step->c1,
@@ -1351,6 +1406,8 @@
         if (gn && cw.has_wl && (H * W == 16 || (H * W == 4 && B % 4 == 0)) && conv_gn_local_ok(H, W, cin, c0, N, GROUPS))
             return 2.0 * B * H * W * 9.0 * cin * N;
         if (gn && cw.has_wwl && H * W == 64 && conv_gn_wlocal_ok(H, W, cin, c0, N, GROUPS)) return 2.0 * B * (H * W / 4) * 16.0 * cin * N;
+        if (gn && u->cluster_gn && conv_wino_cluster_device_ok() && wino4_cluster_np(*u, cw, B, H, W, cin, N) > 0)
+            return 2.0 * (double)(ceil_div((long long)B * (H / 4) * (W / 4), 32) * 32) * 36.0 * cin * N;
         if (use_wino(cw, H, W, cin, N)) return 2.0 * (double)(ceil_div((long long)B * (H / 2) * (W / 2), 32) * 32) * 16.0 * cin * N;
         return 2.0 * B * H * W * 9.0 * cin * N;
     };
@@ -1395,7 +1452,10 @@
         H *= 2; W *= 2;
         cur_c = din;
     }
-    f += conv3(u->final_conv, H, W, cur_c, 0, u->cfg.chan, true) + 2.0 * B * H * W * (double)u->cfg.chan * u->cfg.in_ch;
+    const bool fw4 = final_wino4(*u, B, H, W, cur_c, u->cfg.chan) &&
+                     final_tail_ok(H * W, u->cfg.chan, GROUPS, u->cfg.in_ch, conv_wino_stats_parts(B, H, W, cur_c, u->cfg.chan, GROUPS));
+    f += (fw4 ? 2.0 * (double)(ceil_div((long long)B * (H / 4) * (W / 4), 32) * 32) * 36.0 * cur_c * u->cfg.chan
+              : conv3(u->final_conv, H, W, cur_c, 0, u->cfg.chan, true)) + 2.0 * B * H * W * (double)u->cfg.chan * u->cfg.in_ch;
     return f;
 }
 
diff --git a/downsampled-diffusion_amd/csrc/wino4_matrices.h b/downsampled-diffusion_amd/csrc/wino4_matrices.h
--- /dev/null
+++ b/downsampled-diffusion_amd/csrc/wino4_matrices.h
@@ -0,0 +1,42 @@
+#pragma once
+
+namespace ddk {
+namespace wino4 {
+
+constexpr double AT[4][6] = {
+    {1, 1, 1, 1, 1, 0},
+    {0, 1, -1, 0.5, -2, 0},
+    {0, 1, 1, 0.25, 4, 0},
+    {0, 1, -1, 0.125, -8, 1},
+};
+constexpr double G[6][3] = {
+    {1, 0, 0},
+    {1.0 / 3, 1.0 / 3, 1.0 / 3},
+    {-1.0 / 3, 1.0 / 3, -1.0 / 3},
+    {-16.0 / 15, -8.0 / 15, -4.0 / 15},
+    {1.0 / 15, -2.0 / 15, 4.0 / 15},
+    {0, 0, 1},
+};
+constexpr double BT[6][6] = {
+    {1, -1.5, -2, 1.5, 1, 0},
+    {0, -1, 0.5, 2.5, 1, 0},
+    {0, 1, -2.5, 0.5, 1, 0},
+    {0, -2, -1, 2, 1, 0},
+    {0, 0.5, -1, -0.5, 1, 0},
+    {0, 1, -1.5, -2, 1.5, 1},
+};
+
+template <class T>
+__host__ __device__ __forceinline__ void bt6(T x0, T x1, T x2, T x3, T x4, T x5, T& o0, T& o1, T& o2, T& o3, T& o4, T& o5) {
+    const T u = x4 - x2, w = x3 - x1;
+    const T a = u + 1.5f * x3, b = w + 1.5f * x2;
+    o0 = ((x0 + u) + 1.5f * w) - x2;
+    o1 = a + b;
+    o2 = a - b;
+    o3 = u + 2.0f * w;
+    o4 = u - 0.5f * w;
+    o5 = ((x5 + 1.5f * u) - x3) - w;
+}
+
+}
+}
diff --git a/downsampled-diffusion_amd/ddk/lib.py b/downsampled-diffusion_amd/ddk/lib.py
--- a/downsampled-diffusion_amd/ddk/lib.py
+++ b/downsampled-diffusion_amd/ddk/lib.py
@@ -72,6 +72,11 @@
     "ddk_pack_conv_weight_wino": (_I, [_P, _P, _I, _I, _I, _P]),
     "ddk_pack_conv_weight_wino_dgrad": (_I, [_P, _P, _I, _I, _I, _I, _I, _P]),
     "ddk_conv_wino_splits": (_I, [_I, _I, _I, _I, _I]),
+    "ddk_pack_conv_weight_wino4": (_I, [_P, _P, _I, _I, _I, _P]),
+    "ddk_conv_wino4_ok": (_I, [_I, _I, _I, _I, _I]),
+    "ddk_conv_wino4_gn_partials": (_I, [_I, _I, _I, _I, _I, _I]),
+    "ddk_conv_wino4_forward": (_I, [C.POINTER(ConvArgs), _P]),
+    "ddk_debug_wino4_matrices": (_I, [_P, _P, _P]),
     "ddk_pack_convT_weight_wino": (_I, [_P, _P, _I, _I, _I, _P]),
     "ddk_convT_wino_splits": (_I, [_I, _I, _I, _I, _I]),
     "ddk_conv_gn_partials": (_I, [_I, _I, _I, _I, _I, _I]),
@@ -141,6 +146,7 @@
     "ddk_conv3x3_gn_mish_cluster_workspace_bytes": (_SZ, [_I, _I, _I, _I]),
     "ddk_conv3x3_gn_mish_cluster_split_workspace_bytes": (_SZ, [_I, _I, _I, _I, _I, _I]),
     "ddk_conv3x3_gn_mish_cluster": (_I, [_P, _I, _P, _I, _P, _P, _P, _P, _P, _I, _P, _P, _I, _I, _I, _I, _I, _F, _P, _SZ, _P]),
+    "ddk_conv3x3_gn_mish_cluster_wino4": (_I, [_P, _I, _P, _I, _P, _P, _P, _P, _P, _I, _P, _P, _I, _I, _I, _I, _I, _F, _P, _SZ, _P]),
     "ddk_unet_set_option": (_I, [_P, _I, _I]),
     "ddk_debug_cluster_timeouts": (C.c_uint, []),
     "ddk_conv3x3_gn_mish_cluster_check": (_I, [_P, _I, _P]),
diff --git a/downsampled-diffusion_amd/ddk/ops.py b/downsampled-diffusion_amd/ddk/ops.py
--- a/downsampled-diffusion_amd/ddk/ops.py
+++ b/downsampled-diffusion_amd/ddk/ops.py
@@ -182,6 +182,33 @@
     return out
 
 
+def pack_conv_weight_wino4(w):
+    o, i, kh, kw = w.shape
+    if (kh, kw) != (3, 3):
+        raise L.DDKError("pack_conv_weight_wino4: kernel must be 3x3")
+    out = torch.empty((pad32(i) // 32, 36, o, 32), device=w.device, dtype=torch.float32)
+    L.check(L.load().ddk_pack_conv_weight_wino4(L.ptr(_f32(w.contiguous())), L.ptr(out), o, i, pad32(i), L.stream()), "pack_conv_weight_wino4")
+    return out
+
+
+def conv_wino4(x, w_wino4, bias=None, x2=None, resid=None, post_mish=False, gn_groups=0):
+    b, h, w_, c0 = x.shape
+    c1 = 0 if x2 is None else x2.shape[-1]
+    n = w_wino4.shape[2]
+    lib = L.load()
+    out = torch.empty((b, h, w_, n), device=x.device, dtype=torch.float32)
+    part, np_ = None, 0
+    if gn_groups:
+        np_ = lib.ddk_conv_wino4_gn_partials(b, h, w_, c0 + c1, n, gn_groups)
+        if np_ <= 0:
+            raise L.DDKError(f"conv_wino4: shape {tuple(x.shape)} -> {n} cannot emit GroupNorm partials")
+        part = torch.empty((b * np_, gn_groups, 2), device=x.device, dtype=torch.float32)
+    a = L.ConvArgs(CONV3X3_S1, L.ptr(_f32(x)), L.ptr(x2), c0, c1, None, L.ptr(bias), L.ptr(resid), L.ptr(out), b, h, w_, n, 0,
+                   int(post_mish), 0, None, 0, L.ptr(w_wino4), L.ptr(part), gn_groups)
+    L.check(lib.ddk_conv_wino4_forward(C.byref(a), L.stream()), "conv_wino4_forward")
+    return (out, part, np_) if gn_groups else out
+
+
 def pack_convT_weight_wino(w):
     i, o, kh, kw = w.shape
     if (kh, kw) != (4, 4):
@@ -426,6 +453,22 @@
     return out
 
 
+def conv3x3_gn_mish_cluster_wino4(x, w_wino4, bias, gamma, beta, temb=None, addend=None, groups=GN_GROUPS, eps=GN_EPS, check=True):
+    b, h, w_, c0 = x.shape
+    n = w_wino4.shape[2]
+    lib = L.load()
+    nbytes = lib.ddk_conv3x3_gn_mish_cluster_workspace_bytes(b, h, w_, n)
+    ws = _ws(x.device, nbytes, "cluster")
+    out = torch.empty((b, h, w_, n), device=x.device, dtype=torch.float32)
+    stride = temb.stride(0) if temb is not None else 0
+    L.check(lib.ddk_conv3x3_gn_mish_cluster_wino4(L.ptr(_f32(x)), c0, None, 0, L.ptr(w_wino4), L.ptr(bias), L.ptr(gamma), L.ptr(beta),
+                                                  temb.data_ptr() if temb is not None else None, stride, L.ptr(addend), L.ptr(out), b, h, w_,
+                                                  n, groups, eps, L.ptr(ws), nbytes, L.stream()), "conv3x3_gn_mish_cluster_wino4")
+    if check:
+        L.check(lib.ddk_conv3x3_gn_mish_cluster_check(L.ptr(ws), b, L.stream()), "conv3x3_gn_mish_cluster_wino4")
+    return out
+
+
 def cluster_check(device, b):
     ws = _scratch.get((str(device), "cluster", torch.cuda.current_stream().cuda_stream))
     if ws is None:
diff --git a/include/ddk.h b/include/ddk.h
--- a/include/ddk.h
+++ b/include/ddk.h
@@ -62,6 +62,15 @@
 } ddk_conv_args;
 
 int ddk_pack_conv_weight_wino(const float* w_oihw, float* dst, int O, int I, int i_pad, ddk_stream_t s);
+int ddk_pack_conv_weight_wino4(const float* w_oihw, float* dst, int O, int I, int i_pad, ddk_stream_t s);
+int ddk_conv_wino4_ok(int B, int H, int W, int cin, int N);
+int ddk_conv_wino4_gn_partials(int B, int H, int W, int cin, int N, int groups);
+int ddk_conv_wino4_forward(const ddk_conv_args* a, ddk_stream_t s);
+int ddk_conv3x3_gn_mish_cluster_wino4(const float* src0, int c0, const float* src1, int c1, const float* weight_wino4, const float* bias,
+                                      const float* gamma, const float* beta, const float* temb, int temb_stride, const float* addend,
+                                      float* out, int B, int H, int W, int N, int groups, float eps, void* workspace, size_t workspace_bytes,
+                                      ddk_stream_t s);
+int ddk_debug_wino4_matrices(double* at, double* g, double* bt);
 int ddk_conv_gn_partials(int B, int H, int W, int cin, int N, int groups);
 int ddk_conv_wino_splits(int B, int H, int W, int cin, int N);
 size_t ddk_conv_workspace_bytes(int kind, int B, int H, int W, int cin, int N);
@@ -192,6 +201,7 @@
 #define DDK_OPT_ATTENTION_KV_CONTEXT 6
 #define DDK_OPT_LEVEL_CHAIN 7
 #define DDK_OPT_FIRST_GROUPNORM 8
+#define DDK_OPT_WINO4 12
 int ddk_unet_set_option(ddk_unet* u, int option, int value);
 int ddk_unet_cluster_check(const ddk_unet* u, void* workspace, int B, int H, int W, ddk_stream_t s);
 unsigned ddk_debug_cluster_timeouts(void);
```
